# lijx10/DeepI2P

Measured on AMD Instinct MI355X. Metric: frames/sec (img+pc infer + 60-restart GN pose) KITTI 20k-pt, 1/2/4/8 GPU, higher is better.
Workload: dtype f32 network (fp32-input MFMA; 3x3 convolutions, GEMM-shaped point layers and the per-point head: bf16 MFMA on exact three-way fp32 splits, fp32 accumulation) + f64 solver; 1 GPU; BASELINE configs[1]: KITTI 20480-pt / 160x512, batch 32 per GPU, coarse classification + 60-restart 2D GN/LM solver, max_iter 500; mode=frames, points=20480, restarts=60, parallelism=dp1, streams=8, hw_queues=4, hip_graph=True, weights_broadcast_bytes=0

## Files before the change

deepi2p_amd/_lib.py:

```python
import ctypes
import os

import torch

_HERE = os.path.dirname(os.path.abspath(__file__))
LIB_PATH = os.environ.get("DI2P_LIB") or os.path.join(_HERE, "lib", "libdeepi2p_hip.so")
_lib = None

c_void_p, c_int, c_float, c_double, c_ll = ctypes.c_void_p, ctypes.c_int, ctypes.c_float, ctypes.c_double, ctypes.c_longlong


class DeepI2PHipError(RuntimeError):
    pass


class SrcT(ctypes.Structure):
    _fields_ = [("ptr", c_void_p), ("gidx", c_void_p), ("batch_stride", c_ll), ("row_stride", c_int),
                ("channels", c_int), ("mode", c_int), ("group", c_int), ("pad_", c_int)]


class EpilogueT(ctypes.Structure):
    _fields_ = [("scale", c_void_p), ("shift", c_void_p), ("batch_bias", c_void_p), ("relu", c_int),
                ("group_max", c_int), ("g_table", c_void_p * 2), ("g_idx", c_void_p * 2), ("g_w", c_void_p * 2),
                ("g_nodes", c_int * 2), ("g_k", c_int * 2), ("transpose_out", c_int), ("group_max_out", c_void_p),
                ("planes_out", c_void_p)]


class HeadX3T(ctypes.Structure):
    _fields_ = [("src", c_void_p * 2), ("batch_stride", c_ll * 2), ("row_stride", c_int * 2), ("channels", c_int * 2),
                ("W0p", c_void_p), ("W1p", c_void_p), ("scale_shift", c_void_p), ("relu0", c_int), ("relu1", c_int),
                ("tab", c_void_p * 2), ("idx", c_void_p * 2), ("w", c_void_p * 2), ("nodes", c_int * 2),
                ("W2t", c_void_p), ("scale2", c_void_p), ("shift2", c_void_p), ("relu2", c_int), ("P", c_int)]


class HeadLabelsX3T(ctypes.Structure):
    _fields_ = [("y0", c_void_p), ("batch_stride", c_ll), ("row_stride", c_int), ("K", c_int),
                ("W1p", c_void_p), ("scale1", c_void_p), ("shift1", c_void_p), ("relu1", c_int),
                ("W2p", c_void_p), ("scale2", c_void_p), ("shift2", c_void_p), ("P", c_int),
                ("scores", c_void_p), ("coarse", c_void_p), ("fine", c_void_p)]


class SampleOptT(ctypes.Structure):
    _fields_ = [("mode", c_int), ("crop_top", c_int), ("img_scale", c_double), ("img_H", c_int), ("img_W", c_int), ("Hs", c_int), ("Ws", c_int),
                ("amplitude", c_double * 6), ("color_range", c_double * 8)]
    dataset, crop_bottom, resize_k, max_range = 0, 0, 0, 0.0


SRC_DENSE, SRC_GATHER, SRC_GROUP = 0, 1, 2

_SIGS = {
    "di2p_index_max_forward": [c_void_p, c_void_p, c_void_p, c_int, c_int, c_int, c_int, c_void_p, c_void_p],
    "di2p_index_max_values": [c_void_p, c_void_p, c_void_p, c_void_p, c_void_p, c_int, c_int, c_int, c_int, c_void_p, c_void_p],
    "di2p_ball_query_forward": [c_void_p, c_void_p, c_float, c_int, c_int, c_int, c_int, c_void_p],
    "di2p_knn_nodes": [c_void_p, c_void_p, c_void_p, c_void_p, c_int, c_int, c_int, c_int, c_void_p],
    "di2p_cluster_stats": [c_void_p, c_void_p, c_int, c_void_p, c_void_p, c_void_p, c_int, c_int, c_int, c_void_p],
    "di2p_build_point_input": [c_void_p] * 7 + [c_int, c_int, c_int, c_void_p],
    "di2p_interpolate": [c_void_p] * 4 + [c_int] * 5 + [c_void_p],
    "di2p_gather_neighbors": [c_void_p] * 4 + [c_int] * 4 + [c_void_p],
    "di2p_argmax_channels": [c_void_p, c_void_p, c_int, c_int, c_int, c_ll, c_void_p],
    "di2p_pointwise_gemm": [ctypes.POINTER(SrcT), c_int, c_void_p, c_void_p, c_int, c_int, c_int, c_int,
                            ctypes.POINTER(EpilogueT), c_void_p],
    "di2p_pointwise_gemm_x3": [ctypes.POINTER(SrcT), c_int, c_void_p, c_void_p, c_int, c_int, c_int, c_int,
                               ctypes.POINTER(EpilogueT), c_void_p],
    "di2p_pointwise_gemm_x3p": [c_void_p, c_void_p, c_void_p, c_int, c_int, c_int, c_int, ctypes.POINTER(EpilogueT), c_void_p],
    "di2p_bf16x3_pack": [c_void_p, c_int, c_int, c_void_p, c_void_p],
    "di2p_bf16x3_pack_conv3x3": [c_void_p, c_int, c_int, c_int, c_void_p, c_void_p],
    "di2p_batch_gemv": [c_void_p, c_int, c_int, c_void_p, c_int, c_void_p, c_int, c_void_p],
    "di2p_batch_gemv2": [c_void_p, c_int, c_int, c_void_p, c_int, c_int, c_void_p, c_int, c_void_p, c_int, c_void_p],
    "di2p_attention_pool": [c_void_p, c_void_p, c_void_p, c_int, c_int, c_int, c_int, c_void_p],
    "di2p_point_head": [c_void_p, c_int, c_void_p, c_int, c_void_p, c_void_p, c_void_p, c_void_p, c_int, c_void_p, c_void_p,
                        c_void_p, c_int, c_void_p, c_int, c_int, c_int, c_int, c_void_p],
    "di2p_point_chain": [c_void_p, c_int, c_void_p, c_int, c_void_p, c_void_p, c_void_p, c_void_p, c_int, c_void_p, c_void_p,
                         c_void_p, c_int, c_void_p, c_int, c_int, c_int, c_void_p],
    "di2p_conv2d": [c_void_p] * 6 + [c_int] * 11 + [c_void_p],
    "di2p_conv2d_ws": [c_void_p] * 6 + [c_int] * 11 + [c_void_p, c_ll, c_void_p],
    "di2p_maxpool3x3s2": [c_void_p, c_void_p, c_int, c_int, c_int, c_int, c_void_p],
    "di2p_global_avgpool": [c_void_p, c_void_p, c_int, c_int, c_int, c_void_p],
    "di2p_channel_max": [c_void_p, c_void_p, c_int, c_int, c_int, c_void_p],
    "di2p_initial_guess": [c_void_p] * 5 + [c_int, c_int, c_void_p],
    "di2p_solve_batched": [c_void_p] * 6 + [c_double, c_double, ctypes.POINTER(c_double), ctypes.POINTER(c_double)]
                          + [c_int] * 5 + [c_void_p, c_void_p, c_void_p, c_void_p, c_void_p, c_void_p],
    "di2p_solve_batched_f32": [c_void_p] * 6 + [c_double, c_double, ctypes.POINTER(c_double), ctypes.POINTER(c_double)]
                              + [c_int] * 5 + [c_void_p, c_void_p, c_void_p, c_void_p, c_void_p, c_void_p],
    "di2p_select_best": [c_void_p, c_void_p, c_void_p, c_int, c_int, c_int, c_void_p, c_void_p, c_void_p, c_void_p],
    "di2p_solver_residuals": [c_void_p] * 4 + [c_double, c_double, c_int, c_int, c_int, c_void_p, c_void_p, c_void_p, c_void_p],
    "di2p_f32_to_f64": [c_void_p, c_void_p, c_ll, c_void_p],
    "di2p_farthest_point_sampling": [c_void_p, c_void_p, c_void_p, c_void_p, c_int, c_int, c_int, c_void_p],
    "di2p_gather_points": [c_void_p, c_void_p, c_void_p, c_int, c_int, c_int, c_int, c_void_p],
    "di2p_project_labels": [c_void_p, c_void_p, c_int, c_void_p, c_float, c_float, c_float, c_void_p, c_void_p, c_void_p, c_int, c_int, c_void_p],
    "di2p_label_accuracy": [c_void_p, c_void_p, c_void_p, c_void_p, c_void_p, c_int, c_int, c_void_p],
    "di2p_pnp_ransac": [c_void_p] * 5 + [c_int, c_void_p, c_int, c_double, c_int, c_int, c_int, c_int] + [c_void_p] * 7,
    "di2p_draw_restarts": [ctypes.c_ulonglong, c_int, c_int, c_double, c_double, c_void_p, c_void_p, c_void_p],
    "di2p_random_choice": [ctypes.c_ulonglong, c_int, c_int, c_int, c_int, c_void_p, c_void_p, c_void_p],
    "di2p_random_choice_ragged": [ctypes.c_ulonglong, c_int, c_int, c_void_p, c_int, c_int, c_void_p, c_void_p, c_void_p],
    "di2p_voxel_down_sample": [c_void_p, c_void_p, c_int, c_int, c_int, c_double, c_double, c_int] + [c_void_p] * 9,
    "di2p_estimate_normals": [c_void_p, c_int, c_int, c_double, c_int, c_double] + [c_void_p] * 5,
    "di2p_nearest_raw": [c_void_p, c_void_p, c_void_p, c_int, c_int, c_double] + [c_void_p] * 5,
    "di2p_gather_ragged": [c_void_p] * 6 + [c_int, c_int] + [c_void_p] * 4,
    "di2p_pnp_pack": [c_void_p] * 4 + [c_int, c_int, c_int] + [c_void_p] * 3,
    "di2p_pnp_ransac_epnp": [c_void_p] * 5 + [c_int, c_void_p, c_int, c_double, c_int, c_int] + [c_void_p] * 7,
    "di2p_classifier_loss": [c_void_p] * 4 + [c_int, c_int, c_int, c_float, c_float, c_float] + [c_void_p] * 5,
    "di2p_adam_step": [c_void_p] * 4 + [c_ll, c_int, c_float, c_float, c_float, c_float, c_void_p],
    "di2p_pack_pc_label": [c_void_p, c_void_p, c_void_p, c_void_p, c_void_p, c_void_p, c_int, c_int, c_void_p],
    "di2p_stem_pack": [c_void_p, c_void_p, c_void_p],
    "di2p_conv7x7s2_stem": [c_void_p] * 5 + [c_int] * 4 + [c_void_p],
    "di2p_winograd_weight_transform": [c_void_p, c_void_p, c_int, c_int, c_void_p],
    "di2p_winograd_weight_transform_dgrad": [c_void_p, c_void_p, c_int, c_int, c_void_p],
    "di2p_conv3x3_winograd": [c_void_p] * 6 + [c_int] * 6 + [c_void_p],
    "di2p_conv3x3_x3": [c_void_p] * 6 + [c_int] * 7 + [c_void_p] * 4 + [c_int, c_void_p],
    "di2p_conv3x3_x3_supported": [c_int] * 7,
    "di2p_conv3x3_x3_plan": [c_int] * 7 + [ctypes.POINTER(ctypes.c_int32)],
    "di2p_head_x3_pack": [c_void_p, c_int, c_void_p, c_void_p],
    "di2p_stem_x3_pack": [c_void_p, c_void_p, c_void_p],
    "di2p_stem_x3_supported": [c_int, c_int],
    "di2p_stem_x3": [c_void_p] * 5 + [c_int] * 3 + [c_void_p],
    "di2p_point_head_x3": [ctypes.POINTER(HeadX3T), c_void_p, c_int, c_int, c_void_p],
    "di2p_head_labels_x3_pack": [c_void_p, c_int, c_int, c_void_p, c_void_p],
    "di2p_point_head_labels_x3": [ctypes.POINTER(HeadLabelsX3T), c_int, c_int, c_void_p],
    "di2p_bn_train_forward": [c_void_p] * 9 + [c_float, c_float, c_int, c_int, c_int, c_int, c_void_p, c_void_p],
    "di2p_bn_train_backward": [c_void_p] * 6 + [c_int] + [c_void_p] * 4 + [c_int, c_int, c_int, c_void_p, c_void_p],
    "di2p_channel_sum": [c_void_p, c_void_p, c_int, c_int, c_int, c_void_p, c_void_p],
    "di2p_bmm_rc": [c_void_p, c_ll, c_ll, c_void_p, c_ll, c_ll, c_void_p, c_int, c_int, c_int, c_int, c_float, c_int, c_void_p, c_ll, c_void_p],
    "di2p_rc_vec_ok": [c_void_p, c_ll, c_ll, c_int],
    "di2p_rc_route": [c_int] * 7 + [ctypes.POINTER(ctypes.c_int32)],
    "di2p_pointwise_route": [c_int] * 6 + [ctypes.POINTER(ctypes.c_int32)],
    "di2p_conv2d_route": [c_int] * 12 + [c_ll, ctypes.POINTER(ctypes.c_int32)],
    "di2p_winograd_route": [c_int] * 5 + [ctypes.POINTER(ctypes.c_int32)],
    "di2p_point_chain_route": [c_int] * 6 + [ctypes.POINTER(ctypes.c_int32)],
    "di2p_point_head_route": [c_int] * 8 + [ctypes.POINTER(ctypes.c_int32)],
    "di2p_bmm_km": [c_void_p, c_int, c_ll, c_void_p, c_int, c_ll, c_void_p, c_int, c_int, c_int, c_int, c_float, c_void_p],
    "di2p_gather_backward": [c_void_p, c_void_p, c_void_p, c_int, c_void_p, c_int, c_int, c_int, c_int, c_void_p, c_ll, c_void_p],
    "di2p_conv2d_wgrad": [c_void_p] * 3 + [c_int] * 9 + [c_void_p, c_ll, c_void_p],
    "di2p_conv2d_dgrad": [c_void_p] * 3 + [c_int] * 9 + [c_void_p],
    "di2p_maxpool3x3s2_backward": [c_void_p] * 3 + [c_int] * 4 + [c_void_p],
    "di2p_segment_max_backward": [c_void_p] * 4 + [c_int] * 4 + [c_void_p],
    "di2p_group_max_forward": [c_void_p, c_void_p, c_void_p, c_ll, c_int, c_void_p],
    "di2p_group_max_backward": [c_void_p, c_void_p, c_void_p, c_ll, c_int, c_void_p],
    "di2p_dropout_mask": [ctypes.c_ulonglong, c_int, c_float, c_ll, c_void_p, c_void_p],
    "di2p_apply_mask": [c_void_p, c_void_p, c_float, c_void_p, c_ll, c_void_p],
    "di2p_sample_draws": [ctypes.c_ulonglong, c_void_p, c_int, c_int, ctypes.POINTER(SampleOptT)] + [c_void_p] * 10,
    "di2p_image_prepare": [c_void_p, c_int, c_int, c_int, ctypes.POINTER(SampleOptT), c_void_p, c_void_p, c_int, c_int, c_int, c_void_p, c_void_p,
                           c_void_p],
    "di2p_transform_segments": [c_void_p] * 4 + [c_int, c_int] + [c_void_p] * 3,
    "di2p_gather_ragged_aug": [c_void_p] * 6 + [c_int, c_int, ctypes.c_ulonglong, c_void_p, c_int, c_double, c_double] + [c_void_p] * 4,
    "di2p_random_choice_dseed": [c_void_p, c_int, c_int, c_int, c_int, c_void_p, c_void_p, c_void_p],
    "di2p_random_choice_ragged_dseed": [c_void_p, c_int, c_int, c_void_p, c_int, c_int, c_void_p, c_void_p, c_void_p],
    "di2p_range_shuffle": [c_void_p, c_void_p, c_int, c_int, c_int, c_double, ctypes.c_ulonglong] + [c_void_p] * 6,
    "di2p_gather_ragged_aug_intensity": [c_void_p] * 5 + [c_int, c_int, ctypes.c_ulonglong, c_void_p, c_int, c_double, c_double] + [c_void_p] * 3,
    "di2p_sample_draws_ds": [ctypes.c_ulonglong, c_void_p, c_int, c_int, ctypes.POINTER(SampleOptT), c_int] + [c_void_p] * 10,
    "di2p_image_prepare_ds": [c_void_p, c_int, c_int, c_int, ctypes.POINTER(SampleOptT), c_int, c_int, c_void_p, c_void_p, c_void_p, c_int, c_int,
                              c_void_p, c_void_p, c_void_p],
    "di2p_estimate_normals_cells": [c_void_p, c_int, c_int, c_double, c_int, c_double] + [c_void_p] * 5,
    "di2p_compose_poses": [c_void_p, c_void_p, c_int, c_void_p, c_void_p],
    "di2p_pose_errors": [c_void_p, c_void_p, c_int, c_void_p, c_int, c_int, c_double, c_double, c_void_p, c_void_p, c_void_p, c_void_p],
    "di2p_eval_accumulate": [c_void_p] * 5 + [c_int, c_void_p, c_void_p],
    "di2p_eval_acc_reset": [c_void_p, c_void_p],
    "di2p_enu2cam_points": [c_void_p, c_void_p, c_int, c_int, c_void_p],
    "di2p_vis_classification": [c_void_p] * 6 + [c_int] * 10 + [c_void_p] * 3,
    "di2p_vis_registration": [c_void_p] * 5 + [c_int] * 7 + [c_void_p] * 3,
    "di2p_submap_build": [c_void_p] * 6 + [c_int] * 5 + [c_double, c_double, c_int] + [c_void_p] * 7,
    "di2p_submap_to_camera": [c_void_p] * 4 + [c_int, c_int, c_void_p, c_void_p],
    "di2p_pose_matrices": [c_void_p, c_int, c_void_p, c_void_p],
    "di2p_sweep_transforms": [c_void_p] * 5 + [c_int, c_int] + [c_void_p] * 3,
    "di2p_sweep_accumulate": [c_void_p] * 4 + [c_int] * 6 + [c_float, c_float] + [c_void_p] * 6,
    "di2p_world_trace": [c_void_p, c_void_p, c_int, c_int, c_void_p, c_void_p, c_int, c_void_p, c_void_p, c_void_p],
    "di2p_world_render_camera": [c_void_p, c_void_p, c_int, c_int, c_void_p, c_void_p, c_int, c_int, c_double] + [c_void_p] * 4,
    "di2p_world_render_scan": [c_void_p, c_void_p, c_int, c_int, c_void_p, c_void_p, c_void_p, c_int, c_int] + [c_double] * 4
                              + [ctypes.c_ulonglong, c_void_p, c_int] + [c_void_p] * 5,
}
# ... 122 lines not shown
```

deepi2p_amd/csrc/common.h:

```cpp
#pragma once
#include <hip/hip_runtime.h>
#include <stdint.h>
#include <stdio.h>

#include "../../include/deepi2p_hip.h"

#define DI2P_WAVE 64

void di2p_set_error(const char* fmt, ...);

#define DI2P_CHECK_ARG(cond, msg)                                   \
    do {                                                            \
        if (!(cond)) {                                              \
            di2p_set_error("%s: %s", __func__, msg);                \
            return -1;                                              \
        }                                                           \
    } while (0)

#define DI2P_RETURN_LAUNCH()                                                        \
    do {                                                                            \
        hipError_t e_ = hipGetLastError();                                          \
        if (e_ != hipSuccess) {                                                     \
            di2p_set_error("%s: launch failed: %s", __func__, hipGetErrorString(e_)); \
            return (int)e_;                                                         \
        }                                                                           \
        return 0;                                                                   \
    } while (0)

static inline int di2p_cdiv(long long a, long long b) { return (int)((a + b - 1) / b); }

#define DI2P_OPTIONS(X) \
    X(CONV_NOSPLIT, "conv_nosplit", "DI2P_CONV_NOSPLIT", 0)                        \
    X(CONV_DEPTH1, "conv_depth1", "DI2P_CONV_DEPTH1", 0)                           \
    X(PW_NOVEC, "pw_novec", "DI2P_PW_NOVEC", 0)                                    \
    X(SOLVER_NOCULL, "solver_nocull", "DI2P_SOLVER_NOCULL", 0)                     \
    X(SOLVER_NOPREFILTER, "solver_noprefilter", "DI2P_SOLVER_NOPREFILTER", 0)      \
    X(SOLVER_TIER_SWEEPS, "solver_tier_sweeps", "DI2P_SOLVER_TIER_SWEEPS", 0)      \
    X(WINO_COB, "wino_cob", "DI2P_WINO_COB", 0)                                    \
    X(CONV_NOWINOGRAD, "conv_nowinograd", "DI2P_CONV_NOWINOGRAD", 0)               \
    X(WINO_KC, "wino_kc", "DI2P_WINO_KC", 0)                                       \
    X(CONV_NOSTEM, "conv_nostem", "DI2P_CONV_NOSTEM", 0)                           \
    X(WINO_REG, "wino_reg", "DI2P_WINO_REG", 0)                                    \
    X(SOLVER_NOCACHE, "solver_nocache", "DI2P_SOLVER_NOCACHE", 0)                  \
    X(SOLVER_PREP_SINGLE, "solver_prep_single", "DI2P_SOLVER_PREP_SINGLE", 0)      \
    X(SOLVER_PREP_BITONIC, "solver_prep_bitonic", "DI2P_SOLVER_PREP_BITONIC", 0)   \
    X(PW_X3, "pw_x3", "DI2P_PW_X3", 1)                                             \
    X(PW_NOCHAIN, "pw_nochain", "DI2P_PW_NOCHAIN", 0)                              \
    X(HEAD_REG, "head_reg", "DI2P_HEAD_REG", 0)                                    \
    X(CONV_S2SCALAR, "conv_s2scalar", "DI2P_CONV_S2SCALAR", 0)                     \
    X(CONV_X3, "conv_x3", "DI2P_CONV_X3", 31)                                      \
    X(CONV_X3_CFG, "conv_x3_cfg", "DI2P_CONV_X3_CFG", -1)                          \
    X(HEAD_X3, "head_x3", "DI2P_HEAD_X3", 1)                                       \
    X(HEAD_X3_TAB, "head_x3_tab", "DI2P_HEAD_X3_TAB", 1)                           \
    X(STEM_X3, "stem_x3", "DI2P_STEM_X3", 1)                                       \
    X(BN_UNFUSED, "bn_unfused", "DI2P_BN_UNFUSED", 0)                              \
    X(PW_X3_PLANES, "pw_x3_planes", "DI2P_PW_X3_PLANES", 1)                        \
    X(CONV_DGRAD_DENSE, "conv_dgrad_dense", "DI2P_CONV_DGRAD_DENSE", 0)            \
    X(RC_TILE64, "rc_tile64", "DI2P_RC_TILE64", 0)
enum Di2pOption {
#define DI2P_OPT_ENUM(ID, NAME, ENV, DEF) DI2P_OPT_##ID,
    DI2P_OPTIONS(DI2P_OPT_ENUM)
#undef DI2P_OPT_ENUM
    DI2P_OPT_COUNT
};
long long di2p_opt(int id);
int di2p_cu_count();
int di2p_allow_dynamic_lds(const void* kernel, size_t bytes, const char* who);
void di2p_pack_a32(const float* Wt, int K, int M, int tiles, int tile_stride, int step_stride, void* Wp, void* stream);
```

deepi2p_amd/csrc/gemm.hip:

```cpp
#include "bf16x3.h"
#include "mfma_tile.h"

#include <stdint.h>
#include <stdlib.h>

namespace {

struct LoaderWt {
    const float* Wt;
    int K, M;
    __device__ __forceinline__ float load(int k, int m) const { return (k < K && m < M) ? Wt[k * M + m] : 0.0f; }
};

struct SrcDev {
    const float* ptr[DI2P_MAX_SRC];
    const int* gidx[DI2P_MAX_SRC];
    long long batch_stride[DI2P_MAX_SRC];
    int row_stride[DI2P_MAX_SRC];
    int c_end[DI2P_MAX_SRC];
    int mode[DI2P_MAX_SRC];
    int group[DI2P_MAX_SRC];
    int n_src;
};

// ... 400 lines not shown
    __syncthreads();
    {
        LoaderWt4 la{tl.W1t, HEAD_M, HEAD_M};
        EpiDev e1{};
        e1.scale = tl.sc1; e1.shift = tl.sh1; e1.relu = tl.relu1; e1.group_max = 1;
        EpiPointwise ep{e1, nullptr, b, HEAD_M, N};
        ep.lds_tile = hbuf; ep.lds_n0 = j_blk; ep.lds_ld = HEAD_BN;
        mfma_gemm_block_blds<HeadCfg>(stage, la, hbuf, HEAD_BN, ep, HEAD_M, 0, j_blk);
    }
    __syncthreads();
    const int lane = threadIdx.x & 63, p = threadIdx.x >> 6;
    const int n = j_blk + lane;
    if (p < tl.P) {
        float a = 0.0f;
        for (int k0 = 0; k0 < HEAD_M; k0 += 16) {
            float w[16], h[16];
#pragma unroll
            for (int u = 0; u < 16; ++u) { w[u] = tl.W2t[(k0 + u) * tl.P + p]; h[u] = hbuf[(k0 + u) * HEAD_BN + lane]; }
#pragma unroll
            for (int u = 0; u < 16; ++u) a = fmaf(w[u], h[u], a);
        }
        if (tl.sc2) a *= tl.sc2[p];
        if (tl.sh2) a += tl.sh2[p];
        if (tl.relu2) a = fmaxf(a, 0.0f);
        if (n < N) out[((long long)b * tl.P + p) * N + n] = a;
    }
}

struct ChainTail {
    const float* W1t;
    const float* sc1;
    const float* sh1;
    const float* W2t;
    const float* sc2;
    const float* sh2;
    int relu1, relu2;
};

__device__ __forceinline__ void chain_rows_to_ksteps(const float (&v)[16], float* f) {
#pragma unroll
    for (int g = 0; g < 4; ++g) {
        auto p = __builtin_amdgcn_permlane32_swap(__float_as_uint(v[4 * g + 0]), __float_as_uint(v[4 * g + 1]), false, false);
        auto q = __builtin_amdgcn_permlane32_swap(__float_as_uint(v[4 * g + 2]), __float_as_uint(v[4 * g + 3]), false, false);
        f[4 * g + 0] = __uint_as_float(p[0]);
        f[4 * g + 1] = __uint_as_float(q[0]);
        f[4 * g + 2] = __uint_as_float(p[1]);
        f[4 * g + 3] = __uint_as_float(q[1]);
    }
}

#ifndef DI2P_CHAIN_WAVES
#define DI2P_CHAIN_WAVES 2
#endif
template <int M, int KS0, int NL, int TN>
__global__ __launch_bounds__(256) __attribute__((amdgpu_waves_per_eu(DI2P_CHAIN_WAVES, 8))) void point_chain_kernel(const float* __restrict__ X, long long x_bs, int x_rs, const float* __restrict__ W0t,
                                                           int K0, EpiDev e0, ChainTail tl, float* __restrict__ Y, int N, int nblk, int total) {
    constexpr int TM = M / 32, KS = M / 2, KSMAX = KS0 > KS ? KS0 : KS;
    extern __shared__ __attribute__((aligned(16))) float lds[];
    float* w0 = lds;
    float* w1 = w0 + 2 * KS0 * M;
    float* w2 = w1 + M * M;
    float* ss = w2 + (NL == 3 ? M * M : 0);
    for (int i = threadIdx.x; i < 2 * KS0 * M; i += 256) w0[i] = i < K0 * M ? W0t[i] : 0.0f;
    for (int i = threadIdx.x; i < M * M; i += 256) w1[i] = tl.W1t[i];
    if (NL == 3)
        for (int i = threadIdx.x; i < M * M; i += 256) w2[i] = tl.W2t[i];
    {
        const float* rows[6] = {e0.scale, e0.shift, tl.sc1, tl.sh1, NL == 3 ? tl.sc2 : nullptr, NL == 3 ? tl.sh2 : nullptr};
#pragma unroll
        for (int q = 0; q < 6; ++q)
            if (rows[q] && threadIdx.x < M) ss[q * M + threadIdx.x] = rows[q][threadIdx.x];
    }
    __syncthreads();
    if (e0.scale) e0.scale = ss;
    if (e0.shift) e0.shift = ss + M;
    const int lane = threadIdx.x & 63, wave = __builtin_amdgcn_readfirstlane(threadIdx.x >> 6);
    const int l31 = lane & 31, half = lane >> 5;
    EpiDev e1{}, e2{};
    e1.scale = tl.sc1 ? ss + 2 * M : nullptr; e1.shift = tl.sh1 ? ss + 3 * M : nullptr; e1.relu = tl.relu1; e1.group_max = 1;
    e2.scale = tl.sc2 ? ss + 4 * M : nullptr; e2.shift = tl.sh2 ? ss + 5 * M : nullptr; e2.relu = tl.relu2; e2.group_max = 1;

    float fn[TN][KS0];
    auto request = [&](int g) {
        const int fb = g / nblk, blk = g - fb * nblk;
        const float* Xb = X + (long long)fb * x_bs;
#pragma unroll
        for (int s = 0; s < KS0; ++s) {
            const int k = 2 * s + half;
#pragma unroll
            for (int j = 0; j < TN; ++j) {
                const float x = Xb[(long long)min(k, K0 - 1) * x_rs + min((blk * TN + j) * 32 + l31, N - 1)];
                fn[j][s] = k < K0 ? x : 0.0f;
            }
        }
    };
    const int g0 = blockIdx.x * 4 + wave, stride = gridDim.x * 4;
    if (g0 < total) request(g0);
    for (int g = g0; g < total; g += stride) {
        const int b = g / nblk, blk = g - b * nblk;
        EpiPointwise ep0{e0, nullptr, b, M, N}, ep1{e1, nullptr, b, M, N}, ep2{e2, nullptr, b, M, N};
        int n[TN], nc[TN];
#pragma unroll
        for (int j = 0; j < TN; ++j) { n[j] = (blk * TN + j) * 32 + l31; nc[j] = min(n[j], N - 1); }
        float f[TN][KSMAX];
#pragma unroll
        for (int j = 0; j < TN; ++j)
#pragma unroll
            for (int s = 0; s < KS0; ++s) f[j][s] = fn[j][s];
        request(min(g + stride, total - 1));
        f32x16 acc[TM][TN];
        auto zero = [&]() {
#pragma unroll
            for (int i = 0; i < TM; ++i)
#pragma unroll
                for (int j = 0; j < TN; ++j)
#pragma unroll
                    for (int r = 0; r < 16; ++r) acc[i][j][r] = 0.0f;
        };
        auto layer = [&](const float* w, auto ks_tag) {
            constexpr int STEPS = decltype(ks_tag)::value;
            const float* wl = w + half * M + l31;
#pragma unroll
            for (int s = 0; s < STEPS; ++s) {
                float a[TM];
#pragma unroll
                for (int i = 0; i < TM; ++i) a[i] = wl[2 * s * M + i * 32];
#pragma unroll
                for (int i = 0; i < TM; ++i)
#pragma unroll
                    for (int j = 0; j < TN; ++j) acc[i][j] = __builtin_amdgcn_mfma_f32_32x32x2f32(a[i], f[j][s], acc[i][j], 0, 0, 0);
            }
        };
        auto to_operands = [&](const EpiPointwise& ep) {
#pragma unroll
            for (int j = 0; j < TN; ++j)
#pragma unroll
                for (int i = 0; i < TM; ++i) {
                    float v[16];
                    ep.apply(i * 32 + 4 * half, nc[j], acc[i][j], v);
                    chain_rows_to_ksteps(v, &f[j][i * 16]);
                }
        };
        auto to_memory = [&](const EpiPointwise& ep) {
#pragma unroll
            for (int j = 0; j < TN; ++j)
#pragma unroll
                for (int i = 0; i < TM; ++i) {
                    float v[16];
                    ep.apply(i * 32 + 4 * half, nc[j], acc[i][j], v);
                    if (n[j] < N) {
#pragma unroll
                        for (int r = 0; r < 16; ++r)
                            Y[((long long)b * M + i * 32 + 4 * half + (r & 3) + 8 * (r >> 2)) * N + n[j]] = v[r];
                    }
                }
        };
        zero();
        layer(w0, std::integral_constant<int, KS0>{});
        to_operands(ep0);
        zero();
        layer(w1, std::integral_constant<int, KS>{});
        if (NL == 3) {
            to_operands(ep1);
            zero();
            layer(w2, std::integral_constant<int, KS>{});
            to_memory(ep2);
        } else {
            to_memory(ep1);
        }
    }
}

template <bool G33, int KS0>
__global__ __launch_bounds__(512) void point_head_reg_kernel(SrcDev srcs, const float* __restrict__ W0t, int K0, EpiDev e0, HeadTail tl,
                                                              float* __restrict__ out, int N, int nblk, int total) {
    constexpr int M = HEAD_M, TM = M / 32, KS = M / 2;
    extern __shared__ __attribute__((aligned(16))) float lds[];
    float* w0 = lds;
    float* w1 = w0 + 2 * KS0 * M;
    float* w2 = w1 + M * M;
    float* ss = w2 + M * 4;
    for (int i = threadIdx.x; i < 2 * KS0 * M; i += 512) w0[i] = i < K0 * M ? W0t[i] : 0.0f;
    for (int i = threadIdx.x; i < M * M; i += 512) w1[i] = tl.W1t[i];
    for (int i = threadIdx.x; i < M * 4; i += 512) w2[i] = (i & 3) < tl.P ? tl.W2t[(i >> 2) * tl.P + (i & 3)] : 0.0f;
    {
        const float* rows[4] = {e0.scale, e0.shift, tl.sc1, tl.sh1};
#pragma unroll
        for (int q = 0; q < 4; ++q)
            if (rows[q] && threadIdx.x < M) ss[q * M + threadIdx.x] = rows[q][threadIdx.x];
    }
    __syncthreads();
    if (e0.scale) e0.scale = ss;
    if (e0.shift) e0.shift = ss + M;
    EpiDev e1{};
    e1.scale = tl.sc1 ? ss + 2 * M : nullptr; e1.shift = tl.sh1 ? ss + 3 * M : nullptr; e1.relu = tl.relu1; e1.group_max = 1;
    const int lane = threadIdx.x & 63, wave = __builtin_amdgcn_readfirstlane(threadIdx.x >> 6);
    const int l31 = lane & 31, half = lane >> 5;
    const int c0 = srcs.c_end[0];

    constexpr int CH = 8;
    static_assert(KS0 % CH == 0, "layer 0 = whole chunks");
    float f0[KS0];
    auto request = [&](int g) {
        const int fb = __builtin_amdgcn_readfirstlane(g / nblk);
        const int col = min((g - fb * nblk) * 32 + l31, N - 1);
        const int rs0 = srcs.row_stride[0], rs1 = srcs.row_stride[1];
// ... 699 lines not shown
    else hipLaunchKernelGGL(pointwise_gemm_x3p_kernel<false>, grid, dim3(256), 0, st, (const u32x4_t*)planes, (const u32x4_t*)Wp, Y, M, K, N, Mp, e);
    DI2P_RETURN_LAUNCH();
}

extern "C" int di2p_point_head(const di2p_src_t* srcs, int n_src, const float* W0t, int K0, const di2p_epilogue_t* epi0,
                               const float* W1t, const float* scale1, const float* shift1, int relu1, const float* W2t,
                               const float* scale2, const float* shift2, int relu2, float* out, int B, int M, int P, int N,
                               void* stream) {
    DI2P_CHECK_ARG(srcs && n_src >= 1 && n_src <= DI2P_MAX_SRC && W0t && W1t && W2t && out && epi0, "null pointer");
    DI2P_CHECK_ARG(M == HEAD_M && P >= 1 && P <= 4, "fused head: hidden width 128, at most 4 outputs (use the separate layers otherwise)");
    DI2P_CHECK_ARG(B >= 0 && N >= 4 && N % 4 == 0 && K0 >= 1, "bad size");
    DI2P_CHECK_ARG(epi0->group_max <= 1 && !epi0->transpose_out && !epi0->planes_out, "fused head: layer 0 takes scale/shift/relu/bias/gathered only");
    if (B == 0) return 0;
    for (int i = 0; i < n_src; ++i) DI2P_CHECK_ARG(srcs[i].ptr && srcs[i].channels > 0 && srcs[i].mode == DI2P_SRC_DENSE, "fused head: dense sources only");
    SrcDev s;
    bool dense;
    if (pw_sources(__func__, srcs, n_src, K0, "K0", s, dense)) return -1;
    DI2P_CHECK_ARG(dense, "sources must be 16-byte addressable");
    DI2P_CHECK_ARG(aligned16(W0t) && aligned16(W1t), "weights must be 16-byte aligned");
    EpiDev e;
    if (pw_epilogue(__func__, epi0, nullptr, M, N, false, e)) return -1;
    HeadTail tl{W1t, scale1, shift1, W2t, scale2, shift2, relu1, relu2, P};
    bool reg_range = true;
    for (int i = 0; i < n_src; ++i) reg_range = reg_range && (long long)srcs[i].channels * srcs[i].row_stride * 4 < (1ll << 31);
    const HeadRoute rt = head_route(K0, n_src, srcs[0].channels, reg_range, e.g_table[0] && e.g_table[1] && e.g_k[0] == 3 && e.g_k[1] == 3, B, N,
                                    di2p_cu_count());
    if (rt.reg) {
        constexpr int KS0 = 48;
        const int nblk = rt.nblk;
        const long long total = rt.total;
        DI2P_CHECK_ARG(total < (1ll << 30), "too many column blocks");
        const int wgs = rt.wgs;
        const size_t lds_reg = (size_t)(2 * KS0 * HEAD_M + HEAD_M * HEAD_M + HEAD_M * 4 + 4 * HEAD_M) * sizeof(float);
        if (rt.g33) {
            if (di2p_allow_dynamic_lds((const void*)point_head_reg_kernel<true, KS0>, lds_reg, __func__)) return -1;
            hipLaunchKernelGGL((point_head_reg_kernel<true, KS0>), dim3(wgs), dim3(512), lds_reg, (hipStream_t)stream, s, W0t, K0, e, tl, out, N, nblk, (int)total);
        } else {
            if (di2p_allow_dynamic_lds((const void*)point_head_reg_kernel<false, KS0>, lds_reg, __func__)) return -1;
            hipLaunchKernelGGL((point_head_reg_kernel<false, KS0>), dim3(wgs), dim3(512), lds_reg, (hipStream_t)stream, s, W0t, K0, e, tl, out, N, nblk, (int)total);
        }
        DI2P_RETURN_LAUNCH();
    }
    const size_t lds = (HeadCfg::LDS_FLOATS + HEAD_M * HEAD_BN) * sizeof(float);
    if (rt.g33) {
        if (di2p_allow_dynamic_lds((const void*)point_head_kernel<true>, lds, __func__)) return -1;
        hipLaunchKernelGGL(point_head_kernel<true>, dim3(di2p_cdiv(N, HEAD_BN), B), dim3(HeadCfg::THREADS), lds, (hipStream_t)stream, s, W0t, K0, e, tl, out, N);
    } else {
        if (di2p_allow_dynamic_lds((const void*)point_head_kernel<false>, lds, __func__)) return -1;
        hipLaunchKernelGGL(point_head_kernel<false>, dim3(di2p_cdiv(N, HEAD_BN), B), dim3(HeadCfg::THREADS), lds, (hipStream_t)stream, s, W0t, K0, e, tl, out, N);
    }
    DI2P_RETURN_LAUNCH();
}

extern "C" int di2p_point_chain(const di2p_src_t* srcs, int n_src, const float* W0t, int K0, const di2p_epilogue_t* epi0,
                                const float* W1t, const float* scale1, const float* shift1, int relu1, const float* W2t,
                                const float* scale2, const float* shift2, int relu2, float* Y, int B, int M, int N, void* stream) {
    DI2P_CHECK_ARG(srcs && n_src == 1 && W0t && W1t && epi0, "fused chain: one dense source");
    DI2P_CHECK_ARG(M == 32 || M == 64, "fused chain: width 32 or 64 (use the separate layers otherwise)");
    DI2P_CHECK_ARG(K0 <= M, "fused chain: at most M input channels");
    DI2P_CHECK_ARG(B >= 0 && N >= 1 && K0 >= 1, "bad size");
    DI2P_CHECK_ARG(epi0->group_max <= 1 && !epi0->transpose_out && !epi0->planes_out, "fused chain: layer 0 takes scale/shift/relu/bias/gathered only");
    if (B == 0) return 0;
    DI2P_CHECK_ARG(Y && srcs[0].ptr && srcs[0].channels == K0 && srcs[0].mode == DI2P_SRC_DENSE, "fused chain: one dense source of K0 channels");
    DI2P_CHECK_ARG((long long)srcs[0].channels * srcs[0].row_stride < (1ll << 31), "per-frame source extent must fit 31 bits");
    EpiDev e;
    if (pw_epilogue(__func__, epi0, nullptr, M, N, false, e)) return -1;
    ChainTail tl{W1t, scale1, shift1, W2t, scale2, shift2, relu1, relu2};
    const float* X = srcs[0].ptr;
    const long long x_bs = srcs[0].batch_stride;
    const int x_rs = (int)srcs[0].row_stride;
    hipStream_t st = (hipStream_t)stream;
    const ChainRoute rt = chain_route(M, K0, W2t != nullptr, B, N, di2p_cu_count());
    DI2P_CHECK_ARG(rt.total < (1ll << 30), "too many column blocks");
#define DI2P_CHAIN_LAUNCH(MM, KS0, NL, TN)                                                                                          \
    do {                                                                                                                            \
        const size_t lds = (size_t)(2 * (KS0) * (MM) + ((NL) - 1) * (MM) * (MM) + 6 * (MM)) * sizeof(float);                        \
        hipLaunchKernelGGL((point_chain_kernel<MM, KS0, NL, TN>), dim3(rt.wgs), dim3(256), lds, st, X, x_bs, x_rs, W0t, K0, e, tl, Y, N, \
                           rt.nblk, (int)rt.total);                                                                                 \
    } while (0)
    const bool three = rt.layers == 3;
    if (M == 32) {
        if (rt.ks0 == 4) { if (three) DI2P_CHAIN_LAUNCH(32, 4, 3, DI2P_CHAIN_TN32); else DI2P_CHAIN_LAUNCH(32, 4, 2, DI2P_CHAIN_TN32); }
        else             { if (three) DI2P_CHAIN_LAUNCH(32, 16, 3, DI2P_CHAIN_TN32); else DI2P_CHAIN_LAUNCH(32, 16, 2, DI2P_CHAIN_TN32); }
    } else {
        if (rt.ks0 == 16) { if (three) DI2P_CHAIN_LAUNCH(64, 16, 3, DI2P_CHAIN_TN64); else DI2P_CHAIN_LAUNCH(64, 16, 2, DI2P_CHAIN_TN64); }
        else              { if (three) DI2P_CHAIN_LAUNCH(64, 32, 3, DI2P_CHAIN_TN64); else DI2P_CHAIN_LAUNCH(64, 32, 2, DI2P_CHAIN_TN64); }
    }
#undef DI2P_CHAIN_LAUNCH
    DI2P_RETURN_LAUNCH();
}

extern "C" int di2p_point_chain_route(int M, int K0, int layers, int B, int N, int cus, int32_t* out) {
    DI2P_CHECK_ARG(out && (M == 32 || M == 64) && K0 >= 1 && K0 <= M && (layers == 2 || layers == 3) && B >= 1 && N >= 1 && cus >= 1, "bad args");
    const ChainRoute rt = chain_route(M, K0, layers == 3, B, N, cus);
    DI2P_CHECK_ARG(rt.total < (1ll << 30), "too many column blocks");
    out[0] = M; out[1] = rt.ks0; out[2] = rt.layers; out[3] = rt.tn; out[4] = rt.nblk; out[5] = (int)rt.total; out[6] = rt.wgs; out[7] = rt.w;
    return 0;
}

extern "C" int di2p_point_head_route(int K0, int n_src, int c0, int reg_range, int g33, int B, int N, int cus, int32_t* out) {
    DI2P_CHECK_ARG(out && K0 >= 1 && n_src >= 1 && n_src <= DI2P_MAX_SRC && c0 >= 1 && c0 <= K0 && B >= 1 && N >= 4 && N % 4 == 0 && cus >= 1, "bad args");
    const HeadRoute rt = head_route(K0, n_src, c0, reg_range != 0, g33 != 0, B, N, cus);
    DI2P_CHECK_ARG(!rt.reg || rt.total < (1ll << 30), "too many column blocks");
    out[0] = rt.reg; out[1] = rt.g33; out[2] = rt.bn; out[3] = rt.nblk; out[4] = (int)rt.total; out[5] = rt.wgs;
    return 0;
}

extern "C" int di2p_batch_gemv(const float* Wt, int M, int k0, const float* v, int Kv, float* out, int B, void* stream) {
    DI2P_CHECK_ARG(Wt && v && out && M >= 1 && Kv >= 1 && k0 >= 0 && B >= 0, "bad args");
    if (B == 0) return 0;
    hipLaunchKernelGGL(batch_gemv_kernel, dim3(di2p_cdiv(M, 64), B), dim3(256), 0, (hipStream_t)stream, Wt, M, k0, v, Kv, 0,
                       (const float*)nullptr, 0, out);
    DI2P_RETURN_LAUNCH();
}

extern "C" int di2p_batch_gemv2(const float* Wt, int M, int k0, const float* v0, int Kv0, int k1, const float* v1, int Kv1,
                                float* out, int B, void* stream) {
    DI2P_CHECK_ARG(Wt && v0 && v1 && out && M >= 1 && Kv0 >= 1 && Kv1 >= 1 && k0 >= 0 && k1 >= 0 && B >= 0, "bad args");
    if (B == 0) return 0;
    hipLaunchKernelGGL(batch_gemv_kernel, dim3(di2p_cdiv(M, 64), B), dim3(256), 0, (hipStream_t)stream, Wt, M, k0, v0, Kv0, k1, v1, Kv1, out);
    DI2P_RETURN_LAUNCH();
}

extern "C" int di2p_attention_pool(const float* feat, const float* score, float* out, int B, int C, int HW, int Mn, void* stream) {
    DI2P_CHECK_ARG(feat && score && out && B >= 0 && C >= 1 && HW >= 1 && Mn >= 1, "bad args");
    if (B == 0) return 0;
    using Cfg = Cfg64x64;
    hipLaunchKernelGGL(attention_pool_kernel<Cfg>, dim3(di2p_cdiv(Mn, Cfg::BN), di2p_cdiv(C, Cfg::BM), B), dim3(Cfg::THREADS),
                       Cfg::LDS_FLOATS * sizeof(float), (hipStream_t)stream, feat, score, out, C, HW, Mn);
    DI2P_RETURN_LAUNCH();
}
```

deepi2p_amd/csrc/head_x3.hip:

```cpp
#include <stdint.h>

#include <type_traits>

#include "bf16x3.h"
#include "common.h"

namespace {

using bf16x3::u32x4_t;
using bf16x3::f32x16;

constexpr int HX_M = 128, HX_TM = 4, HX_TROW = HX_M + 4;

struct HxArgs {
    const float* src[2]; long long src_bs[2]; int src_rs[2]; int c0, K0;
    const u32x4_t* W0p; const u32x4_t* W1p;
    const float* ss;
    const float* tab[2]; const int* idx[2]; const float* gw[2]; int nodes[2];
    const float* W2t; const float* sc2; const float* sh2;
    float* out;
    int relu0, relu1, relu2, P, N, nblk, total, parts;
};

template <bool TAB_LDS, int KS0, int NW, int MINW, bool SYNC, bool DEEP, bool LEAN = false>
__global__ __launch_bounds__(NW * 64, MINW) void point_head_x3_kernel(const HxArgs a) {
    extern __shared__ __attribute__((aligned(16))) float lds[];
    float* ssl = lds;
    float* w2l = ssl + 4 * HX_M;
    float* tabl = w2l + 4 * HX_M;
    const int tid = threadIdx.x, lane = tid & 63, wave = __builtin_amdgcn_readfirstlane(tid >> 6);
    const int nl = lane & 31, h = lane >> 5;
    for (int i = tid; i < 4 * HX_M; i += NW * 64) {
        ssl[i] = a.ss[i];
        w2l[i] = (i & 3) < a.P ? a.W2t[(i >> 2) * a.P + (i & 3)] : 0.0f;
    }
    int g_first, g_stride, g_end, fb_fixed = 0;
    if (TAB_LDS) {
        const int fb = blockIdx.x / a.parts, part = blockIdx.x - fb * a.parts;
        fb_fixed = fb;
#pragma unroll
        for (int t = 0; t < 2; ++t) {
            const float* T = a.tab[t] + (long long)fb * a.nodes[t] * HX_M;
            float* L = tabl + (t == 0 ? 0 : a.nodes[0] * HX_TROW);
            for (int i = tid; i < a.nodes[t] * (HX_M / 4); i += NW * 64) {
                const int node = i / (HX_M / 4), c4 = i - node * (HX_M / 4);
                *reinterpret_cast<float4*>(L + node * HX_TROW + 4 * c4) = *reinterpret_cast<const float4*>(T + node * HX_M + 4 * c4);
            }
        }
        g_first = fb * a.nblk + part * NW + wave; g_stride = a.parts * NW; g_end = (fb + 1) * a.nblk;
    } else {
        g_first = blockIdx.x * NW + wave; g_stride = gridDim.x * NW; g_end = a.total;
    }
    __syncthreads();
    const __amdgpu_buffer_rsrc_t w0r = __builtin_amdgcn_make_buffer_rsrc((void*)a.W0p, 0, (a.K0 / 16) * HX_TM * 3 * 1024, 0x00020000);
    const __amdgpu_buffer_rsrc_t w1r = __builtin_amdgcn_make_buffer_rsrc((void*)a.W1p, 0, (HX_M / 16) * HX_TM * 3 * 1024, 0x00020000);

    int gi_n[6];
    float gw_n[6], x_n[KS0][8];
    const int trips = SYNC ? (g_end - (g_first - wave) + g_stride - 1) / g_stride : 0;
    for (int it = 0, g0 = g_first; SYNC ? it < trips : g0 < g_end; ++it, g0 += g_stride) {
        const bool live = g0 < g_end;
        const int g = SYNC ? min(g0, g_end - 1) : g0;
        asm volatile("" ::: "memory");
        int hq = 4 * h;
        asm volatile("" : "+v"(hq));
        const int fb = TAB_LDS ? fb_fixed : __builtin_amdgcn_readfirstlane(g / a.nblk);
        const int n = (g - fb * a.nblk) * 32 + nl, nc = min(n, a.N - 1);
        auto request_nb = [&](int gg, int (&gi_)[6], float (&gw_)[6]) __attribute__((always_inline)) {
            const int fq = TAB_LDS ? fb_fixed : __builtin_amdgcn_readfirstlane(gg / a.nblk);
            const int nq = min((gg - fq * a.nblk) * 32 + nl, a.N - 1);
#pragma unroll
            for (int t = 0; t < 2; ++t)
#pragma unroll
                for (int j = 0; j < 3; ++j) {
                    const long long o = ((long long)fq * a.N + nq) * 3 + j;
                    gi_[3 * t + j] = a.idx[t][o];
                    gw_[3 * t + j] = a.gw[t] ? a.gw[t][o] : 1.0f;
                }
        };
        auto x_load = [&](int gg, int s, float (&f)[8]) __attribute__((always_inline)) {
            const int fq = TAB_LDS ? fb_fixed : __builtin_amdgcn_readfirstlane(gg / a.nblk);
            const int nq = min((gg - fq * a.nblk) * 32 + nl, a.N - 1);
            const __amdgpu_buffer_rsrc_t r0 = __builtin_amdgcn_make_buffer_rsrc((void*)(a.src[0] + (long long)fq * a.src_bs[0]), 0, a.c0 * a.src_rs[0] * 4, 0x00020000);
            const __amdgpu_buffer_rsrc_t r1 = __builtin_amdgcn_make_buffer_rsrc((void*)(a.src[1] + (long long)fq * a.src_bs[1]), 0, (a.K0 - a.c0) * a.src_rs[1] * 4, 0x00020000);
            const int v0 = (8 * h * a.src_rs[0] + nq) * 4, v1 = (8 * h * a.src_rs[1] + nq) * 4;
            const int c = 16 * s;
            if (c < a.c0) {
#pragma unroll
                for (int e = 0; e < 8; ++e) f[e] = __builtin_bit_cast(float, __builtin_amdgcn_raw_buffer_load_b32(r0, v0, (c + e) * a.src_rs[0] * 4, 0));
            } else {
#pragma unroll
                for (int e = 0; e < 8; ++e) f[e] = __builtin_bit_cast(float, __builtin_amdgcn_raw_buffer_load_b32(r1, v1, (c - a.c0 + e) * a.src_rs[1] * 4, 0));
            }
        };
        int gi[6];
        float gwt[6];
        float xall[KS0][8];
        if (it == 0) {
            request_nb(g, gi_n, gw_n);
#pragma unroll
            for (int s = 0; s < KS0; ++s) x_load(g, s, x_n[s]);
        }
#pragma unroll
        for (int s = 0; s < 6; ++s) { gi[s] = gi_n[s]; gwt[s] = gw_n[s]; }
#pragma unroll
        for (int s = 0; s < KS0; ++s)
#pragma unroll
            for (int e = 0; e < 8; ++e) xall[s][e] = x_n[s][e];
        f32x16 acc[HX_TM];
#pragma unroll
        for (int i = 0; i < HX_TM; ++i)
#pragma unroll
            for (int r = 0; r < 16; ++r) acc[i][r] = 0.0f;
        u32x4_t af[2][HX_TM][3];
        auto a_load = [&](int slot, const __amdgpu_buffer_rsrc_t& wr, int ks, int p) __attribute__((always_inline)) {
#pragma unroll
            for (int i = 0; i < HX_TM; ++i) af[slot][i][p] = __builtin_amdgcn_raw_buffer_load_b128(wr, lane * 16, ((ks * HX_TM + i) * 3 + p) * 1024, 0);
        };
        auto kstep = [&](int slot, const u32x4_t (&bf)[3], const __amdgpu_buffer_rsrc_t& wr, int ks_next) __attribute__((always_inline)) {
#define DI2P_HX_PROD(QA, QB) _Pragma("unroll") for (int i = 0; i < HX_TM; ++i) acc[i] = bf16x3::mma(af[slot][i][QA], bf[QB], acc[i]);
            if constexpr (SYNC) __builtin_amdgcn_s_barrier();
            if constexpr (DEEP) {
                if (ks_next >= 0) { a_load(slot ^ 1, wr, ks_next, 2); a_load(slot ^ 1, wr, ks_next, 1); a_load(slot ^ 1, wr, ks_next, 0); }
            }
            DI2P_HX_PROD(2, 0)
            if (!DEEP && ks_next >= 0) a_load(slot ^ 1, wr, ks_next, 2);
            DI2P_HX_PROD(1, 1) DI2P_HX_PROD(1, 0)
            if (!DEEP && ks_next >= 0) a_load(slot ^ 1, wr, ks_next, 1);
// ... 43 lines not shown
                if (LEAN) {
                    if (k + 1 < 4 * HX_TM) g_issue(k + 1, q[(k + 1) & 1]);
                    __builtin_amdgcn_sched_barrier(0);
                } else if ((k & 1) == 0) {
                    if (k + 2 < 4 * HX_TM) g_issue(k + 2, q[(k + 2) & 3]);
                    if (k + 3 < 4 * HX_TM) g_issue(k + 3, q[(k + 3) & 3]);
                    __builtin_amdgcn_sched_barrier(0);
                }
                const float4 (&qq)[6] = q[LEAN ? (k & 1) : (k & 3)];
                float4 t4 = make_float4(0.0f, 0.0f, 0.0f, 0.0f);
#pragma unroll
                for (int s = 0; s < 6; ++s) {
                    t4.x = fmaf(gwt[s], qq[s].x, t4.x); t4.y = fmaf(gwt[s], qq[s].y, t4.y);
                    t4.z = fmaf(gwt[s], qq[s].z, t4.z); t4.w = fmaf(gwt[s], qq[s].w, t4.w);
                }
                const float4 sc = *reinterpret_cast<const float4*>(ssl + 32 * i + 8 * gq + hq);
                const float4 sh = *reinterpret_cast<const float4*>(ssl + HX_M + 32 * i + 8 * gq + hq);
                v[4 * gq + 0] = (acc[i][4 * gq + 0] + t4.x) * sc.x + sh.x; v[4 * gq + 1] = (acc[i][4 * gq + 1] + t4.y) * sc.y + sh.y;
                v[4 * gq + 2] = (acc[i][4 * gq + 2] + t4.z) * sc.z + sh.z; v[4 * gq + 3] = (acc[i][4 * gq + 3] + t4.w) * sc.w + sh.w;
                if (LEAN || (k & 1)) __builtin_amdgcn_sched_barrier(0);
            }
            if (a.relu0) {
#pragma unroll
                for (int r = 0; r < 16; ++r) v[r] = fmaxf(v[r], 0.0f);
            }
#pragma unroll
            for (int q2 = 0; q2 < 2; ++q2)
#pragma unroll
                for (int j = 0; j < 4; ++j) {
                    float X = v[8 * q2 + j], Y = v[8 * q2 + 4 + j];
                    asm volatile("s_nop 1\n\tv_permlane32_swap_b32 %0, %1" : "+v"(X), "+v"(Y));
                    f1[2 * i + q2][j] = X;
                    f1[2 * i + q2][4 + j] = Y;
                }
        }
#pragma unroll
        for (int i = 0; i < HX_TM; ++i)
#pragma unroll
            for (int r = 0; r < 16; ++r) acc[i][r] = 0.0f;
        {
            u32x4_t bfr[2][3];
            bf16x3::split8(f1[0], bfr[0][0], bfr[0][1], bfr[0][2]);
#pragma unroll
            for (int s = 0; s < 2 * HX_TM; ++s) {
                __builtin_amdgcn_sched_barrier(0);
                if (s + 1 < 2 * HX_TM) bf16x3::split8(f1[s + 1], bfr[(s + 1) & 1][0], bfr[(s + 1) & 1][1], bfr[(s + 1) & 1][2]);
                kstep(s & 1, bfr[s & 1], w1r, s + 1 < 2 * HX_TM ? s + 1 : -1);
#pragma unroll
                for (int u = 0; u < 6 * HX_TM; ++u) { __builtin_amdgcn_sched_group_barrier(0x008, 1, 0); __builtin_amdgcn_sched_group_barrier(0x002, 3, 0); }
            }
            __builtin_amdgcn_sched_barrier(0);
        }
        __builtin_amdgcn_sched_barrier(0);
        {
            const int gn = min(g + g_stride, g_end - 1);
            request_nb(gn, gi_n, gw_n);
#pragma unroll
            for (int s = 0; s < KS0; ++s) x_load(gn, s, x_n[s]);
        }
        __builtin_amdgcn_sched_barrier(0);
        float part[4] = {0.0f, 0.0f, 0.0f, 0.0f};
#pragma unroll
        for (int i = 0; i < HX_TM; ++i)
#pragma unroll
            for (int gq = 0; gq < 4; ++gq) {
                if (gq & 1) __builtin_amdgcn_sched_barrier(0);
                const int row = 32 * i + 8 * gq + hq;
                const float4 sc = *reinterpret_cast<const float4*>(ssl + 2 * HX_M + row);
                const float4 sh = *reinterpret_cast<const float4*>(ssl + 3 * HX_M + row);
                float y[4] = {acc[i][4 * gq + 0] * sc.x + sh.x, acc[i][4 * gq + 1] * sc.y + sh.y, acc[i][4 * gq + 2] * sc.z + sh.z, acc[i][4 * gq + 3] * sc.w + sh.w};
#pragma unroll
                for (int j = 0; j < 4; ++j) {
                    if (a.relu1) y[j] = fmaxf(y[j], 0.0f);
                    const float4 w = *reinterpret_cast<const float4*>(w2l + 4 * (row + j));
                    part[0] = fmaf(w.x, y[j], part[0]); part[1] = fmaf(w.y, y[j], part[1]);
                    part[2] = fmaf(w.z, y[j], part[2]); part[3] = fmaf(w.w, y[j], part[3]);
                }
                if (LEAN) asm volatile("" : "+v"(part[0]), "+v"(part[1]), "+v"(part[2]), "+v"(part[3]));
            }
#pragma unroll
        for (int p = 0; p < 4; ++p) {
            const float other = __builtin_bit_cast(float, __builtin_amdgcn_ds_bpermute((lane ^ 32) * 4, __builtin_bit_cast(int, part[p])));
            float o = (hq ? other : part[p]) + (hq ? part[p] : other);
            if (p < a.P) {
                if (a.sc2) o *= a.sc2[p];
                if (a.sh2) o += a.sh2[p];
                if (a.relu2) o = fmaxf(o, 0.0f);
                if (n < a.N && hq == 0 && live) a.out[((long long)fb * a.P + p) * a.N + n] = o;
            }
        }
    }
}

__global__ __launch_bounds__(256) void pack_a32_kernel(const float* __restrict__ Wt, unsigned short* __restrict__ Wp, int K, int M, int tiles,
                                                       int tile_stride, int step_stride) {
    const long long t = (long long)blockIdx.x * 256 + threadIdx.x;
    const int ks = K / 16;
    if (t >= (long long)tiles * ks * 64) return;
    const int lane = (int)(t & 63), s = (int)((t >> 6) % ks), tile = (int)((t >> 6) / ks);
    const int row = 32 * tile + (lane & 31), k0 = 16 * s + 8 * (lane >> 5);
    unsigned short* d = Wp + (((long long)tile * tile_stride + (long long)s * step_stride) * 3 * 64 + lane) * 8;
#pragma unroll
    for (int e = 0; e < 8; ++e) {
        const float v = row < M ? Wt[(long long)(k0 + e) * M + row] : 0.0f;
        float pl[3];
        bf16x3::split(v, pl[0], pl[1], pl[2]);
#pragma unroll
        for (int p = 0; p < 3; ++p) d[p * 64 * 8 + e] = bf16x3::bits(pl[p]);
    }
}

}

void di2p_pack_a32(const float* Wt, int K, int M, int tiles, int tile_stride, int step_stride, void* Wp, void* stream) {
    hipLaunchKernelGGL(pack_a32_kernel, dim3(di2p_cdiv((long long)tiles * (K / 16) * 64, 256)), dim3(256), 0, (hipStream_t)stream, Wt,
                       (unsigned short*)Wp, K, M, tiles, tile_stride, step_stride);
}

extern "C" long long di2p_head_x3_packed_bytes(int K) { return K >= 16 && K % 16 == 0 ? (long long)(K / 16) * HX_TM * 3 * 1024 : 0; }

extern "C" int di2p_head_x3_pack(const float* Wt, int K, void* Wp, void* stream) {
    DI2P_CHECK_ARG(Wt && Wp && K >= 16 && K % 16 == 0, "needs K % 16 == 0 (and 128 output channels)");
    DI2P_CHECK_ARG(((uintptr_t)Wp & 15) == 0, "packed weights must be 16-byte aligned");
    di2p_pack_a32(Wt, K, HX_M, HX_TM, 1, HX_TM, Wp, stream);
    DI2P_RETURN_LAUNCH();
}

extern "C" int di2p_point_head_x3(const di2p_head_x3_t* hd, float* out, int B, int N, void* stream) {
    DI2P_CHECK_ARG(hd && out, "null pointer");
    DI2P_CHECK_ARG(B >= 0 && N >= 1, "bad size");
    DI2P_CHECK_ARG(hd->src[0] && hd->src[1] && hd->W0p && hd->W1p && hd->scale_shift && hd->W2t, "null operand");
    DI2P_CHECK_ARG(hd->channels[0] >= 16 && hd->channels[0] % 16 == 0 && hd->channels[1] >= 16 && hd->channels[1] % 16 == 0, "source channels must be multiples of 16");
    DI2P_CHECK_ARG(hd->P >= 1 && hd->P <= 4, "1..4 outputs");
    for (int t = 0; t < 2; ++t) DI2P_CHECK_ARG(hd->tab[t] && hd->idx[t] && hd->nodes[t] >= 1, "both gathered tables (3 neighbours each) are required");
    DI2P_CHECK_ARG(((uintptr_t)hd->W0p & 15) == 0 && ((uintptr_t)hd->W1p & 15) == 0 && ((uintptr_t)hd->tab[0] & 15) == 0 && ((uintptr_t)hd->tab[1] & 15) == 0 &&
                   ((uintptr_t)hd->scale_shift & 15) == 0, "16-byte alignment of the packed weights, the tables and the scale / shift rows");
    for (int t = 0; t < 2; ++t)
        DI2P_CHECK_ARG((long long)hd->channels[t] * hd->row_stride[t] * 4 < (1ll << 31), "per-frame source extent must fit 31 bits");
    if (B == 0) return 0;
    HxArgs a{};
    for (int t = 0; t < 2; ++t) {
        a.src[t] = hd->src[t]; a.src_bs[t] = hd->batch_stride[t]; a.src_rs[t] = hd->row_stride[t];
        a.tab[t] = hd->tab[t]; a.idx[t] = hd->idx[t]; a.gw[t] = hd->w[t]; a.nodes[t] = hd->nodes[t];
    }
    a.c0 = hd->channels[0]; a.K0 = hd->channels[0] + hd->channels[1];
    a.W0p = (const u32x4_t*)hd->W0p; a.W1p = (const u32x4_t*)hd->W1p; a.ss = hd->scale_shift;
    a.W2t = hd->W2t; a.sc2 = hd->scale2; a.sh2 = hd->shift2; a.out = out;
    a.relu0 = hd->relu0; a.relu1 = hd->relu1; a.relu2 = hd->relu2; a.P = hd->P; a.N = N;
    a.nblk = di2p_cdiv(N, 32); a.total = B * a.nblk;
    hipStream_t st = (hipStream_t)stream;
    const size_t lds_small = (size_t)8 * HX_M * sizeof(float);
    const size_t lds_tab = lds_small + (size_t)(hd->nodes[0] + hd->nodes[1]) * HX_TROW * sizeof(float);
    const long long opt = di2p_opt(DI2P_OPT_HEAD_X3_TAB);
    DI2P_CHECK_ARG(a.K0 == 96, "this build instantiates the head for 96 dense channels (32 + 64: first_pointnet + second_pointnet)");
    if (opt != 0 && lds_tab <= 160 * 1024) {
        const int cus = di2p_cu_count();
        int parts = di2p_cdiv(cus, B);
        while (parts > 1 && a.nblk < parts * 16) --parts;
        a.parts = parts;
        if (opt == 2) {
            if (di2p_allow_dynamic_lds((const void*)point_head_x3_kernel<true, 6, 4, 1, false, true>, lds_tab, __func__)) return -1;
            hipLaunchKernelGGL((point_head_x3_kernel<true, 6, 4, 1, false, true>), dim3(B * parts), dim3(256), lds_tab, st, a);
        } else {
            if (di2p_allow_dynamic_lds((const void*)point_head_x3_kernel<true, 6, 8, 2, false, false, true>, lds_tab, __func__)) return -1;
            hipLaunchKernelGGL((point_head_x3_kernel<true, 6, 8, 2, false, false, true>), dim3(B * parts), dim3(512), lds_tab, st, a);
        }
    } else {
        const int grid = (int)(a.total / 4 < 1ll * di2p_cu_count() ? di2p_cdiv(a.total, 4) : di2p_cu_count());
        hipLaunchKernelGGL((point_head_x3_kernel<false, 6, 4, 1, false, true>), dim3(grid), dim3(256), lds_small, st, a);
    }
    DI2P_RETURN_LAUNCH();
}
```

deepi2p_amd/csrc/point_ops.hip:

```cpp
#include "common.h"

namespace {

template <int KN>
__global__ __launch_bounds__(256) void knn_nodes_kernel(const float* __restrict__ query, const float* __restrict__ nodes,
                                                        int* __restrict__ idx, float* __restrict__ weights, int Nq,
                                                        int M) {
    const int b = blockIdx.y;
    const float* __restrict__ nb = nodes + (long long)b * 3 * M;
    const int n = blockIdx.x * blockDim.x + threadIdx.x;
    const int nc = min(n, Nq - 1);
    const float* q = query + (long long)b * 3 * Nq;
    const float qx = q[nc], qy = q[Nq + nc], qz = q[2 * Nq + nc];
    unsigned kd[KN];
    int ki[KN];
#pragma unroll
    for (int j = 0; j < KN; ++j) { kd[j] = 0x7f800001u; ki[j] = 0x7fffffff; }
    auto consider = [&](float nx, float ny, float nz, int m) __attribute__((always_inline)) {
        const float dx = __fsub_rn(qx, nx), dy = __fsub_rn(qy, ny), dz = __fsub_rn(qz, nz);
        const unsigned d = __float_as_uint(__fadd_rn(__fadd_rn(__fmul_rn(dx, dx), __fmul_rn(dy, dy)), __fmul_rn(dz, dz)));
        bool lt[KN];
#pragma unroll
        for (int j = 0; j < KN; ++j) lt[j] = d < kd[j];
#pragma unroll
// ... 87 lines not shown
            bi[j] = sw ? bi[j - 1] : t;
            bi[j - 1] = sw ? t : bi[j - 1];
        }
    int mine_i = 0;
    float mine_d = 0.0f;
#pragma unroll
    for (int j = 0; j < KN; ++j)
        if (lane == j) { mine_i = bi[j]; mine_d = bd[j]; }
    if (lane < KN) idx[((long long)b * Nq + n) * KN + lane] = mine_i;
    if (weights) {
        float sum = bd[0];
#pragma unroll
        for (int j = 1; j < KN; ++j) sum = __fadd_rn(sum, bd[j]);
        if (lane < KN) weights[((long long)b * Nq + n) * KN + lane] = __fsub_rn(1.0f, __fdiv_rn(mine_d, sum));
    }
}

constexpr double kFix = 16777216.0;

__global__ __launch_bounds__(1024) void cluster_stats_kernel(const float* __restrict__ pc, const int* __restrict__ knn_idx,
                                                             int idx_stride, float* __restrict__ cluster_mean,
                                                             float* __restrict__ mask, int* __restrict__ min_idx, int N,
                                                             int M) {
    extern __shared__ unsigned long long s_acc[];
    const int b = blockIdx.x;
    for (int i = threadIdx.x; i < 4 * M; i += blockDim.x) s_acc[i] = 0ull;
    __syncthreads();
    const float* p = pc + (long long)b * 3 * N;
    const int* ki = knn_idx + (long long)b * N * idx_stride;
    for (int n = threadIdx.x; n < N; n += blockDim.x) {
        const int k = ki[(long long)n * idx_stride];
        if (min_idx) min_idx[(long long)b * N + n] = k;
        const long long fx = __double2ll_rn((double)p[n] * kFix);
        const long long fy = __double2ll_rn((double)p[N + n] * kFix);
        const long long fz = __double2ll_rn((double)p[2 * N + n] * kFix);
        atomicAdd(&s_acc[4 * k + 0], (unsigned long long)fx);
        atomicAdd(&s_acc[4 * k + 1], (unsigned long long)fy);
        atomicAdd(&s_acc[4 * k + 2], (unsigned long long)fz);
        atomicAdd(&s_acc[4 * k + 3], 1ull);
    }
    __syncthreads();
    for (int k = threadIdx.x; k < M; k += blockDim.x) {
        const float cnt = (float)s_acc[4 * k + 3];
        const float den = __fadd_rn(cnt, 1e-5f);
#pragma unroll
        for (int c = 0; c < 3; ++c) {
            const float s = (float)((double)(long long)s_acc[4 * k + c] / kFix);
            cluster_mean[((long long)b * 3 + c) * M + k] = __fdiv_rn(s, den);
        }
        if (mask) mask[(long long)b * M + k] = cnt > 0.0f ? 1.0f : 0.0f;
    }
}

__global__ __launch_bounds__(256) void build_point_input_kernel(const float* __restrict__ pc, const float* __restrict__ intensity,
                                                                const float* __restrict__ sn, const float* __restrict__ cluster_mean,
                                                                const int* __restrict__ min_idx, float* __restrict__ centers,
                                                                float* __restrict__ aug, int N, int M) {
    const int b = blockIdx.y;
    const int n = blockIdx.x * blockDim.x + threadIdx.x;
    if (n >= N) return;
    const int k = min_idx[(long long)b * N + n];
    const float* cm = cluster_mean + (long long)b * 3 * M;
    const float* p = pc + (long long)b * 3 * N;
    float* a = aug + (long long)b * 7 * N;
#pragma unroll
    for (int c = 0; c < 3; ++c) {
        const float ctr = cm[c * M + k];
        if (centers) centers[((long long)b * 3 + c) * N + n] = ctr;
        a[c * N + n] = __fsub_rn(p[c * N + n], ctr);
    }
    a[3 * N + n] = intensity[(long long)b * N + n];
    const float* s = sn + (long long)b * 3 * N;
#pragma unroll
    for (int c = 0; c < 3; ++c) a[(4 + c) * N + n] = s[c * N + n];
}

__global__ __launch_bounds__(256) void interpolate_kernel(const float* __restrict__ feats, const int* __restrict__ idx,
                                                          const float* __restrict__ weights, float* __restrict__ out, int C,
                                                          int M, int Nq, int k) {
    const int b = blockIdx.z;
    const int n = blockIdx.x * blockDim.x + threadIdx.x;
    if (n >= Nq) return;
    const int c0 = blockIdx.y * 32;
    const int* ii = idx + ((long long)b * Nq + n) * k;
    const float* ww = weights + ((long long)b * Nq + n) * k;
    for (int c = c0; c < min(C, c0 + 32); ++c) {
        const float* f = feats + ((long long)b * C + c) * M;
        float acc = 0.0f;
        for (int j = 0; j < k; ++j) acc = __fadd_rn(acc, __fmul_rn(ww[j], f[ii[j]]));
        out[((long long)b * C + c) * Nq + n] = acc;
    }
}

template <int KN>
__global__ __launch_bounds__(256) void interpolate_lds_kernel(const float* __restrict__ feats, const int* __restrict__ idx,
                                                              const float* __restrict__ weights, float* __restrict__ out, int C, int M, int Nq) {
    extern __shared__ float tab[];
    const int b = blockIdx.z, c0 = blockIdx.y * 32, cn = min(32, C - c0);
    const float* f = feats + ((long long)b * C + c0) * M;
    for (int i = threadIdx.x; i < cn * M; i += 256) tab[i] = f[i];
    __syncthreads();
    const int n = blockIdx.x * 256 + threadIdx.x;
    if (n >= Nq) return;
    int ii[KN];
    float ww[KN];
#pragma unroll
    for (int j = 0; j < KN; ++j) { ii[j] = idx[((long long)b * Nq + n) * KN + j]; ww[j] = weights[((long long)b * Nq + n) * KN + j]; }
    for (int c = 0; c < cn; ++c) {
        float acc = 0.0f;
#pragma unroll
        for (int j = 0; j < KN; ++j) acc = __fadd_rn(acc, __fmul_rn(ww[j], tab[c * M + ii[j]]));
        out[((long long)b * C + c0 + c) * Nq + n] = acc;
    }
}

__global__ void gather_neighbors_kernel(const float* __restrict__ database, const float* __restrict__ query,
                                        const int* __restrict__ idx, float* __restrict__ out, int Md, int Mq, int K) {
    const int b = blockIdx.y;
    const int t = blockIdx.x * blockDim.x + threadIdx.x;
    if (t >= Mq * K) return;
    const int m = t / K;
    const int src = idx[(long long)b * Mq * K + t];
#pragma unroll
    for (int c = 0; c < 3; ++c)
        out[((long long)b * 3 + c) * Mq * K + t] =
            __fsub_rn(database[((long long)b * 3 + c) * Md + src], query[((long long)b * 3 + c) * Mq + m]);
}
// ... 23 lines not shown
    float m = -__builtin_inff();
    if (row < rows) {
        const float* r = x + row * N;
        for (int n = n0; n < N; n += G) m = nanmax(m, r[n]);
    }
    for (int o = G >> 1; o > 0; o >>= 1) m = nanmax(m, __shfl_xor(m, o));
    if (row < rows && n0 == 0) y[row] = m;
}

__global__ void f32_to_f64_kernel(const float* __restrict__ in, double* __restrict__ out, long long n) {
    long long i = (long long)blockIdx.x * blockDim.x + threadIdx.x;
    const long long stride = (long long)gridDim.x * blockDim.x;
    for (; i < n; i += stride) out[i] = (double)in[i];
}

}

extern "C" int di2p_knn_nodes(const float* query, const float* nodes, int32_t* idx, float* weights, int B, int Nq, int M,
                              int k, void* stream) {
    DI2P_CHECK_ARG(B >= 0 && Nq >= 0 && M > 0, "bad size");
    DI2P_CHECK_ARG(k >= 1 && k <= 16 && k <= M, "k must be in [1,16] and <= M");
    DI2P_CHECK_ARG(M <= 4096, "M must be <= 4096");
    if (B == 0 || Nq == 0) return 0;
    const dim3 grid(di2p_cdiv(Nq, 256), B), block(256);
    hipStream_t st = (hipStream_t)stream;
    const bool per_wave = M <= 256 && Nq <= 1024;
    const dim3 wgrid(di2p_cdiv(Nq, 4), B);
#define DI2P_KNN_CASE(KK) \
    case KK: if (per_wave) hipLaunchKernelGGL(knn_nodes_wave_kernel<KK>, wgrid, block, 0, st, query, nodes, idx, weights, Nq, M); \
             else hipLaunchKernelGGL(knn_nodes_kernel<KK>, grid, block, 0, st, query, nodes, idx, weights, Nq, M); \
             break;
    switch (k) {
        DI2P_KNN_CASE(1) DI2P_KNN_CASE(2) DI2P_KNN_CASE(3) DI2P_KNN_CASE(4) DI2P_KNN_CASE(5) DI2P_KNN_CASE(6)
        DI2P_KNN_CASE(7) DI2P_KNN_CASE(8) DI2P_KNN_CASE(9) DI2P_KNN_CASE(10) DI2P_KNN_CASE(11) DI2P_KNN_CASE(12)
        DI2P_KNN_CASE(13) DI2P_KNN_CASE(14) DI2P_KNN_CASE(15) DI2P_KNN_CASE(16)
    }
#undef DI2P_KNN_CASE
    DI2P_RETURN_LAUNCH();
}

extern "C" int di2p_cluster_stats(const float* pc, const int32_t* knn_idx, int idx_stride, float* cluster_mean, float* mask,
                                  int32_t* min_idx, int B, int N, int M, void* stream) {
    DI2P_CHECK_ARG(B >= 0 && N >= 0 && M > 0 && idx_stride >= 1, "bad size");
    DI2P_CHECK_ARG(M <= 2048, "M too large");
    if (B == 0) return 0;
    hipLaunchKernelGGL(cluster_stats_kernel, dim3(B), dim3(1024), (size_t)4 * M * sizeof(unsigned long long),
                       (hipStream_t)stream, pc, knn_idx, idx_stride, cluster_mean, mask, min_idx, N, M);
    DI2P_RETURN_LAUNCH();
}

extern "C" int di2p_build_point_input(const float* pc, const float* intensity, const float* sn, const float* cluster_mean,
                                      const int32_t* min_idx, float* pc_centers, float* augmented, int B, int N, int M,
                                      void* stream) {
    DI2P_CHECK_ARG(B >= 0 && N >= 0 && M > 0, "bad size");
    if (B == 0 || N == 0) return 0;
    hipLaunchKernelGGL(build_point_input_kernel, dim3(di2p_cdiv(N, 256), B), dim3(256), 0, (hipStream_t)stream, pc,
                       intensity, sn, cluster_mean, min_idx, pc_centers, augmented, N, M);
    DI2P_RETURN_LAUNCH();
}

extern "C" int di2p_interpolate(const float* feats, const int32_t* idx, const float* weights, float* out, int B, int C, int M,
                                int Nq, int k, void* stream) {
    DI2P_CHECK_ARG(B >= 0 && C >= 0 && M > 0 && Nq >= 0 && k >= 1, "bad size");
    if (B == 0 || C == 0 || Nq == 0) return 0;
    const dim3 grid(di2p_cdiv(Nq, 256), di2p_cdiv(C, 32), B);
    const size_t lds = (size_t)32 * M * sizeof(float);
    if (k <= 4 && lds <= 64 * 1024 && Nq >= 1024) {
        hipStream_t st = (hipStream_t)stream;
        switch (k) {
            case 1: hipLaunchKernelGGL(interpolate_lds_kernel<1>, grid, dim3(256), lds, st, feats, idx, weights, out, C, M, Nq); break;
            case 2: hipLaunchKernelGGL(interpolate_lds_kernel<2>, grid, dim3(256), lds, st, feats, idx, weights, out, C, M, Nq); break;
            case 3: hipLaunchKernelGGL(interpolate_lds_kernel<3>, grid, dim3(256), lds, st, feats, idx, weights, out, C, M, Nq); break;
            default: hipLaunchKernelGGL(interpolate_lds_kernel<4>, grid, dim3(256), lds, st, feats, idx, weights, out, C, M, Nq); break;
        }
        DI2P_RETURN_LAUNCH();
    }
    hipLaunchKernelGGL(interpolate_kernel, grid, dim3(256), 0, (hipStream_t)stream, feats, idx, weights, out, C, M, Nq, k);
    DI2P_RETURN_LAUNCH();
}

extern "C" int di2p_gather_neighbors(const float* database, const float* query, const int32_t* idx, float* out, int B, int Md,
                                     int Mq, int K, void* stream) {
    DI2P_CHECK_ARG(B >= 0 && Md > 0 && Mq >= 0 && K >= 1, "bad size");
    if (B == 0 || Mq == 0) return 0;
    hipLaunchKernelGGL(gather_neighbors_kernel, dim3(di2p_cdiv((long long)Mq * K, 256), B), dim3(256), 0,
                       (hipStream_t)stream, database, query, idx, out, Md, Mq, K);
    DI2P_RETURN_LAUNCH();
}

extern "C" int di2p_argmax_channels(const float* scores, int32_t* out, int B, int C, int N, long long batch_stride, void* stream) {
    DI2P_CHECK_ARG(B >= 0 && C >= 1 && N >= 0, "bad size");
    if (B == 0 || N == 0) return 0;
    if (batch_stride <= 0) batch_stride = (long long)C * N;
    hipLaunchKernelGGL(argmax_channels_kernel, dim3(di2p_cdiv(N, 256), B), dim3(256), 0, (hipStream_t)stream, scores, out, C, N, batch_stride);
    DI2P_RETURN_LAUNCH();
}

extern "C" int di2p_channel_max(const float* x, float* y, int B, int C, int N, void* stream) {
    DI2P_CHECK_ARG(B >= 0 && C >= 0 && N >= 1, "bad size");
    const long long rows = (long long)B * C;
    if (rows == 0) return 0;
    int G = 1;
    while (G < N && G < 64) G <<= 1;
    hipLaunchKernelGGL(channel_max_kernel, dim3(di2p_cdiv(rows, 4 * (64 / G))), dim3(256), 0, (hipStream_t)stream, x, y, rows, N, G);
    DI2P_RETURN_LAUNCH();
}

extern "C" int di2p_f32_to_f64(const float* in, double* out, long long n, void* stream) {
    if (n <= 0) return 0;
    const int blocks = (int)((n + 255) / 256 < 4096 ? (n + 255) / 256 : 4096);
// ... 4 lines not shown
```

deepi2p_amd/csrc/solver.hip:

```cpp
#include "common.h"
#include "solver_prep.h"

#include <float.h>
#include <math.h>
#include <stdlib.h>
#include <type_traits>

#ifndef DI2P_SOLVER_DEFAULT_MINW
#define DI2P_SOLVER_DEFAULT_MINW 4
#endif
#ifndef DI2P_SOLVER_DEFAULT_WPH
#define DI2P_SOLVER_DEFAULT_WPH 4
#endif
#ifndef DI2P_SOLVER_PF
#define DI2P_SOLVER_PF 4
#endif
#ifndef DI2P_SOLVER_PFC
#define DI2P_SOLVER_PFC 2
#endif

namespace {

enum { T_MAX_ITER = 0, T_GRADIENT = 1, T_PARAMETER = 2, T_FUNCTION = 3, T_RADIUS = 4, T_INVALID = 5, T_EVAL_FAIL = 6 };

// ... 1391 lines not shown
        int* sweeps_out = a->sweeps_out;
        if (sweeps_out) sweeps_out[hr] = st.nsweep;
    }
}

__device__ __forceinline__ void angle_axis_to_R(const double* w, double* R) {
    const double t2 = w[0] * w[0] + w[1] * w[1] + w[2] * w[2];
    if (t2 > DBL_EPSILON) {
        const double t = sqrt(t2), wx = w[0] / t, wy = w[1] / t, wz = w[2] / t, c = cos(t), s = sin(t);
        R[0] = c + wx * wx * (1 - c);       R[1] = wx * wy * (1 - c) - wz * s;  R[2] = wy * s + wx * wz * (1 - c);
        R[3] = wz * s + wx * wy * (1 - c);  R[4] = c + wy * wy * (1 - c);       R[5] = -wx * s + wy * wz * (1 - c);
        R[6] = -wy * s + wx * wz * (1 - c); R[7] = wx * s + wy * wz * (1 - c);  R[8] = c + wz * wz * (1 - c);
    } else {
        R[0] = 1; R[1] = -w[2]; R[2] = w[1]; R[3] = w[2]; R[4] = 1; R[5] = -w[0]; R[6] = -w[1]; R[7] = w[0]; R[8] = 1;
    }
}

__global__ __launch_bounds__(64) void select_best_kernel(const double* __restrict__ params, const double* __restrict__ cost,
                                                         const int* __restrict__ has_inside, int np, int R, int* __restrict__ best,
                                                         double* __restrict__ P, double* __restrict__ best_cost) {
    const int f = blockIdx.x, lane = threadIdx.x;
    double bc = __builtin_inf();
    int bi = 0x7fffffff;
    for (int r = lane; r < R; r += 64) {
        const double c = cost[(long long)f * R + r];
        if (c < bc || (c == bc && r < bi)) { bc = c; bi = r; }
    }
#pragma unroll
    for (int o = 32; o > 0; o >>= 1) {
        const double oc = __shfl_xor(bc, o);
        const int oi = __shfl_xor(bi, o);
        if (oc < bc || (oc == bc && oi < bi)) { bc = oc; bi = oi; }
    }
    if (lane != 0) return;
    double* Pf = P + (long long)f * 16;
    for (int i = 0; i < 16; ++i) Pf[i] = (i % 5 == 0) ? 1.0 : 0.0;
    if (has_inside && has_inside[f] == 0) {
        best[f] = -1;
        best_cost[f] = 1e4;
        return;
    }
    if (bi == 0x7fffffff) bi = 0;
    const double* x = params + ((long long)f * R + bi) * np;
    double w[3] = {0, 0, 0};
    int toff;
    if (np == 4) { w[1] = x[0]; toff = 1; } else { w[0] = x[0]; w[1] = x[1]; w[2] = x[2]; toff = 3; }
    double Rm[9];
    angle_axis_to_R(w, Rm);
    for (int r = 0; r < 3; ++r) { for (int c = 0; c < 3; ++c) Pf[r * 4 + c] = Rm[r * 3 + c]; Pf[r * 4 + 3] = x[toff + r]; }
    best[f] = bi;
    best_cost[f] = cost[(long long)f * R + bi];
}

__global__ __launch_bounds__(1024) void initial_guess_kernel(const double* __restrict__ points, const int* __restrict__ labels,
                                                             double* __restrict__ yaw0, int* __restrict__ labels_out,
                                                             int* __restrict__ has_inside, int N) {
    __shared__ double s_a[1024], s_b[1024], s_c[1024];
    const int f = blockIdx.x, tid = threadIdx.x;
    const double* px = points + (long long)f * 3 * N;
    const double* pz = px + 2 * (long long)N;
    const int* lab = labels + (long long)f * N;
    double sx = 0, sz = 0, cnt = 0;
    for (int n = tid; n < N; n += 1024)
        if (lab[n] == 1) { sx += px[n]; sz += pz[n]; cnt += 1.0; }
    s_a[tid] = sx; s_b[tid] = sz; s_c[tid] = cnt;
    __syncthreads();
    for (int o = 512; o > 0; o >>= 1) {
        if (tid < o) { s_a[tid] += s_a[tid + o]; s_b[tid] += s_b[tid + o]; s_c[tid] += s_c[tid + o]; }
        __syncthreads();
    }
    const double count = s_c[0];
    const double mx = s_a[0] / count, mz = s_b[0] / count;
    __syncthreads();
    if (!(count > 0.0)) {
        if (tid == 0) { yaw0[f] = 0.0; has_inside[f] = 0; }
        for (int n = tid; n < N; n += 1024) labels_out[(long long)f * N + n] = lab[n];
        return;
    }
    const double kPi = 3.14159265358979323846;
    double a = fmod(atan2(mz, mx) - kPi / 2 + kPi, 2 * kPi);
    if (a < 0) a += 2 * kPi;
    a -= kPi;
    const double c = cos(a), s = sin(a);
    double zmin = __builtin_inf();
    for (int n = tid; n < N; n += 1024)
        if (lab[n] == 1) zmin = fmin(zmin, -s * px[n] + c * pz[n]);
    s_a[tid] = zmin;
    __syncthreads();
    for (int o = 512; o > 0; o >>= 1) {
        if (tid < o) s_a[tid] = fmin(s_a[tid], s_a[tid + o]);
        __syncthreads();
    }
    const double thr = s_a[0] - 10.0;
    for (int n = tid; n < N; n += 1024) {
        const double zr = -s * px[n] + c * pz[n];
        labels_out[(long long)f * N + n] = zr > thr ? lab[n] : -1;
    }
    if (tid == 0) { yaw0[f] = a; has_inside[f] = 1; }
}

template <int NP>
__global__ __launch_bounds__(256) void residuals_kernel(const double* __restrict__ points, const int* __restrict__ labels,
                                                        const double* __restrict__ Kmat, const double* __restrict__ params, double H,
                                                        double W, int N, double* __restrict__ residuals, int* __restrict__ counts,
                                                        double* __restrict__ cost_out) {
    __shared__ int s_scan[256];
    __shared__ double s_cost[256];
    __shared__ int s_base;
    constexpr int TOFF = NP == 4 ? 1 : 3;
    const int f = blockIdx.x, tid = threadIdx.x;
    const double* px = points + (long long)f * 3 * N;
    const int* lab = labels + (long long)f * N;
    const double* Kf = Kmat + (long long)f * 9;
    const Cam k{Kf[0], Kf[4], Kf[2], Kf[5], H - 1.0, W - 1.0};
    const double* x = params + (long long)f * NP;
    double xr[NP];
    for (int i = 0; i < NP; ++i) xr[i] = x[i];
    Rot<NP> rot;
    make_rot<NP>(xr, rot);
    double* out = residuals + (long long)f * 3 * N;
    if (tid == 0) s_base = 0;
    double cost = 0.0;
    __syncthreads();
    for (int n0 = 0; n0 < N; n0 += 256) {
        const int n = n0 + tid;
        int nr = 0;
        double rv[3] = {0, 0, 0};
        if (n < N && (lab[n] == 0 || lab[n] == 1)) {
            const double X = px[n], Y = px[N + n], Z = px[2 * (long long)N + n];
            const double qx = rot.R[0] * X + rot.R[1] * Y + rot.R[2] * Z, qy = rot.R[3] * X + rot.R[4] * Y + rot.R[5] * Z,
                         qz = rot.R[6] * X + rot.R[7] * Y + rot.R[8] * Z;
            const double p0 = qx + xr[TOFF], p1 = qy + xr[TOFF + 1], p2 = qz + xr[TOFF + 2];
            const double pix_x = p0 * k.fx / p2 + k.cx, pix_y = p1 * k.fy / p2 + k.cy;
            if (lab[n] == 1) {
                nr = 3;
                rv[0] = fmax(-pix_x, 0.0) + fmax(pix_x - k.W1, 0.0);
                rv[1] = fmax(-pix_y, 0.0) + fmax(pix_y - k.H1, 0.0);
                rv[2] = fmax(-p2, 0.0) * 100.0;
            } else {
                nr = 1;
                const double dx = k.W1 * 0.5 - fabs(pix_x - k.W1 * 0.5), dy = k.H1 * 0.5 - fabs(pix_y - k.H1 * 0.5);
                rv[0] = (dx + dy) * (fmax(p2, 0.0) / p2) * (fmax(dx, 0.0) / dx) * (fmax(dy, 0.0) / dy);
            }
            const double s = rv[0] * rv[0] + rv[1] * rv[1] + rv[2] * rv[2];
            cost += 0.5 * log1p(s);
            const double sq = sqrt(1.0 / (1.0 + s));
            for (int i = 0; i < 3; ++i) rv[i] *= sq;
        }
// ... 99 lines not shown
        if (g_prof) DI2P_LAUNCH_SOLVE(4, (MINW > 3 ? 3 : MINW), WPH, true, pend1, tier, 0);
        else DI2P_LAUNCH_SOLVE(4, MINW, WPH, false, pend1, tier, 0);
        if (tier > 0) DI2P_LAUNCH_SOLVE(4, 3, 12, false, pending, 0, 1);
    } else {
        if (g_prof) DI2P_LAUNCH_SOLVE(6, 2, 4, true, pend1, tier, 0);
        else DI2P_LAUNCH_SOLVE(6, 2, 4, false, pend1, tier, 0);
        if (tier > 0) DI2P_LAUNCH_SOLVE(6, 2, 8, false, pending, 0, 1);
    }
#undef DI2P_LAUNCH_SOLVE
    return 0;
}

}

template <typename PT>
static int solve_batched_entry(const char* who, const PT* points, const int32_t* labels, const double* K, const double* init_y, const double* init_T,
                               const double* yaw0, double H, double W, const double* lb_host, const double* ub_host, int max_iter, int is_2d,
                               int F, int R, int N, double* params, double* cost, int32_t* iters, int32_t* sweeps, void* workspace, void* stream) {
    const bool ptrs = points && labels && K && init_y && init_T && lb_host && ub_host && params && cost && iters && workspace;
    if (!ptrs || !(F >= 0 && R >= 0 && N >= 0 && max_iter >= 0)) { di2p_set_error("%s: %s", who, ptrs ? "bad size" : "null pointer"); return -1; }
    if (F == 0 || R == 0) return 0;
    launch_solve<PT>(points, labels, K, init_y, init_T, yaw0, H, W, lb_host, ub_host, max_iter, is_2d, F, R, N, params, cost, iters, sweeps, workspace, (hipStream_t)stream);
    const hipError_t e = hipGetLastError();
    if (e != hipSuccess) { di2p_set_error("%s: launch failed: %s", who, hipGetErrorString(e)); return (int)e; }
    return 0;
}

extern "C" int di2p_solve_batched(const double* points, const int32_t* labels, const double* K, const double* init_y,
                                  const double* init_T, const double* yaw0, double H, double W, const double* lb_host,
                                  const double* ub_host, int max_iter, int is_2d, int F, int R, int N, double* params,
                                  double* cost, int32_t* iters, int32_t* sweeps, void* workspace, void* stream) {
    return solve_batched_entry(__func__, points, labels, K, init_y, init_T, yaw0, H, W, lb_host, ub_host, max_iter, is_2d, F, R, N, params, cost, iters, sweeps, workspace, stream);
}

extern "C" int di2p_solve_batched_f32(const float* points, const int32_t* labels, const double* K, const double* init_y,
                                      const double* init_T, const double* yaw0, double H, double W, const double* lb_host,
                                      const double* ub_host, int max_iter, int is_2d, int F, int R, int N, double* params,
                                      double* cost, int32_t* iters, int32_t* sweeps, void* workspace, void* stream) {
    return solve_batched_entry(__func__, points, labels, K, init_y, init_T, yaw0, H, W, lb_host, ub_host, max_iter, is_2d, F, R, N, params, cost, iters, sweeps, workspace, stream);
}

extern "C" int di2p_select_best(const double* params, const double* cost, const int32_t* has_inside, int is_2d, int F, int R,
                                int32_t* best, double* P, double* best_cost, void* stream) {
    DI2P_CHECK_ARG(params && cost && best && P && best_cost && F >= 0 && R >= 1, "bad args");
    if (F == 0) return 0;
    hipLaunchKernelGGL(select_best_kernel, dim3(F), dim3(64), 0, (hipStream_t)stream, params, cost, has_inside, is_2d ? 4 : 6, R, best, P, best_cost);
    DI2P_RETURN_LAUNCH();
}

extern "C" int di2p_initial_guess(const double* points, const int32_t* labels, double* yaw0, int32_t* labels_out,
                                  int32_t* has_inside, int F, int N, void* stream) {
    DI2P_CHECK_ARG(points && labels && yaw0 && labels_out && has_inside && F >= 0 && N >= 0, "bad args");
    if (F == 0) return 0;
    hipLaunchKernelGGL(initial_guess_kernel, dim3(F), dim3(1024), 0, (hipStream_t)stream, points, labels, yaw0, labels_out, has_inside, N);
    DI2P_RETURN_LAUNCH();
}

extern "C" int di2p_solver_residuals(const double* points, const int32_t* labels, const double* K, const double* params, double H,
                                     double W, int is_2d, int F, int N, double* residuals, int32_t* counts, double* cost,
                                     void* stream) {
    DI2P_CHECK_ARG(points && labels && K && params && residuals && counts && cost && F >= 0 && N >= 0, "bad args");
    if (F == 0) return 0;
    if (is_2d)
        hipLaunchKernelGGL(residuals_kernel<4>, dim3(F), dim3(256), 0, (hipStream_t)stream, points, labels, K, params, H, W, N, residuals, counts, cost);
    else
        hipLaunchKernelGGL(residuals_kernel<6>, dim3(F), dim3(256), 0, (hipStream_t)stream, points, labels, K, params, H, W, N, residuals, counts, cost);
    DI2P_RETURN_LAUNCH();
}

extern "C" long long di2p_solve_workspace_bytes(int F, int R, int N) {
    if (F < 0 || N < 0 || R < 0) return 0;
    return (long long)solve_ws_layout(F, R, N).bytes;
}

extern "C" void di2p_solver_set_profile_buffer(void* buf) { g_prof = (long long*)buf; }
```

deepi2p_amd/networks.py:

```python
import torch
import torch.nn as nn

from . import _lib, ops
from .ops import Src

BN_EPS = 1e-5


class _Holder(nn.Module):
    pass


def _register(root, key, tensor, is_buffer):
    parts = key.split(".")
    mod = root
    for p in parts[:-1]:
        if p not in mod._modules:
            mod.add_module(p, _Holder())
        mod = mod._modules[p]
    if is_buffer:
        mod.register_buffer(parts[-1], tensor)
    else:
        mod.register_parameter(parts[-1], nn.Parameter(tensor, requires_grad=False))

# ... 122 lines not shown

def _run_pn(x, layers, **kw):
    N = x.shape[2]
    if not kw and ops.point_chain_ok([Src(x)], layers, N):
        return ops.point_chain([Src(x)], layers, N)
    for layer in layers:
        x = _run_layer([Src(x)], layer, N, **kw)
    return x


def _run_split_pn(dense_srcs, dense_rows, node_feats, node_rows, idx, layers, N):
    Wt, scale, shift, act = layers[0]
    M = Wt.shape[1]
    B = node_feats.shape[0]
    head = (Wt[dense_rows[0]:dense_rows[1]], scale, shift, act)
    chain = [head] + list(layers[1:])
    if ops.point_chain_ok(dense_srcs, chain, N):
        G = ops.pointwise_gemm([Src(node_feats)], Wt[node_rows[0]:node_rows[1]], M, node_feats.shape[2], transpose_out=True)
        return ops.point_chain(dense_srcs, chain, N, gathered=[(G, idx.reshape(B, N, 1), None)])
    x = _run_split_layer(dense_srcs, dense_rows, node_feats, node_rows, idx, layers[0], N)
    return _run_pn(x, layers[1:])


class PCEncoder(_PackedModule):
    def __init__(self, opt, Ca: int, Cb: int, Cg: int, prefix=""):
        super().__init__()
        self.opt, self.Ca, self.Cb, self.Cg = opt, Ca, Cb, Cg
        spec = (_pn_spec("first_pointnet", 7, [Ca // 2] * 3, True)
                + _pn_spec("second_pointnet", Ca, [Ca, Ca], True)
                + _c2d_spec("knnlayer.layers_before.0", 3 + Ca, Cb) + _c2d_spec("knnlayer.layers_before.1", Cb, Cb)
                + _c2d_spec("knnlayer.layers_after.0", 2 * Cb, 2 * Cb) + _c2d_spec("knnlayer.layers_after.1", 2 * Cb, Cb)
                + _pn_spec("final_pointnet", 3 + Cb, [Cg // 2, Cg], True))
        _materialise(self, spec)

    def _pack(self):
        if self._packed is None:
            sd = self._sd()
            p = {"first": _pn_pack(sd, "first_pointnet"), "second": _pn_pack(sd, "second_pointnet"),
                 "final": _pn_pack(sd, "final_pointnet")}
            for name in ("layers_before.0", "layers_before.1", "layers_after.0", "layers_after.1"):
                q = "knnlayer." + name
                p[name] = _fold(sd, q + ".conv", q + ".norm")
            self._packed = p
        return self._packed

    def _group_index(self, B, Mb, K, device):
        key = (B, Mb, K, str(device))
        cache = self.__dict__.setdefault("_gidx_cache", {})
        if key not in cache:
            cache[key] = (torch.arange(Mb * K, dtype=torch.int32, device=device) // K).unsqueeze(0).expand(B, -1).contiguous()
            torch.cuda.current_stream().synchronize()
        return cache[key]

    def forward_device(self, pc, intensity, sn, node_a, node_b):
        if pc.size(2) != self.opt.input_pt_num:
            raise RuntimeError("N must equal opt.input_pt_num (the reference bakes it in, networks_pc.py:44-45)")
        p = self._pack()
        B, N, Ma, Mb = pc.size(0), pc.size(2), node_a.size(2), node_b.size(2)
        idx_a, w_a = ops.knn_nodes(pc, node_a, self.opt.k_interp_point_a, want_weights=True)
        cluster_mean, mask, min_idx = ops.cluster_stats(pc, idx_a, Ma)
        pc_centers, aug = ops.build_point_input(pc, intensity, sn, cluster_mean, min_idx)
        first = _run_pn(aug, p["first"])
        _, first_max = ops.index_max(first, min_idx, Ma, return_values=True, mask=mask)
        Ch = first.shape[1]
        second = _run_split_pn([Src(first)], (0, Ch), first_max, (Ch, 2 * Ch), min_idx, p["second"], N)
        _, node_a_features = ops.index_max(second, min_idx, Ma, return_values=True, mask=mask)
        K = self.opt.k_ab
        knn_I = ops.knn_nodes(node_b, cluster_mean, K)
        coord = ops.gather_neighbors(cluster_mean, node_b, knn_I)
        y = _run_split_layer([Src(coord)], (0, 3), node_a_features, (3, 3 + node_a_features.shape[1]), knn_I.view(B, Mb * K),
                             p["layers_before.0"], Mb * K)
        pow2 = K & (K - 1) == 0 and K <= 32
        Cb1 = p["layers_before.1"][0].shape[1]
        pl = [pow2 and ops.x3_planes_link(p["layers_before.1"], p["layers_after.0"][0][Cb1:2 * Cb1], B, Mb * K),
              pow2 and ops.x3_planes_link(p["layers_after.0"], p["layers_after.1"][0], B, Mb * K)]
        if pow2:
            y, fmax = _run_layer([Src(y)], p["layers_before.1"], Mb * K, group_max=K, also_full=True, planes_out=pl[0])
            Cb = y.shape[1]
        else:
            y = _run_layer([Src(y)], p["layers_before.1"], Mb * K)
            Cb = y.shape[1]
            fmax = ops.channel_max(y.view(B, Cb * Mb, K)).view(B, Cb, Mb)
        y = _run_split_layer([y if pl[0] else Src(y)], (Cb, 2 * Cb), fmax, (0, Cb), self._group_index(B, Mb, K, pc.device), p["layers_after.0"], Mb * K,
                             planes_out=pl[1])
        if pow2:
            node_b_features = _run_layer([y if pl[1] else Src(y)], p["layers_after.1"], Mb * K, group_max=K)
        else:
            y = _run_layer([Src(y)], p["layers_after.1"], Mb * K)
            node_b_features = ops.channel_max(y.view(B, y.shape[1] * Mb, K)).view(B, y.shape[1], Mb)
        final = _run_layer([Src(node_b), Src(node_b_features)], p["final"][0], Mb)
        final = _run_pn(final, p["final"][1:])
        global_feature = ops.channel_max(final).unsqueeze(2)
        ref_tuple = (pc_centers, cluster_mean, idx_a, first, second, node_a_features, node_b_features, global_feature)
        return ref_tuple, dict(w_a=w_a, min_idx=min_idx, mask=mask, knn_I=knn_I)

    def forward(self, pc, intensity, sn, node_a, node_b):
        t, _ = self.forward_device(pc, intensity, sn, node_a, node_b)
        return t[0], t[1], t[2].long(), t[3], t[4], t[5], t[6], t[7]


def _block_conv3x3(blk, n, x, stride, residual=None):
    Wt, sc, sh, _ = blk["c" + n]
    Cout = Wt.shape[1]
    kernel, cfg = ops.conv_route(x.shape, (Cout, x.shape[1], 3, 3), stride, 1)
    if kernel == "x3" and stride == 2:
        _, sd_, shd, _ = blk["ds"]
        return ops.conv3x3_x3(x, blk["X" + n], Cout, sc, sh, 2, True, downsample=(blk["Xd"], sd_, shd), cfg=cfg)
    if kernel == "x3":
        return ops.conv3x3_x3(x, blk["X" + n], Cout, sc, sh, 1, True, residual=residual, cfg=cfg), None
    if kernel == "winograd":
        return ops.conv3x3_winograd(x, blk["U" + n], sc, sh, True, residual=residual), None
    return ops.conv2d(x, Wt, sc, sh, 3, 3, stride, 1, True, residual=residual, tap_major=True), None


class ImageEncoder(_PackedModule):
    LAYERS = (3, 4, 6, 3)

    def __init__(self, opt):
        super().__init__()
        self.opt = opt
        r = "backbone"
        spec = [(r + ".conv1.weight", (64, 3, 7, 7))] + _bn_spec(r + ".bn1", 64)
        inpl = 64
        for li, (planes, nb) in enumerate(zip((64, 128, 256, 512), self.LAYERS), start=1):
            for bi in range(nb):
                q = "%s.layer%d.%d" % (r, li, bi)
                spec += [(q + ".conv1.weight", (planes, inpl, 3, 3))] + _bn_spec(q + ".bn1", planes)
                spec += [(q + ".conv2.weight", (planes, planes, 3, 3))] + _bn_spec(q + ".bn2", planes)
                if bi == 0 and li > 1:
                    spec += [(q + ".downsample.0.weight", (planes, inpl, 1, 1))] + _bn_spec(q + ".downsample.1", planes)
                inpl = planes
        spec += [(r + ".fc.weight", (1000, 512)), (r + ".fc.bias", (1000,))]
        _materialise(self, spec)

    def _pack(self):
        if self._packed is None:
            sd = self._sd()
            r = "backbone"
            p = {"stem": _fold(sd, r + ".conv1", r + ".bn1"), "blocks": []}
            w_stem = sd[r + ".conv1.weight"]
            if w_stem.is_cuda and tuple(w_stem.shape) == (64, 3, 7, 7):
                p["stem_p"] = ops.stem_weights(w_stem)
                p["stem_x3"] = ops.stem_x3_weights(w_stem)
            for li, nb in enumerate(self.LAYERS, start=1):
                for bi in range(nb):
                    q = "%s.layer%d.%d" % (r, li, bi)
                    blk = {"c1": _fold(sd, q + ".conv1", q + ".bn1", True), "c2": _fold(sd, q + ".conv2", q + ".bn2", True),
# ... 30 lines not shown
            if identity is None:
                identity = x
                if "ds" in blk:
                    Wd, sd_, shd, _ = blk["ds"]
                    identity = ops.conv2d(x, Wd, sd_, shd, 1, 1, blk["stride"], 0, False, tap_major=True)
            x, _ = _block_conv3x3(blk, "2", y, 1, identity)
            if blk["last_of_stage"]:
                stage_out[blk["stage"]] = x
        return stage_out[3], stage_out[4], ops.global_avgpool(stage_out[4])


class KeypointDetector(_PackedModule):
    fuse_head = True

    def __init__(self, opt):
        super().__init__()
        self.opt = opt
        self.pc_encoder = PCEncoder(opt, Ca=64, Cb=256, Cg=512)
        self.img_encoder = ImageEncoder(opt)
        self.H_fine_res = int(round(opt.img_H / opt.img_fine_resolution_scale))
        self.W_fine_res = int(round(opt.img_W / opt.img_fine_resolution_scale))
        L = self.H_fine_res * self.W_fine_res
        spec = (_pn_spec("node_b_attention_pn", 256 + 512, [256, L], False)
                + _pn_spec("node_b_pn", 256 + 512 + 512 + 512, [1024, 512, 512], False)
                + _pn_spec("node_a_attention_pn", 64 + 512, [256, L * 4], False)
                + _pn_spec("node_a_pn", 64 + 256 + 512, [512, 128, 128], False))
        if opt.is_fine_resolution:
            spec += _pn_spec("per_point_pn", 736, [256, 256, 2 + L], False)
        else:
            spec += _pn_spec("per_point_pn", 736, [128, 128, 2], False)
        _materialise(self, spec)

    def _pack(self):
        if self._packed is None:
            sd = {k: v for k, v in self.state_dict().items() if not k.startswith(("pc_encoder.", "img_encoder."))}
            p = {n: _pn_pack(sd, n) for n in ("node_b_attention_pn", "node_b_pn", "node_a_attention_pn", "node_a_pn", "per_point_pn")}
            Wt = p["node_b_pn"][0][0]
            p["node_b_pn_dense_Wt"] = torch.cat((Wt[0:256], Wt[768:1280]), dim=0).contiguous()
            l0, l1, l2 = p["per_point_pn"]
            if (l0[0].is_cuda and tuple(l0[0].shape) == (736, 128) and tuple(l1[0].shape) == (128, 128) and l2[0].shape[0] == 128
                    and l2[0].shape[1] <= 4 and not l0[0].requires_grad):
                ones = torch.ones(128, device=l0[0].device)
                p["head_x3"] = {"W0p": ops.head_x3_pack(l0[0][640:736].contiguous()), "W1p": ops.head_x3_pack(l1[0]),
                                "ss": torch.stack((l0[1] if l0[1] is not None else ones, l0[2], l1[1] if l1[1] is not None else ones, l1[2])).contiguous(),
                                "relu0": l0[3], "relu1": l1[3], "W2t": l2[0], "sc2": l2[1], "sh2": l2[2], "relu2": l2[3]}
            if (l0[0].is_cuda and l0[0].shape[1] == 256 and tuple(l1[0].shape) == (256, 256) and l2[0].shape[0] == 256 and l2[0].shape[1] >= 3
                    and not l2[3] and not l0[0].requires_grad):
                p["head_labels_x3"] = {"W1p": ops.head_labels_pack(l1[0]), "W2p": ops.head_labels_pack(l2[0]), "P": int(l2[0].shape[1]),
                                       "sc1": l1[1] if l1[1] is not None else torch.ones(256, device=l1[0].device), "sh1": l1[2],
                                       "relu1": l1[3], "sc2": l2[1], "sh2": l2[2]}
            self._packed = p
        return self._packed

    def forward(self, pc, intensity, sn, node_a, node_b, img):
        p, B, N, first, second, idx_a, idx_pb, gathered = self._trunk(pc, intensity, sn, node_a, node_b, img)
        Wt, sc, sh, act = p["per_point_pn"][0]
        M0 = Wt.shape[1]
        G_a, ex_w_a = gathered[0][0], gathered[0][2]
        G_b, w_pb = gathered[1][0], gathered[1][2]
        l1, l2 = p["per_point_pn"][1], p["per_point_pn"][2]
        if ("head_x3" in p and self.fuse_head and _lib.get_option("head_x3") and first.shape[1] == 32 and second.shape[1] == 64
                and idx_a.shape[-1] == 3 and idx_pb.shape[-1] == 3):
            scores = ops.point_head_x3(first, second, p["head_x3"],
                                       [(G_a, idx_a.reshape(B, N, 3), ex_w_a), (G_b, idx_pb.reshape(B, N, 3), w_pb)], N)
        elif M0 == 128 and l1[0].shape[1] == 128 and l2[0].shape[1] <= 4 and N % 4 == 0 and self.fuse_head:
            scores = ops.point_head([Src(first), Src(second)], (Wt[640:736], sc, sh, act), l1, l2, N, gathered=gathered)
        else:
            h = ops.pointwise_gemm([Src(first), Src(second)], Wt[640:736], M0, N, scale=sc, shift=sh, relu=act, gathered=gathered)
            scores = _run_pn(h, p["per_point_pn"][1:], x3=False if M0 == 128 else None)
        coarse = scores[:, 0:2, :]
        if self.opt.is_fine_resolution:
            return coarse, scores[:, 2:, :]
        return coarse

    def predict_labels(self, pc, intensity, sn, node_a, node_b, img, scores_out=None):
        if not self.opt.is_fine_resolution:
            return ops.argmax_channels(self.forward(pc, intensity, sn, node_a, node_b, img)), None
        p, B, N, first, second, idx_a, idx_pb, gathered = self._trunk(pc, intensity, sn, node_a, node_b, img)
        Wt, sc, sh, act = p["per_point_pn"][0]
        M0 = Wt.shape[1]
        h = ops.pointwise_gemm([Src(first), Src(second)], Wt[640:736], M0, N, scale=sc, shift=sh, relu=act, gathered=gathered)
        if "head_labels_x3" not in p:
            raise RuntimeError("predict_labels: the fine head has no labels-only kernel for per_point_pn %s"
                               % [tuple(l[0].shape) for l in p["per_point_pn"]])
        return ops.point_head_labels(h, p["head_labels_x3"], N, scores_out=scores_out)

    def _trunk(self, pc, intensity, sn, node_a, node_b, img):
        ops.require_cuda(pc, intensity, sn, node_a, node_b, img)
        p = self._pack()
        B, N, Ma, Mb = pc.size(0), pc.size(2), node_a.size(2), node_b.size(2)
        (pc_center, cluster_mean, idx_a, first, second, node_a_features, node_b_features, global_feature), ex = \
            self.pc_encoder.forward_device(pc, intensity, sn, node_a, node_b)
        s16, s32, iglob = self.img_encoder(img)
        s16f = s16.view(B, s16.size(1), -1)
        s32f = s32.view(B, s32.size(1), -1)
        ig = iglob.view(B, -1)
        gf = global_feature.view(B, -1)

        Wt, sc, sh, act = p["node_b_attention_pn"][0]
        h = ops.pointwise_gemm([Src(node_b_features)], Wt[0:256], Wt.shape[1], Mb, scale=sc, shift=sh, relu=act,
                               batch_bias=ops.batch_gemv(Wt, 256, ig))
        score_b = _run_pn(h, p["node_b_attention_pn"][1:])
        w_s32 = ops.attention_pool(s32f, score_b)
        Wt, sc, sh, act = p["node_b_pn"][0]
        bias = ops.batch_gemv2(Wt, 256, gf, 1280, ig)
        h = ops.pointwise_gemm([Src(node_b_features), Src(w_s32)], p["node_b_pn_dense_Wt"], Wt.shape[1], Mb,
                               scale=sc, shift=sh, relu=act, batch_bias=bias)
        up_b = _run_pn(h, p["node_b_pn"][1:])
        idx_pb, w_pb = ops.knn_nodes(pc, node_b, self.opt.k_interp_point_b, want_weights=True)
        Wt, sc, sh, act = p["node_a_attention_pn"][0]
        h = ops.pointwise_gemm([Src(node_a_features)], Wt[0:64], Wt.shape[1], Ma, scale=sc, shift=sh, relu=act,
                               batch_bias=ops.batch_gemv(Wt, 64, ig))
        score_a = _run_pn(h, p["node_a_attention_pn"][1:])
        w_s16 = ops.attention_pool(s16f, score_a)
        idx_ab, w_ab = ops.knn_nodes(node_a, node_b, self.opt.k_interp_ab, want_weights=True)
        interp_ab = ops.interpolate(up_b, idx_ab, w_ab)
        h = _run_layer([Src(node_a_features), Src(interp_ab), Src(w_s16)], p["node_a_pn"][0], Ma)
        up_a = _run_pn(h, p["node_a_pn"][1:])
        Wt, sc, sh, act = p["per_point_pn"][0]
        M0 = Wt.shape[1]
        G_a = ops.pointwise_gemm([Src(up_a)], Wt[0:128], M0, Ma, transpose_out=True)
        G_b = ops.pointwise_gemm([Src(up_b)], Wt[128:640], M0, Mb, transpose_out=True)
        gathered = [(G_a, idx_a, ex["w_a"]), (G_b, idx_pb, w_pb)]
        return p, B, N, first, second, idx_a, idx_pb, gathered

    def intermediates(self, pc, intensity, sn, node_a, node_b, img):
        p = self._pack()
        B, N, Ma, Mb = pc.size(0), pc.size(2), node_a.size(2), node_b.size(2)
        t, ex = self.pc_encoder.forward_device(pc, intensity, sn, node_a, node_b)
        s16, s32, iglob = self.img_encoder(img)
        return dict(pc_center=t[0], cluster_mean=t[1], a_min_k_idx=t[2], first_pn_out=t[3], second_pn_out=t[4],
                    node_a_features=t[5], node_b_features=t[6], global_feature=t[7], s16=s16, s32=s32, img_global=iglob,
                    w_a=ex["w_a"], knn_I=ex["knn_I"])


def model_state_dict_convert_auto(sd):
    if len(sd) and all(k.startswith("module.") for k in sd):
        return {k[len("module."):]: v for k, v in sd.items()}
    return sd


class MMClassifer:

    fine = True

    def __init__(self, opt, writer=None):
        self.opt = opt
        self.writer = writer
        opt.is_fine_resolution = self.fine if not hasattr(opt, "is_fine_resolution") else opt.is_fine_resolution
        self.device = getattr(opt, "device", torch.device("cuda", 0))
        self.detector = KeypointDetector(opt).to(self.device).eval()
        self.pc = self.intensity = self.sn = self.node_a = self.node_b = self.P = self.img = self.K = None

    def load_model(self, model_path):
        self.detector.load_state_dict(model_state_dict_convert_auto(torch.load(model_path, map_location="cpu")))

    def set_input(self, pc, intensity, sn, node_a, node_b, P, img, K):
        def put(name, t):
            cur = getattr(self, name)
            if cur is None or cur.shape != t.shape or cur.dtype != t.dtype:
                cur = torch.empty(t.shape, dtype=t.dtype, device=self.device)
                setattr(self, name, cur)
            cur.copy_(t, non_blocking=True)
        for n, t in (("pc", pc), ("intensity", intensity), ("sn", sn), ("node_a", node_a), ("node_b", node_b),
                     ("P", P), ("img", img), ("K", K)):
            put(n, t)

    def forward(self, pc, intensity, sn, node_a, node_b, img):
        return self.detector(pc, intensity, sn, node_a, node_b, img)

    def _trainer(self):
        if getattr(self, "_trainer_obj", None) is None:
            from .training import ClassifierTrainer
            self._trainer_obj = ClassifierTrainer(self.detector, self.opt, lr=self._lr())
        return self._trainer_obj

    def _lr(self):
# ... 51 lines not shown
```

deepi2p_amd/ops.py:

```python
import ctypes
import weakref

import torch

from . import _lib
from ._lib import EpilogueT, SrcT, call, ptr, require_cuda, stream

_f32, _i32, _f64 = torch.float32, torch.int32, torch.float64
MAX_GK = 16


def _chk(t, dtype, name):
    if t.dtype != dtype:
        raise RuntimeError("%s must be %s, got %s" % (name, dtype, t.dtype))


def _work(name, macs):
    if _lib.WORK is not None:
        _lib.WORK[name] = _lib.WORK.get(name, 0) + macs


def index_max(data, index, K, return_values=False, mask=None):
    require_cuda(data, index, mask)
    _chk(data, _f32, "data")
# ... 7 lines not shown
    idx = torch.empty((B, C, K), dtype=_i32, device=data.device)
    ws = torch.empty((B * C * K,), dtype=torch.int64, device=data.device)
    if return_values:
        val = torch.empty((B, C, K), dtype=_f32, device=data.device)
        call("di2p_index_max_values", ptr(data), ptr(index), ptr(mask), ptr(val), ptr(idx), B, C, N, K, ptr(ws), stream())
        return idx, val
    call("di2p_index_max_forward", ptr(data), ptr(index), ptr(idx), B, C, N, K, ptr(ws), stream())
    return idx


def ball_query(node_to_point_dist, radius, K):
    require_cuda(node_to_point_dist)
    _chk(node_to_point_dist, _f32, "node_to_point_dist")
    B, M, N = node_to_point_dist.shape
    out = torch.empty((B, M, int(K)), dtype=_i32, device=node_to_point_dist.device)
    call("di2p_ball_query_forward", ptr(node_to_point_dist), ptr(out), float(radius), int(K), B, M, N, stream())
    return out


def _shape(t, shape, name, what):
    if t.dim() != len(shape) or any(e is not None and int(s) != int(e) for s, e in zip(t.shape, shape)):
        raise RuntimeError("%s must be %s, got %s" % (name, what, list(t.shape)))


def knn_nodes(query, nodes, k, want_weights=False):
    require_cuda(query, nodes)
    _chk(query, _f32, "query")
    _chk(nodes, _f32, "nodes")
    _shape(query, (None, 3, None), "query", "f32[B, 3, Nq]")
    B, _, Nq = query.shape
    _shape(nodes, (B, 3, None), "nodes", "f32[B, 3, M] for query f32[B, 3, Nq]")
    M, k = nodes.shape[2], int(k)
    idx = torch.empty((B, Nq, k), dtype=_i32, device=query.device)
    w = torch.empty((B, Nq, k), dtype=_f32, device=query.device) if want_weights else None
    call("di2p_knn_nodes", ptr(query), ptr(nodes), ptr(idx), ptr(w), B, Nq, M, k, stream())
    return (idx, w) if want_weights else idx


def cluster_stats(pc, knn_idx, M):
    require_cuda(pc, knn_idx)
    _chk(pc, _f32, "pc")
    _chk(knn_idx, _i32, "knn_idx")
    _shape(pc, (None, 3, None), "pc", "f32[B, 3, N]")
    B, _, N = pc.shape
    _shape(knn_idx, (B, N, None), "knn_idx", "i32[B, N, k] for pc f32[B, 3, N]")
    M = int(M)
    mean = torch.empty((B, 3, M), dtype=_f32, device=pc.device)
    mask = torch.empty((B, M), dtype=_f32, device=pc.device)
    min_idx = torch.empty((B, N), dtype=_i32, device=pc.device)
    call("di2p_cluster_stats", ptr(pc), ptr(knn_idx), knn_idx.shape[2], ptr(mean), ptr(mask), ptr(min_idx), B, N, M, stream())
    return mean, mask, min_idx


def build_point_input(pc, intensity, sn, cluster_mean, min_idx):
    require_cuda(pc, intensity, sn, cluster_mean, min_idx)
    for t, name in ((pc, "pc"), (intensity, "intensity"), (sn, "sn"), (cluster_mean, "cluster_mean")):
        _chk(t, _f32, name)
    _chk(min_idx, _i32, "min_idx")
    _shape(pc, (None, 3, None), "pc", "f32[B, 3, N]")
    B, _, N = pc.shape
    _shape(intensity, (B, 1, N), "intensity", "f32[B, 1, N] for pc f32[B, 3, N]")
    _shape(sn, (B, 3, N), "sn", "f32[B, 3, N] for pc f32[B, 3, N]")
    _shape(cluster_mean, (B, 3, None), "cluster_mean", "f32[B, 3, M] for pc f32[B, 3, N]")
    _shape(min_idx, (B, N), "min_idx", "i32[B, N] for pc f32[B, 3, N]")
    centers = torch.empty_like(pc)
    aug = torch.empty((B, 7, N), dtype=_f32, device=pc.device)
    call("di2p_build_point_input", ptr(pc), ptr(intensity), ptr(sn), ptr(cluster_mean), ptr(min_idx), ptr(centers),
         ptr(aug), B, N, cluster_mean.shape[2], stream())
    return centers, aug


def interpolate(feats, idx, weights):
    require_cuda(feats, idx, weights)
    _chk(feats, _f32, "feats")
    _chk(idx, _i32, "idx")
    _chk(weights, _f32, "weights")
    _shape(feats, (None, None, None), "feats", "f32[B, C, M]")
    B, C, M = feats.shape
    _shape(idx, (B, None, None), "idx", "i32[B, Nq, k] for feats f32[B, C, M]")
    Nq, k = idx.shape[1], idx.shape[2]
    _shape(weights, (B, Nq, k), "weights", "f32[B, Nq, k] for idx i32[B, Nq, k]")
    out = torch.empty((B, C, Nq), dtype=_f32, device=feats.device)
    call("di2p_interpolate", ptr(feats), ptr(idx), ptr(weights), ptr(out), B, C, M, Nq, k, stream())
    return out


def gather_neighbors(database, query, idx):
    require_cuda(database, query, idx)
    _chk(database, _f32, "database")
    _chk(query, _f32, "query")
    _chk(idx, _i32, "idx")
    _shape(database, (None, 3, None), "database", "f32[B, 3, Md]")
    B, _, Md = database.shape
    _shape(query, (B, 3, None), "query", "f32[B, 3, Mq] for database f32[B, 3, Md]")
    _shape(idx, (B, query.shape[2], None), "idx", "i32[B, Mq, K] for query f32[B, 3, Mq]")
    Mq, K = idx.shape[1], idx.shape[2]
    out = torch.empty((B, 3, Mq * K), dtype=_f32, device=database.device)
    call("di2p_gather_neighbors", ptr(database), ptr(query), ptr(idx), ptr(out), B, Md, Mq, K, stream())
    return out


def argmax_channels(scores):
    if not scores.is_cuda:
        raise RuntimeError("tensor must be a CUDA tensor/variable")
    B, C, N = scores.shape
    if scores.stride(2) != 1 or scores.stride(1) != N:
        raise RuntimeError("scores rows must be contiguous")
    out = torch.empty((B, N), dtype=_i32, device=scores.device)
    call("di2p_argmax_channels", ptr(scores), ptr(out), B, C, N, scores.stride(0), stream())
    return out


def channel_max(x):
    require_cuda(x)
    _chk(x, _f32, "x")
    _shape(x, (None, None, None), "x", "f32[B, C, N]")
    B, C, N = x.shape
    out = torch.empty((B, C), dtype=_f32, device=x.device)
    call("di2p_channel_max", ptr(x), ptr(out), B, C, N, stream())
# ... 196 lines not shown
        e.planes_out = ptr(Y.t)
        if group_max > 1:
            Ymax = torch.empty((B, M, Nout), dtype=_f32, device=Wt.device)
            e.group_max_out = ptr(Ymax)
        y_ptr = None
    elif also_full and group_max > 1:
        Y = torch.empty((B, M, N), dtype=_f32, device=Wt.device)
        Ymax = torch.empty((B, M, Nout), dtype=_f32, device=Wt.device)
        e.group_max_out = ptr(Ymax)
        y_ptr = ptr(Y)
    else:
        Y = torch.empty((B, Nout, M) if transpose_out else (B, M, Nout), dtype=_f32, device=Wt.device)
        y_ptr = ptr(Y)
    if Wp is not None:
        _work("di2p_pointwise_gemm_x3", B * M * K * N)
        if from_planes:
            call("di2p_pointwise_gemm_x3p", ptr(srcs[0].t), ptr(Wp), y_ptr, B, M, K, N, ctypes.byref(e), stream())
        else:
            call("di2p_pointwise_gemm_x3", arr, len(srcs), ptr(Wp), y_ptr, B, M, K, N, ctypes.byref(e), stream())
        return (Y, Ymax) if Ymax is not None else Y
    _work("di2p_pointwise_gemm", B * M * K * N)
    call("di2p_pointwise_gemm", arr, len(srcs), ptr(Wt), ptr(Y), B, M, K, N, ctypes.byref(e), stream())
    return (Y, Ymax) if Ymax is not None else Y


def point_head(srcs, layer0, layer1, layer2, N, batch_bias=None, gathered=None):
    Wt0, sc0, sh0, act0 = layer0
    Wt1, sc1, sh1, act1 = layer1
    Wt2, sc2, sh2, act2 = layer2
    B = srcs[0].t.shape[0]
    M, P = Wt0.shape[1], Wt2.shape[1]
    require_cuda(Wt0, Wt1, Wt2, sc0, sh0, sc1, sh1, sc2, sh2, batch_bias)
    e = EpilogueT()
    e.scale, e.shift, e.batch_bias = ptr(sc0), ptr(sh0), ptr(batch_bias)
    e.relu, e.group_max, e.transpose_out = int(bool(act0)), 1, 0
    _fill_gathered(e, gathered, B, M, N)
    out = torch.empty((B, P, N), dtype=_f32, device=Wt0.device)
    _work("di2p_point_head", B * N * (Wt0.shape[0] * M + M * M + M * P))
    call("di2p_point_head", _fill_srcs(srcs), len(srcs), ptr(Wt0), Wt0.shape[0], ctypes.byref(e), ptr(Wt1), ptr(sc1), ptr(sh1),
         int(bool(act1)), ptr(Wt2), ptr(sc2), ptr(sh2), int(bool(act2)), ptr(out), B, M, P, N, stream())
    return out


def head_x3_pack(Wt):
    require_cuda(Wt)
    K, M = Wt.shape
    if M != 128 or K % 16 or not Wt.is_contiguous():
        raise RuntimeError("head_x3_pack needs a contiguous f32[K,128] with K % 16 == 0")
    Wp = torch.empty((_lib.load().di2p_head_x3_packed_bytes(K),), dtype=torch.uint8, device=Wt.device)
    call("di2p_head_x3_pack", ptr(Wt), K, ptr(Wp), stream())
    return Wp


def point_head_x3(src0, src1, packed, gathered, N):
    require_cuda(src0, src1, packed["W0p"], packed["W1p"], packed["ss"], packed["W2t"], packed["sc2"], packed["sh2"])
    B = src0.shape[0]
    P = packed["W2t"].shape[1]
    k0 = int(src0.shape[1]) + int(src1.shape[1])
    hb = _lib.load().di2p_head_x3_packed_bytes
    if k0 % 16 or packed["W0p"].numel() * packed["W0p"].element_size() != hb(k0) or packed["W1p"].numel() * packed["W1p"].element_size() != hb(128):
        raise RuntimeError("point_head_x3: W0p / W1p must be head_x3_pack of the [%d,128] dense rows and of the [128,128] second layer" % k0)
    for name, n in (("ss", 4 * 128), ("W2t", 128 * P), ("sc2", P), ("sh2", P)):
        if packed[name] is None and name in ("sc2", "sh2"):
            continue
        _chk(packed[name], _f32, "point_head_x3 " + name)
        if packed[name].numel() < n:
            raise RuntimeError("point_head_x3: %s holds %d values, needs %d" % (name, packed[name].numel(), n))
    if tuple(packed["W2t"].shape) != (128, P) or not 1 <= P <= 4:
        raise RuntimeError("point_head_x3: W2t must be f32[128,P] with P <= 4")
    h = _lib.HeadX3T()
    for t, x in enumerate((src0, src1)):
        _chk(x, _f32, "head source")
        if x.dim() != 3 or x.shape[2] != N or x.stride(2) != 1:
            raise RuntimeError("head sources must be [B, ch, N] with unit column stride")
        h.src[t], h.batch_stride[t], h.row_stride[t], h.channels[t] = ptr(x), x.stride(0), x.stride(1), x.shape[1]
    for t, (tab, gi, gw) in enumerate(gathered):
        require_cuda(tab, gi, gw)
        _chk(tab, _f32, "gathered table")
        _chk(gi, _i32, "gathered index")
        if tuple(tab.shape[0::2]) != (B, 128) or tuple(gi.shape) != (B, N, 3) or (gw is not None and tuple(gw.shape) != (B, N, 3)):
            raise RuntimeError("the head takes node tables [B,nodes,128] with three neighbours per point")
        h.tab[t], h.idx[t], h.w[t], h.nodes[t] = ptr(tab), ptr(gi), ptr(gw), tab.shape[1]
    h.W0p, h.W1p, h.scale_shift = ptr(packed["W0p"]), ptr(packed["W1p"]), ptr(packed["ss"])
    h.relu0, h.relu1, h.relu2, h.P = int(bool(packed["relu0"])), int(bool(packed["relu1"])), int(bool(packed["relu2"])), P
    h.W2t, h.scale2, h.shift2 = ptr(packed["W2t"]), ptr(packed["sc2"]), ptr(packed["sh2"])
    out = torch.empty((B, P, N), dtype=_f32, device=src0.device)
    _work("di2p_point_head_x3", B * N * ((src0.shape[1] + src1.shape[1]) * 128 + 128 * 128 + 128 * P))
    call("di2p_point_head_x3", ctypes.byref(h), ptr(out), B, N, stream())
    return out


def head_labels_pack(Wt):
    require_cuda(Wt)
    _chk(Wt, _f32, "head_labels_pack weights")
    if Wt.dim() != 2 or Wt.shape[0] % 16 or Wt.shape[0] < 16:
        raise RuntimeError("head_labels_pack needs a contiguous f32[K,M] with K % 16 == 0")
    K, M = int(Wt.shape[0]), int(Wt.shape[1])
    Wp = torch.empty((_lib.load().di2p_head_labels_x3_packed_bytes(K, M),), dtype=torch.uint8, device=Wt.device)
    call("di2p_head_labels_x3_pack", ptr(Wt), K, M, ptr(Wp), stream())
    return Wp


def point_head_labels(y0, packed, N, scores_out=None):
    require_cuda(y0, packed["W1p"], packed["W2p"], packed["sc1"], packed["sh1"], packed["sc2"], packed["sh2"], scores_out)
    _chk(y0, _f32, "point_head_labels y0")
    P = int(packed["P"])
    if y0.dim() != 3 or y0.shape[1] != 256 or y0.shape[2] != N or y0.stride(2) != 1:
        raise RuntimeError("point_head_labels: y0 must be f32[B,256,N] with unit column stride")
    B = int(y0.shape[0])
    hb = _lib.load().di2p_head_labels_x3_packed_bytes
    if P < 3 or packed["W1p"].numel() * packed["W1p"].element_size() != hb(256, 256) or packed["W2p"].numel() * packed["W2p"].element_size() != hb(256, P):
        raise RuntimeError("point_head_labels: W1p / W2p must be head_labels_pack of the [256,256] layer 1 and of the [256,%d] layer 2 (P >= 3)" % P)
    for name, n in (("sc1", 256), ("sh1", 256), ("sc2", P), ("sh2", P)):
        if packed[name] is None:
            if name in ("sc2", "sh2"):
                continue
            raise RuntimeError("point_head_labels: %s is required" % name)
        _chk(packed[name], _f32, "point_head_labels " + name)
        if packed[name].numel() != n:
            raise RuntimeError("point_head_labels: %s holds %d values, needs %d" % (name, packed[name].numel(), n))
    if scores_out is not None:
        _chk(scores_out, _f32, "point_head_labels scores_out")
        if tuple(scores_out.shape) != (B, P, N) or scores_out.device != y0.device:
            raise RuntimeError("point_head_labels: scores_out must be f32[%d,%d,%d] on the device of y0" % (B, P, N))
    h = _lib.HeadLabelsX3T()
    h.y0, h.batch_stride, h.row_stride, h.K = ptr(y0), y0.stride(0), y0.stride(1), 256
    h.W1p, h.scale1, h.shift1, h.relu1 = ptr(packed["W1p"]), ptr(packed["sc1"]), ptr(packed["sh1"]), int(bool(packed["relu1"]))
    h.W2p, h.scale2, h.shift2, h.P = ptr(packed["W2p"]), ptr(packed["sc2"]), ptr(packed["sh2"]), P
    coarse = torch.empty((B, N), dtype=_i32, device=y0.device)
    fine = torch.empty((B, N), dtype=_i32, device=y0.device)
    h.scores, h.coarse, h.fine = ptr(scores_out), ptr(coarse), ptr(fine)
    _work("di2p_point_head_labels_x3", B * N * 256 * (256 + P))
    call("di2p_point_head_labels_x3", ctypes.byref(h), B, N, stream())
    return coarse, fine


def point_chain_ok(srcs, layers, N):
    if len(layers) not in (2, 3) or len(srcs) != 1 or _lib.get_option("pw_nochain"):
        return False
    M = layers[0][0].shape[1]
    if M not in (32, 64) or layers[0][0].shape[0] > M or any(tuple(l[0].shape) != (M, M) for l in layers[1:]):
        return False
    if any(l[0].requires_grad or not l[0].is_contiguous() for l in layers):
        return False
    return srcs[0].mode == _lib.SRC_DENSE and srcs[0].t.stride(2) == 1


def point_chain(srcs, layers, N, batch_bias=None, gathered=None):
    Wt0, sc0, sh0, act0 = layers[0]
    Wt1, sc1, sh1, act1 = layers[1]
    Wt2, sc2, sh2, act2 = layers[2] if len(layers) == 3 else (None, None, None, False)
    B = srcs[0].t.shape[0]
    M = Wt0.shape[1]
    require_cuda(Wt0, Wt1, Wt2, sc0, sh0, sc1, sh1, sc2, sh2, batch_bias)
    e = EpilogueT()
    e.scale, e.shift, e.batch_bias = ptr(sc0), ptr(sh0), ptr(batch_bias)
    e.relu, e.group_max, e.transpose_out = int(bool(act0)), 1, 0
    _fill_gathered(e, gathered, B, M, N)
    out = torch.empty((B, M, N), dtype=_f32, device=Wt0.device)
    _work("di2p_point_chain", B * N * (Wt0.shape[0] * M + (len(layers) - 1) * M * M))
    call("di2p_point_chain", _fill_srcs(srcs), len(srcs), ptr(Wt0), Wt0.shape[0], ctypes.byref(e), ptr(Wt1), ptr(sc1), ptr(sh1),
         int(bool(act1)), ptr(Wt2), ptr(sc2), ptr(sh2), int(bool(act2)), ptr(out), B, M, N, stream())
    return out


def batch_gemv(Wt, k0, v):
    require_cuda(Wt, v)
    B, Kv = v.shape
    M = Wt.shape[1]
    out = torch.empty((B, M), dtype=_f32, device=Wt.device)
    call("di2p_batch_gemv", ptr(Wt), M, int(k0), ptr(v), Kv, ptr(out), B, stream())
    return out


def batch_gemv2(Wt, k0, v0, k1, v1):
    require_cuda(Wt, v0, v1)
    B = v0.shape[0]
    M = Wt.shape[1]
    out = torch.empty((B, M), dtype=_f32, device=Wt.device)
    call("di2p_batch_gemv2", ptr(Wt), M, int(k0), ptr(v0), v0.shape[1], int(k1), ptr(v1), v1.shape[1], ptr(out), B, stream())
    return out


def attention_pool(feat, score):
    require_cuda(feat, score)
    B, C, HW = feat.shape
    Mn = score.shape[2]
    out = torch.empty((B, C, Mn), dtype=_f32, device=feat.device)
    call("di2p_attention_pool", ptr(feat), ptr(score), ptr(out), B, C, HW, Mn, stream())
    return out


def _conv_operands(who, x, Cout, KH, KW, stride, pad, scale, shift, residual):
    _chk(x, _f32, who + " input")
    if x.dim() != 4:
        raise RuntimeError("%s takes x f32[B,Cin,H,W]" % who)
    B, Cin, H, W = x.shape
    OH, OW = (H + 2 * pad - KH) // stride + 1, (W + 2 * pad - KW) // stride + 1
    for name, v in (("scale", scale), ("shift", shift)):
        if v is None or v.dtype != _f32:
            raise RuntimeError("%s %s must be %s, got %s" % (who, name, _f32, None if v is None else v.dtype))
        if v.numel() < Cout:
            raise RuntimeError("%s: %s holds %d values, needs %d" % (who, name, v.numel(), Cout))
    if residual is not None:
        _chk(residual, _f32, who + " residual")
        if residual.shape != (B, Cout, OH, OW):
            raise RuntimeError("%s: residual must be f32%s, got %s" % (who, (B, Cout, OH, OW), tuple(residual.shape)))
    return B, Cin, H, W, OH, OW


def conv_route(x_shape, w_shape, stride, pad, training=False):
    B, Cin, H, W = x_shape
    Cout, _, KH, KW = w_shape
# ... 182 lines not shown
    require_cuda(w)
    U = torch.empty((16, Cin, Cout), dtype=_f32, device=w.device)
    call("di2p_winograd_weight_transform", ptr(w), ptr(U), Cin, Cout, stream())
    return U


def winograd_weights_dgrad(weight):
    Cout, Cin, KH, KW = weight.shape
    if (KH, KW) != (3, 3) or weight.dtype != _f32:
        raise RuntimeError("winograd_weights_dgrad needs an f32 3x3 filter bank")
    w = weight.detach().contiguous()
    require_cuda(w)
    U = torch.empty((16, Cout, Cin), dtype=_f32, device=w.device)
    call("di2p_winograd_weight_transform_dgrad", ptr(w), ptr(U), Cout, Cin, stream())
    return U


def conv3x3_winograd(x, U, scale, shift, relu, residual=None):
    require_cuda(x, U, scale, shift, residual)
    _chk(U, _f32, "conv3x3_winograd U")
    Cout = U.shape[-1]
    B, Cin, H, W, _, _ = _conv_operands("conv3x3_winograd", x, Cout, 3, 3, 1, 1, scale, shift, residual)
    if tuple(U.shape) != (16, Cin, Cout):
        raise RuntimeError("U must be f32[16, Cin, Cout] = [16, %d, %d], got %s" % (Cin, Cout, tuple(U.shape)))
    y = torch.empty((B, Cout, H, W), dtype=_f32, device=x.device)
    _work("di2p_conv3x3_winograd", B * Cout * Cin * 16 * ((H + 1) // 2) * ((W + 1) // 2))
    call("di2p_conv3x3_winograd", ptr(x), ptr(U), ptr(scale), ptr(shift), ptr(residual), ptr(y), B, Cin, H, W, Cout, int(bool(relu)), stream())
    return y


def maxpool3x3s2(x):
    require_cuda(x)
    B, C, H, W = x.shape
    y = torch.empty((B, C, (H - 1) // 2 + 1, (W - 1) // 2 + 1), dtype=_f32, device=x.device)
    call("di2p_maxpool3x3s2", ptr(x), ptr(y), B, C, H, W, stream())
    return y


def global_avgpool(x):
    require_cuda(x)
    B, C, H, W = x.shape
    y = torch.empty((B, C, 1, 1), dtype=_f32, device=x.device)
    call("di2p_global_avgpool", ptr(x), ptr(y), B, C, H * W, stream())
    return y


def _dbl3(v):
    a = (ctypes.c_double * 3)()
    for i in range(3):
        a[i] = float(v[i])
    return a


def initial_guess(points64, labels):
    require_cuda(points64, labels)
    F, _, N = points64.shape
    yaw0 = torch.empty((F,), dtype=_f64, device=points64.device)
    labels_out = torch.empty_like(labels)
    has_inside = torch.empty((F,), dtype=_i32, device=points64.device)
    call("di2p_initial_guess", ptr(points64), ptr(labels), ptr(yaw0), ptr(labels_out), ptr(has_inside), F, N, stream())
    return yaw0, labels_out, has_inside


def solve_batched(points, labels, K, init_y, init_T, H, W, lb, ub, max_iter, is_2d, yaw0=None, sweeps=None, workspace=None):
    require_cuda(points, labels, K, init_y, init_T, yaw0, workspace)
    _chk(labels, _i32, "labels")
    _chk(K, _f64, "K")
    _chk(init_y, _f64, "init_y")
    _chk(init_T, _f64, "init_T")
    F, _, N = points.shape
    R = init_y.shape[1]
    npar = 4 if is_2d else 6
    params = torch.empty((F, R, npar), dtype=_f64, device=points.device)
    cost = torch.empty((F, R), dtype=_f64, device=points.device)
    iters = torch.empty((F, R), dtype=_i32, device=points.device)
    name = "di2p_solve_batched" if points.dtype == _f64 else "di2p_solve_batched_f32"
    if points.dtype not in (_f64, _f32):
        raise RuntimeError("points must be float64 or float32")
    need = _lib.load().di2p_solve_workspace_bytes(F, R, N)
    if workspace is None:
        ws = torch.empty((need,), dtype=torch.uint8, device=points.device)
    else:
        ws = workspace
        _chk(ws, torch.uint8, "workspace")
        if ws.device != points.device:
            raise RuntimeError("workspace must be on the points' device")
        if ws.numel() < need:
            raise RuntimeError("workspace has %d bytes, di2p_solve_workspace_bytes(%d, %d, %d) = %d" % (ws.numel(), F, R, N, need))
    call(name, ptr(points), ptr(labels), ptr(K), ptr(init_y), ptr(init_T), ptr(yaw0), float(H), float(W), _dbl3(lb),
         _dbl3(ub), int(max_iter), int(bool(is_2d)), F, R, N, ptr(params), ptr(cost), ptr(iters), ptr(sweeps), ptr(ws), stream())
    return params, cost, iters


def select_best(params, cost, is_2d, has_inside=None):
    require_cuda(params, cost, has_inside)
    F, R = cost.shape
    best = torch.empty((F,), dtype=_i32, device=cost.device)
    P = torch.empty((F, 4, 4), dtype=_f64, device=cost.device)
    bc = torch.empty((F,), dtype=_f64, device=cost.device)
    call("di2p_select_best", ptr(params), ptr(cost), ptr(has_inside), int(bool(is_2d)), F, R, ptr(best), ptr(P), ptr(bc), stream())
    return best, P, bc


def solver_residuals(points64, labels, K, params, H, W, is_2d):
    require_cuda(points64, labels, K, params)
    F, _, N = points64.shape
    res = torch.empty((F, 3 * N), dtype=_f64, device=points64.device)
    counts = torch.empty((F,), dtype=_i32, device=points64.device)
    cost = torch.empty((F,), dtype=_f64, device=points64.device)
    call("di2p_solver_residuals", ptr(points64), ptr(labels), ptr(K), ptr(params), float(H), float(W), int(bool(is_2d)),
         F, N, ptr(res), ptr(counts), ptr(cost), stream())
    return res, counts, cost
```

deepi2p_amd/registration.py:

```python
import math

import numpy as np
import torch

from . import ops

__version__ = "deepi2p_amd-1"


def _hip_dev():
    if not torch.cuda.is_available():
        raise RuntimeError("deepi2p_amd.registration needs a HIP device (there is no CPU fallback)")
    return torch.device("cuda", torch.cuda.current_device())


def solvePGivenK_batched(points, labels, K, init_y_angles, init_Ts, H, W, t_xyz_lower_bound, t_xyz_upper_bound,
                         max_iter, is_2d, return_all=False):
    dev = _hip_dev()
    pts = torch.as_tensor(np.ascontiguousarray(points, dtype=np.float64), device=dev).unsqueeze(0)
    lab = torch.as_tensor(np.ascontiguousarray(labels).astype(np.int32), device=dev).unsqueeze(0)
    Kt = torch.as_tensor(np.ascontiguousarray(K, dtype=np.float64), device=dev).reshape(1, 3, 3)
    ys = torch.as_tensor(np.ascontiguousarray(init_y_angles, dtype=np.float64), device=dev).reshape(1, -1)
    R = ys.shape[1]
    Ts = torch.as_tensor(np.ascontiguousarray(init_Ts, dtype=np.float64), device=dev).reshape(1, R, 3)
# ... 78 lines not shown
    noise, Ts = draw_restarts(rng, n, ry_sigma, init_t_amplitude)
    return init_y_angle + noise, Ts


def solve_P_random_perturb(pc_np, coarse_predictions_np, K_np, H, W, init_t_amplitude, init_y_angle, ry_sigma,
                           t_lowerbound, t_upperbound, iteration_num, is_2d, thread_num=None, rng=None,
                           restarts=None, max_iter=500):
    if restarts is None:
        ys, Ts = restart_list(init_y_angle, ry_sigma, init_t_amplitude, iteration_num, thread_num, rng)
    else:
        ys, Ts = restarts
    if len(ys) == 0:
        return None, 1e20, None
    P, cost, best, params, _ = solvePGivenK_batched(pc_np, coarse_predictions_np, K_np, ys, Ts, H, W, t_lowerbound,
                                                    t_upperbound, max_iter, is_2d, return_all=True)
    dev = _hip_dev()
    pts = torch.as_tensor(np.ascontiguousarray(pc_np, dtype=np.float64), device=dev).unsqueeze(0)
    lab = torch.as_tensor(np.ascontiguousarray(coarse_predictions_np).astype(np.int32), device=dev).unsqueeze(0)
    Kt = torch.as_tensor(np.ascontiguousarray(K_np, dtype=np.float64), device=dev).reshape(1, 3, 3)
    res, counts, _ = ops.solver_residuals(pts, lab, Kt, torch.as_tensor(params[best:best + 1], device=dev), H, W, is_2d)
    return P[best], float(cost[best]), res[0, :int(counts.item())].cpu().numpy()


class RegistrationPipeline:

    def __init__(self, H, W, R=60, ry_sigma=10 * math.pi / 180, init_t_amplitude=10.0,
                 t_lowerbound=(-5, -0.1, -10), t_upperbound=(5, 0.1, 10), max_iter=500, is_2d=True, seed=0, frame="cam"):
        from . import evaluation
        self.enu, self.frame = bool(evaluation.check_frame(frame)), frame
        self._convert = {}
        self.H, self.W, self.R = H, W, R
        self.ry_sigma, self.amp = ry_sigma, init_t_amplitude
        self.lb, self.ub = list(t_lowerbound), list(t_upperbound)
        self.max_iter, self.is_2d = max_iter, is_2d
        self.rng = np.random.default_rng(seed)

    def draw(self, F, device):
        noise, Ts = draw_restarts(self.rng, self.R, self.ry_sigma, self.amp, F=F)
        return (torch.as_tensor(noise, dtype=torch.float64, device=device),
                torch.as_tensor(Ts, dtype=torch.float64, device=device))

    def draw_on_device(self, F, device, seed):
        noise = torch.empty((F, self.R), dtype=torch.float64, device=device)
        Ts = torch.empty((F, self.R, 3), dtype=torch.float64, device=device)
        ops.call("di2p_draw_restarts", int(seed), F, self.R, float(self.ry_sigma), float(self.amp), ops.ptr(noise), ops.ptr(Ts),
                 ops.stream())
        return noise, Ts

    def __call__(self, pc_f32, labels_i32, K_f64, restarts):
        F, _, N = pc_f32.shape
        if self.enu:
            from . import evaluation
            pc_f32 = evaluation.enu2cam_points(pc_f32)
        pts64 = torch.empty((F, 3, N), dtype=torch.float64, device=pc_f32.device)
        ops.call("di2p_f32_to_f64", ops.ptr(pc_f32), ops.ptr(pts64), F * 3 * N, ops.stream())
        yaw0, lab_front, has_inside = ops.initial_guess(pts64, labels_i32)
        noise, Ts = restarts
        sweeps = torch.empty(noise.shape, dtype=torch.int32, device=pc_f32.device)
        params, cost, iters = ops.solve_batched(pc_f32, lab_front, K_f64, noise, Ts, self.H, self.W, self.lb, self.ub,
                                                self.max_iter, self.is_2d, yaw0=yaw0, sweeps=sweeps)
        best, P, bc = ops.select_best(params, cost, self.is_2d, has_inside=has_inside)
        out = dict(P=P, cost=bc, best=best, yaw0=yaw0, costs=cost, iters=iters, sweeps=sweeps, params=params, labels_front=lab_front)
        if self.enu:
            out["P_cam"], out["P"] = P, compose_convert(self._convert, P)
        return out


def compose_convert(cache, P_cam):
    key = (P_cam.device, P_cam.shape[0])
    if key not in cache:
        from . import evaluation
        cache[key] = evaluation.convert_matrices(P_cam.shape[0], P_cam.device)
    P = torch.empty_like(P_cam)
    ops.call("di2p_compose_poses", ops.ptr(P_cam), ops.ptr(cache[key]), P_cam.shape[0], ops.ptr(P), ops.stream())
    return P
```

include/deepi2p_hip.h:

```cpp
#ifndef DEEPI2P_HIP_H
#define DEEPI2P_HIP_H

#include <stdint.h>

#ifdef __cplusplus
extern "C" {
#endif

const char* di2p_last_error(void);
int di2p_version(void);
int di2p_set_option(const char* name, long long value);
long long di2p_get_option(const char* name);

int di2p_index_max_forward(const float* data, const int32_t* index, int32_t* max_idx,
                           int B, int C, int N, int K, void* workspace, void* stream);
int di2p_index_max_values(const float* data, const int32_t* index, const float* mask, float* max_val,
                          int32_t* max_idx, int B, int C, int N, int K, void* workspace, void* stream);

int di2p_ball_query_forward(const float* node_to_point_dist, int32_t* out_idx, float radius, int K,
                            int B, int M, int N, void* stream);

int di2p_knn_nodes(const float* query, const float* nodes, int32_t* idx, float* weights,
                   int B, int Nq, int M, int k, void* stream);
int di2p_cluster_stats(const float* pc, const int32_t* knn_idx, int idx_stride, float* cluster_mean,
                       float* mask, int32_t* min_idx, int B, int N, int M, void* stream);
int di2p_build_point_input(const float* pc, const float* intensity, const float* sn,
                           const float* cluster_mean, const int32_t* min_idx, float* pc_centers,
                           float* augmented, int B, int N, int M, void* stream);
int di2p_interpolate(const float* feats, const int32_t* idx, const float* weights, float* out,
                     int B, int C, int M, int Nq, int k, void* stream);
int di2p_gather_neighbors(const float* database, const float* query, const int32_t* idx, float* out,
                          int B, int Md, int Mq, int K, void* stream);
int di2p_argmax_channels(const float* scores, int32_t* out, int B, int C, int N, long long batch_stride , void* stream);

#define DI2P_MAX_SRC 3
#define DI2P_MAX_GK 16
enum { DI2P_SRC_DENSE = 0,
       DI2P_SRC_GATHER = 1,
       DI2P_SRC_GROUP = 2     };
typedef struct {
    const float* ptr;
    const int32_t* gidx;
    long long batch_stride;
    int row_stride;
    int channels;
    int mode;
    int group;
    int pad_;
} di2p_src_t;

typedef struct {
    const float* scale;
    const float* shift;
    const float* batch_bias;
    int relu;
    int group_max;
    const float* g_table[2];
    const int32_t* g_idx[2];
    const float* g_w[2];
    int g_nodes[2];
    int g_k[2];
    int transpose_out;
    float* group_max_out;
    void* planes_out;
} di2p_epilogue_t;

int di2p_pointwise_gemm(const di2p_src_t* srcs_host, int n_src, const float* Wt, float* Y,
                        int B, int M, int K, int N, const di2p_epilogue_t* epi_host, void* stream);
long long di2p_bf16x3_packed_bytes(int K, int M);
int di2p_bf16x3_pack(const float* Wt, int K, int M, void* Wp, void* stream);
int di2p_bf16x3_pack_conv3x3(const float* W, int Cout, int Cin, int dgrad, void* Wp, void* stream);
int di2p_pointwise_gemm_x3(const di2p_src_t* srcs_host, int n_src, const void* Wp, float* Y,
                           int B, int M, int K, int N, const di2p_epilogue_t* epi_host, void* stream);
long long di2p_bf16x3_planes_bytes(int B, int C, int N);
int di2p_pointwise_gemm_x3p(const void* planes, const void* Wp, float* Y,
                            int B, int M, int K, int N, const di2p_epilogue_t* epi_host, void* stream);

int di2p_point_head(const di2p_src_t* srcs_host, int n_src, const float* W0t, int K0, const di2p_epilogue_t* epi0_host,
                    const float* W1t, const float* scale1, const float* shift1, int relu1,
                    const float* W2t, const float* scale2, const float* shift2, int relu2,
                    float* out, int B, int M, int P, int N, void* stream);

int di2p_point_chain(const di2p_src_t* srcs_host, int n_src, const float* W0t, int K0, const di2p_epilogue_t* epi0_host,
                     const float* W1t, const float* scale1, const float* shift1, int relu1, const float* W2t,
                     const float* scale2, const float* shift2, int relu2, float* Y, int B, int M, int N, void* stream);

int di2p_batch_gemv(const float* Wt, int M, int k0, const float* v, int Kv, float* out, int B, void* stream);
int di2p_batch_gemv2(const float* Wt, int M, int k0, const float* v0, int Kv0, int k1, const float* v1, int Kv1,
                     float* out, int B, void* stream);

int di2p_attention_pool(const float* feat, const float* score, float* out, int B, int C, int HW, int Mn, void* stream);

int di2p_conv2d(const float* x, const float* Wt, const float* scale, const float* shift,
                const float* residual, float* y, int B, int Cin, int H, int W, int Cout,
                int KH, int KW, int stride, int pad, int relu, int tap_major, void* stream);
int di2p_conv2d_ws(const float* x, const float* Wt, const float* scale, const float* shift,
                   const float* residual, float* y, int B, int Cin, int H, int W, int Cout,
                   int KH, int KW, int stride, int pad, int relu, int tap_major,
                   void* workspace, long long workspace_bytes, void* stream);
long long di2p_conv2d_workspace_bytes(int B, int Cin, int H, int W, int Cout, int KH, int KW, int stride, int pad,
                                      int tap_major);
int di2p_winograd_weight_transform(const float* weight, float* U, int Cin, int Cout, void* stream);
int di2p_winograd_weight_transform_dgrad(const float* weight, float* U, int Cin_g, int Cout_g, void* stream);
int di2p_conv3x3_winograd(const float* x, const float* U, const float* scale, const float* shift, const float* residual, float* y, int B,
                          int Cin, int H, int W, int Cout, int relu, void* stream);
int di2p_pointwise_route(int M, int K, int N, int B, int dense, int wt_aligned, int32_t* out);
int di2p_conv2d_route(int B, int Cin, int H, int W, int Cout, int KH, int KW, int stride, int pad, int tap_major, int x_aligned,
                      int wt_aligned, long long workspace_bytes, int32_t* out);
int di2p_winograd_route(int B, int Cin, int H, int W, int Cout, int32_t* out);
int di2p_point_chain_route(int M, int K0, int layers, int B, int N, int cus, int32_t* out);
int di2p_point_head_route(int K0, int n_src, int c0, int reg_range, int g33, int B, int N, int cus, int32_t* out);
typedef struct {
    const float* src[2]; long long batch_stride[2]; int row_stride[2]; int channels[2];
    const void* W0p; const void* W1p; const float* scale_shift; int relu0, relu1;
    const float* tab[2]; const int32_t* idx[2]; const float* w[2]; int nodes[2];
    const float* W2t; const float* scale2; const float* shift2; int relu2, P;
} di2p_head_x3_t;
long long di2p_head_x3_packed_bytes(int K);
int di2p_head_x3_pack(const float* Wt, int K, void* Wp, void* stream);
int di2p_point_head_x3(const di2p_head_x3_t* h, float* out, int B, int N, void* stream);
typedef struct {
    const float* y0; long long batch_stride; int row_stride; int K;
    const void* W1p; const float* scale1; const float* shift1; int relu1;
    const void* W2p; const float* scale2; const float* shift2; int P;
    float* scores; int32_t* coarse; int32_t* fine;
} di2p_head_labels_x3_t;
long long di2p_head_labels_x3_packed_bytes(int K, int P);
int di2p_head_labels_x3_pack(const float* Wt, int K, int P, void* Wp, void* stream);
int di2p_point_head_labels_x3(const di2p_head_labels_x3_t* h, int B, int N, void* stream);
int di2p_conv3x3_x3_supported(int B, int Cin, int H, int W, int Cout, int stride, int cfg);
int di2p_conv3x3_x3_plan(int B, int Cin, int H, int W, int Cout, int stride, int cfg, int32_t* out);
int di2p_conv3x3_x3(const float* x, const void* Wp, const float* scale, const float* shift, const float* residual, float* y, int B,
                    int Cin, int H, int W, int Cout, int stride, int relu, const void* Wp_ds, const float* scale_ds,
                    const float* shift_ds, float* y_ds, int cfg, void* stream);
int di2p_stem_pack(const float* weight, float* Wp, void* stream);
int di2p_conv7x7s2_stem(const float* x, const float* Wp, const float* scale, const float* shift, float* y, int B, int H, int W, int relu,
                        void* stream);
int di2p_maxpool3x3s2(const float* x, float* y, int B, int C, int H, int W, void* stream);
long long di2p_stem_x3_packed_bytes(void);
int di2p_stem_x3_pack(const float* weight, void* Wp, void* stream);
int di2p_stem_x3_supported(int H, int W);
int di2p_stem_x3(const float* x, const void* Wp, const float* scale, const float* shift, float* y, int B, int H, int W, void* stream);
int di2p_global_avgpool(const float* x, float* y, int B, int C, int HW, void* stream);
int di2p_channel_max(const float* x, float* y, int B, int C, int N, void* stream);

int di2p_initial_guess(const double* points, const int32_t* labels, double* yaw0, int32_t* labels_out,
                       int32_t* has_inside, int F, int N, void* stream);
int di2p_solve_batched(const double* points, const int32_t* labels, const double* K,
                       const double* init_y, const double* init_T, const double* yaw0,
                       double H, double W, const double* lb_host, const double* ub_host,
                       int max_iter, int is_2d, int F, int R, int N,
                       double* params, double* cost, int32_t* iters, int32_t* sweeps , void* workspace, void* stream);
int di2p_solve_batched_f32(const float* points, const int32_t* labels, const double* K,
                           const double* init_y, const double* init_T, const double* yaw0,
                           double H, double W, const double* lb_host, const double* ub_host,
                           int max_iter, int is_2d, int F, int R, int N,
                           double* params, double* cost, int32_t* iters, int32_t* sweeps , void* workspace, void* stream);
long long di2p_solve_workspace_bytes(int F, int R, int N);
void di2p_solver_set_profile_buffer(void* buf);
int di2p_select_best(const double* params, const double* cost, const int32_t* has_inside, int is_2d,
                     int F, int R, int32_t* best, double* P, double* best_cost, void* stream);
int di2p_solver_residuals(const double* points, const int32_t* labels, const double* K,
                          const double* params, double H, double W, int is_2d, int F, int N,
                          double* residuals, int32_t* counts, double* cost, void* stream);

int di2p_farthest_point_sampling(const float* pts, const int32_t* init_idx, int32_t* idx_out, float* nodes_out,
                                 int B, int M, int k, void* stream);
int di2p_gather_points(const float* src, const int32_t* idx, float* out, int B, int C, int Nsrc, int Nout, void* stream);
int di2p_project_labels(const float* pc, const float* P, int p_rows, const float* K, float H, float W, float fine_scale,
                        int32_t* coarse, int32_t* fine, float* pxpy, int B, int N, void* stream);
int di2p_label_accuracy(const int32_t* coarse_pred, const int32_t* coarse_gt, const int32_t* fine_pred,
                        const int32_t* fine_gt, float* out, int B, int N, void* stream);
int di2p_pack_pc_label(const float* pc, const int32_t* coarse_pred, const int32_t* coarse_gt, const int32_t* fine_pred,
                       const int32_t* fine_gt, double* out, int B, int N, void* stream);

long long di2p_pnp_workspace_bytes(int F, int N, int iters);
int di2p_pnp_pack(const float* pc, const int32_t* coarse, const int32_t* fine, const float* pixels, int W_fine, int F, int N,
                  float* corr, int32_t* n_corr, void* stream);
int di2p_pnp_ransac(const float* pc, const int32_t* coarse, const int32_t* fine, const float* pixels,
                    const double* K_scaled, int W_fine, const int32_t* samples, int iters, double reproj_err,
                    int refine_rounds, int refine_iters, int F, int N, double* P_out, double* outlier_ratio, int32_t* n_inliers,
                    int32_t* n_corr, int32_t* best, void* workspace, void* stream);
int di2p_pnp_ransac_epnp(const float* pc, const int32_t* coarse, const int32_t* fine, const float* pixels,
                         const double* K_scaled, int W_fine, const int32_t* samples, int iters, double reproj_err, int F, int N,
                         double* P_out, double* outlier_ratio, int32_t* n_inliers, int32_t* n_corr, int32_t* best,
                         void* workspace, void* stream);

int di2p_f32_to_f64(const float* in, double* out, long long n, void* stream);

int di2p_draw_restarts(unsigned long long seed, int F, int R, double ry_sigma, double t_amplitude, double* ry_noise,
                       double* init_T, void* stream);
long long di2p_random_choice_workspace_bytes(int B, int n_src);
int di2p_random_choice(unsigned long long seed, int stream_id, int B, int n_src, int n_out, int32_t* idx_out, void* workspace,
                       void* stream);

long long di2p_random_choice_ragged_workspace_bytes(int B, int max_src);
int di2p_random_choice_ragged(unsigned long long seed, int stream_id, int B, const int32_t* offsets, int max_src, int n_out, int32_t* idx_out,
                              void* workspace, void* stream);

long long di2p_scan_prep_workspace_bytes(int B, int cap);
// ... 139 lines not shown
```

Measured before the change: 5106 frames/s.

## Add node-sorted point order with fused segmented max; read f32 points in initial guess

Adds an optional point permutation that sorts points by their assigned cluster node. The first point chain can then fuse the per-node max-pool through wave-level segmented shuffles and atomicMax on bit patterns, and the head kernel writes results back in the original order through the permutation. The node-order path is gated by a new option that defaults to off. Separately, the registration path now calls an f32 variant of the initial guess directly, which drops the f32-to-f64 conversion kernel and its buffer. The atomic max relies on non-negative post-ReLU values.

```diff
diff --git a/deepi2p_amd/_lib.py b/deepi2p_amd/_lib.py
--- a/deepi2p_amd/_lib.py
+++ b/deepi2p_amd/_lib.py
@@ -55,6 +55,8 @@
     "di2p_knn_nodes": [c_void_p, c_void_p, c_void_p, c_void_p, c_int, c_int, c_int, c_int, c_void_p],
     "di2p_cluster_stats": [c_void_p, c_void_p, c_int, c_void_p, c_void_p, c_void_p, c_int, c_int, c_int, c_void_p],
     "di2p_build_point_input": [c_void_p] * 7 + [c_int, c_int, c_int, c_void_p],
+    "di2p_build_point_input_perm": [c_void_p] * 8 + [c_int, c_int, c_int, c_void_p],
+    "di2p_point_perm": [c_void_p] * 5 + [c_int, c_void_p, c_int, c_int, c_int, c_int, c_void_p],
     "di2p_interpolate": [c_void_p] * 4 + [c_int] * 5 + [c_void_p],
     "di2p_gather_neighbors": [c_void_p] * 4 + [c_int] * 4 + [c_void_p],
     "di2p_argmax_channels": [c_void_p, c_void_p, c_int, c_int, c_int, c_ll, c_void_p],
@@ -72,12 +74,15 @@
                         c_void_p, c_int, c_void_p, c_int, c_int, c_int, c_int, c_void_p],
     "di2p_point_chain": [c_void_p, c_int, c_void_p, c_int, c_void_p, c_void_p, c_void_p, c_void_p, c_int, c_void_p, c_void_p,
                          c_void_p, c_int, c_void_p, c_int, c_int, c_int, c_void_p],
+    "di2p_point_chain_segmax": [c_void_p, c_int, c_void_p, c_int, c_void_p, c_void_p, c_void_p, c_void_p, c_int, c_void_p, c_void_p,
+                                c_void_p, c_int, c_void_p, c_void_p, c_void_p, c_int, c_int, c_int, c_int, c_void_p],
     "di2p_conv2d": [c_void_p] * 6 + [c_int] * 11 + [c_void_p],
     "di2p_conv2d_ws": [c_void_p] * 6 + [c_int] * 11 + [c_void_p, c_ll, c_void_p],
     "di2p_maxpool3x3s2": [c_void_p, c_void_p, c_int, c_int, c_int, c_int, c_void_p],
     "di2p_global_avgpool": [c_void_p, c_void_p, c_int, c_int, c_int, c_void_p],
     "di2p_channel_max": [c_void_p, c_void_p, c_int, c_int, c_int, c_void_p],
     "di2p_initial_guess": [c_void_p] * 5 + [c_int, c_int, c_void_p],
+    "di2p_initial_guess_f32": [c_void_p] * 5 + [c_int, c_int, c_void_p],
     "di2p_solve_batched": [c_void_p] * 6 + [c_double, c_double, ctypes.POINTER(c_double), ctypes.POINTER(c_double)]
                           + [c_int] * 5 + [c_void_p, c_void_p, c_void_p, c_void_p, c_void_p, c_void_p],
     "di2p_solve_batched_f32": [c_void_p] * 6 + [c_double, c_double, ctypes.POINTER(c_double), ctypes.POINTER(c_double)]
@@ -115,6 +120,7 @@
     "di2p_stem_x3_supported": [c_int, c_int],
     "di2p_stem_x3": [c_void_p] * 5 + [c_int] * 3 + [c_void_p],
     "di2p_point_head_x3": [ctypes.POINTER(HeadX3T), c_void_p, c_int, c_int, c_void_p],
+    "di2p_point_head_x3_perm": [ctypes.POINTER(HeadX3T), c_void_p, c_void_p, c_int, c_int, c_void_p],
     "di2p_head_labels_x3_pack": [c_void_p, c_int, c_int, c_void_p, c_void_p],
     "di2p_point_head_labels_x3": [ctypes.POINTER(HeadLabelsX3T), c_int, c_int, c_void_p],
     "di2p_bn_train_forward": [c_void_p] * 9 + [c_float, c_float, c_int, c_int, c_int, c_int, c_void_p, c_void_p],
diff --git a/deepi2p_amd/csrc/common.h b/deepi2p_amd/csrc/common.h
--- a/deepi2p_amd/csrc/common.h
+++ b/deepi2p_amd/csrc/common.h
@@ -56,7 +56,8 @@
     X(BN_UNFUSED, "bn_unfused", "DI2P_BN_UNFUSED", 0)                              \
     X(PW_X3_PLANES, "pw_x3_planes", "DI2P_PW_X3_PLANES", 1)                        \
     X(CONV_DGRAD_DENSE, "conv_dgrad_dense", "DI2P_CONV_DGRAD_DENSE", 0)            \
-    X(RC_TILE64, "rc_tile64", "DI2P_RC_TILE64", 0)
+    X(RC_TILE64, "rc_tile64", "DI2P_RC_TILE64", 0)                                 \
+    X(PT_NODE_ORDER, "pt_node_order", "DI2P_PT_NODE_ORDER", 0)
 enum Di2pOption {
 #define DI2P_OPT_ENUM(ID, NAME, ENV, DEF) DI2P_OPT_##ID,
     DI2P_OPTIONS(DI2P_OPT_ENUM)
diff --git a/deepi2p_amd/csrc/gemm.hip b/deepi2p_amd/csrc/gemm.hip
--- a/deepi2p_amd/csrc/gemm.hip
+++ b/deepi2p_amd/csrc/gemm.hip
@@ -476,9 +476,10 @@
 #ifndef DI2P_CHAIN_WAVES
 #define DI2P_CHAIN_WAVES 2
 #endif
-template <int M, int KS0, int NL, int TN>
+template <int M, int KS0, int NL, int TN, bool SEGMAX = false>
 __global__ __launch_bounds__(256) __attribute__((amdgpu_waves_per_eu(DI2P_CHAIN_WAVES, 8))) void point_chain_kernel(const float* __restrict__ X, long long x_bs, int x_rs, const float* __restrict__ W0t,
-                                                           int K0, EpiDev e0, ChainTail tl, float* __restrict__ Y, int N, int nblk, int total) {
+                                                           int K0, EpiDev e0, ChainTail tl, float* __restrict__ Y, int N, int nblk, int total,
+                                                           const int* __restrict__ seg_key, unsigned* __restrict__ seg_max, int seg_nodes) {
     constexpr int TM = M / 32, KS = M / 2, KSMAX = KS0 > KS ? KS0 : KS;
     extern __shared__ __attribute__((aligned(16))) float lds[];
     float* w0 = lds;
@@ -576,6 +577,27 @@
 #pragma unroll
                         for (int r = 0; r < 16; ++r)
                             Y[((long long)b * M + i * 32 + 4 * half + (r & 3) + 8 * (r >> 2)) * N + n[j]] = v[r];
+                    }
+                    if constexpr (SEGMAX) {
+                        const int key = n[j] < N ? seg_key[(long long)b * N + n[j]] : -1;
+#pragma unroll
+                        for (int o = 1; o < 32; o <<= 1) {
+                            const int left = __shfl_up(key, o, 32);
+                            const bool take = l31 >= o && left == key;
+#pragma unroll
+                            for (int r = 0; r < 16; ++r) {
+                                const float u = __shfl_up(v[r], o, 32);
+                                v[r] = take ? fmaxf(v[r], u) : v[r];
+                            }
+                        }
+                        const int right = __shfl_down(key, 1, 32);
+                        const bool last = l31 == 31 || right != key;
+                        if (last && (unsigned)key < (unsigned)seg_nodes) {
+#pragma unroll
+                            for (int r = 0; r < 16; ++r)
+                                atomicMax(&seg_max[((long long)b * M + i * 32 + 4 * half + (r & 3) + 8 * (r >> 2)) * seg_nodes + key],
+                                          __float_as_uint(fmaxf(v[r], 0.0f) + 0.0f));
+                        }
                     }
                 }
         };
@@ -1381,31 +1403,37 @@
     DI2P_RETURN_LAUNCH();
 }
 
-extern "C" int di2p_point_chain(const di2p_src_t* srcs, int n_src, const float* W0t, int K0, const di2p_epilogue_t* epi0,
-                                const float* W1t, const float* scale1, const float* shift1, int relu1, const float* W2t,
-                                const float* scale2, const float* shift2, int relu2, float* Y, int B, int M, int N, void* stream) {
-    DI2P_CHECK_ARG(srcs && n_src == 1 && W0t && W1t && epi0, "fused chain: one dense source");
-    DI2P_CHECK_ARG(M == 32 || M == 64, "fused chain: width 32 or 64 (use the separate layers otherwise)");
-    DI2P_CHECK_ARG(K0 <= M, "fused chain: at most M input channels");
-    DI2P_CHECK_ARG(B >= 0 && N >= 1 && K0 >= 1, "bad size");
-    DI2P_CHECK_ARG(epi0->group_max <= 1 && !epi0->transpose_out && !epi0->planes_out, "fused chain: layer 0 takes scale/shift/relu/bias/gathered only");
+static int point_chain_launch(const char* who, const di2p_src_t* srcs, int n_src, const float* W0t, int K0, const di2p_epilogue_t* epi0,
+                              const float* W1t, const float* scale1, const float* shift1, int relu1, const float* W2t,
+                              const float* scale2, const float* shift2, int relu2, float* Y, const int32_t* seg_key, float* seg_max,
+                              int seg_nodes, int B, int M, int N, void* stream) {
+#define CHAIN_CHECK(cond, msg) do { if (!(cond)) { di2p_set_error("%s: %s", who, msg); return -1; } } while (0)
+    CHAIN_CHECK(srcs && n_src == 1 && W0t && W1t && epi0, "fused chain: one dense source");
+    CHAIN_CHECK(M == 32 || M == 64, "fused chain: width 32 or 64 (use the separate layers otherwise)");
+    CHAIN_CHECK(K0 <= M, "fused chain: at most M input channels");
+    CHAIN_CHECK(B >= 0 && N >= 1 && K0 >= 1, "bad size");
+    CHAIN_CHECK(epi0->group_max <= 1 && !epi0->transpose_out && !epi0->planes_out, "fused chain: layer 0 takes scale/shift/relu/bias/gathered only");
     if (B == 0) return 0;
-    DI2P_CHECK_ARG(Y && srcs[0].ptr && srcs[0].channels == K0 && srcs[0].mode == DI2P_SRC_DENSE, "fused chain: one dense source of K0 channels");
-    DI2P_CHECK_ARG((long long)srcs[0].channels * srcs[0].row_stride < (1ll << 31), "per-frame source extent must fit 31 bits");
+    CHAIN_CHECK(Y && srcs[0].ptr && srcs[0].channels == K0 && srcs[0].mode == DI2P_SRC_DENSE, "fused chain: one dense source of K0 channels");
+    CHAIN_CHECK((long long)srcs[0].channels * srcs[0].row_stride < (1ll << 31), "per-frame source extent must fit 31 bits");
     EpiDev e;
-    if (pw_epilogue(__func__, epi0, nullptr, M, N, false, e)) return -1;
+    if (pw_epilogue(who, epi0, nullptr, M, N, false, e)) return -1;
     ChainTail tl{W1t, scale1, shift1, W2t, scale2, shift2, relu1, relu2};
     const float* X = srcs[0].ptr;
     const long long x_bs = srcs[0].batch_stride;
     const int x_rs = (int)srcs[0].row_stride;
     hipStream_t st = (hipStream_t)stream;
     const ChainRoute rt = chain_route(M, K0, W2t != nullptr, B, N, di2p_cu_count());
-    DI2P_CHECK_ARG(rt.total < (1ll << 30), "too many column blocks");
+    CHAIN_CHECK(rt.total < (1ll << 30), "too many column blocks");
 #define DI2P_CHAIN_LAUNCH(MM, KS0, NL, TN)                                                                                          \
     do {                                                                                                                            \
         const size_t lds = (size_t)(2 * (KS0) * (MM) + ((NL) - 1) * (MM) * (MM) + 6 * (MM)) * sizeof(float);                        \
-        hipLaunchKernelGGL((point_chain_kernel<MM, KS0, NL, TN>), dim3(rt.wgs), dim3(256), lds, st, X, x_bs, x_rs, W0t, K0, e, tl, Y, N, \
-                           rt.nblk, (int)rt.total);                                                                                 \
+        if (seg_key)                                                                                                                \
+            hipLaunchKernelGGL((point_chain_kernel<MM, KS0, NL, TN, true>), dim3(rt.wgs), dim3(256), lds, st, X, x_bs, x_rs, W0t, K0, e, tl, Y, N, \
+                               rt.nblk, (int)rt.total, seg_key, (unsigned*)seg_max, seg_nodes);                                     \
+        else                                                                                                                        \
+            hipLaunchKernelGGL((point_chain_kernel<MM, KS0, NL, TN>), dim3(rt.wgs), dim3(256), lds, st, X, x_bs, x_rs, W0t, K0, e, tl, Y, N, \
+                               rt.nblk, (int)rt.total, (const int*)nullptr, (unsigned*)nullptr, 0);                                 \
     } while (0)
     const bool three = rt.layers == 3;
     if (M == 32) {
@@ -1416,7 +1444,25 @@
         else              { if (three) DI2P_CHAIN_LAUNCH(64, 32, 3, DI2P_CHAIN_TN64); else DI2P_CHAIN_LAUNCH(64, 32, 2, DI2P_CHAIN_TN64); }
     }
 #undef DI2P_CHAIN_LAUNCH
+#undef CHAIN_CHECK
     DI2P_RETURN_LAUNCH();
+}
+
+extern "C" int di2p_point_chain(const di2p_src_t* srcs, int n_src, const float* W0t, int K0, const di2p_epilogue_t* epi0,
+                                const float* W1t, const float* scale1, const float* shift1, int relu1, const float* W2t,
+                                const float* scale2, const float* shift2, int relu2, float* Y, int B, int M, int N, void* stream) {
+    return point_chain_launch(__func__, srcs, n_src, W0t, K0, epi0, W1t, scale1, shift1, relu1, W2t, scale2, shift2, relu2, Y, nullptr, nullptr, 0,
+                              B, M, N, stream);
+}
+
+extern "C" int di2p_point_chain_segmax(const di2p_src_t* srcs, int n_src, const float* W0t, int K0, const di2p_epilogue_t* epi0,
+                                       const float* W1t, const float* scale1, const float* shift1, int relu1, const float* W2t,
+                                       const float* scale2, const float* shift2, int relu2, float* Y, const int32_t* seg_key, float* seg_max,
+                                       int nodes, int B, int M, int N, void* stream) {
+    DI2P_CHECK_ARG(seg_key && seg_max && nodes >= 1, "node-order chain: seg_key, seg_max and the node count are required");
+    DI2P_CHECK_ARG(W2t ? relu2 != 0 : relu1 != 0, "node-order chain: the last layer must end in ReLU (the maxima are combined on bit patterns)");
+    return point_chain_launch(__func__, srcs, n_src, W0t, K0, epi0, W1t, scale1, shift1, relu1, W2t, scale2, shift2, relu2, Y, seg_key, seg_max,
+                              nodes, B, M, N, stream);
 }
 
 extern "C" int di2p_point_chain_route(int M, int K0, int layers, int B, int N, int cus, int32_t* out) {
diff --git a/deepi2p_amd/csrc/head_x3.hip b/deepi2p_amd/csrc/head_x3.hip
--- a/deepi2p_amd/csrc/head_x3.hip
+++ b/deepi2p_amd/csrc/head_x3.hip
@@ -19,10 +19,11 @@
     const float* tab[2]; const int* idx[2]; const float* gw[2]; int nodes[2];
     const float* W2t; const float* sc2; const float* sh2;
     float* out;
+    const int* perm;
     int relu0, relu1, relu2, P, N, nblk, total, parts;
 };
 
-template <bool TAB_LDS, int KS0, int NW, int MINW, bool SYNC, bool DEEP, bool LEAN = false>
+template <bool TAB_LDS, int KS0, int NW, int MINW, bool SYNC, bool DEEP, bool LEAN = false, bool PERM = false>
 __global__ __launch_bounds__(NW * 64, MINW) void point_head_x3_kernel(const HxArgs a) {
     extern __shared__ __attribute__((aligned(16))) float lds[];
     float* ssl = lds;
@@ -69,11 +70,12 @@
         auto request_nb = [&](int gg, int (&gi_)[6], float (&gw_)[6]) __attribute__((always_inline)) {
             const int fq = TAB_LDS ? fb_fixed : __builtin_amdgcn_readfirstlane(gg / a.nblk);
             const int nq = min((gg - fq * a.nblk) * 32 + nl, a.N - 1);
+            const int pq = PERM ? a.perm[(long long)fq * a.N + nq] : nq;
 #pragma unroll
             for (int t = 0; t < 2; ++t)
 #pragma unroll
                 for (int j = 0; j < 3; ++j) {
-                    const long long o = ((long long)fq * a.N + nq) * 3 + j;
+                    const long long o = ((long long)fq * a.N + pq) * 3 + j;
                     gi_[3 * t + j] = a.idx[t][o];
                     gw_[3 * t + j] = a.gw[t] ? a.gw[t][o] : 1.0f;
                 }
@@ -223,6 +225,7 @@
             __builtin_amdgcn_sched_barrier(0);
         }
         __builtin_amdgcn_sched_barrier(0);
+        const int n_out = PERM ? a.perm[(long long)fb * a.N + nc] : n;
         {
             const int gn = min(g + g_stride, g_end - 1);
             request_nb(gn, gi_n, gw_n);
@@ -257,7 +260,7 @@
                 if (a.sc2) o *= a.sc2[p];
                 if (a.sh2) o += a.sh2[p];
                 if (a.relu2) o = fmaxf(o, 0.0f);
-                if (n < a.N && hq == 0 && live) a.out[((long long)fb * a.P + p) * a.N + n] = o;
+                if (n < a.N && hq == 0 && live) a.out[((long long)fb * a.P + p) * a.N + n_out] = o;
             }
         }
     }
@@ -298,6 +301,10 @@
 }
 
 extern "C" int di2p_point_head_x3(const di2p_head_x3_t* hd, float* out, int B, int N, void* stream) {
+    return di2p_point_head_x3_perm(hd, nullptr, out, B, N, stream);
+}
+
+extern "C" int di2p_point_head_x3_perm(const di2p_head_x3_t* hd, const int32_t* perm, float* out, int B, int N, void* stream) {
     DI2P_CHECK_ARG(hd && out, "null pointer");
     DI2P_CHECK_ARG(B >= 0 && N >= 1, "bad size");
     DI2P_CHECK_ARG(hd->src[0] && hd->src[1] && hd->W0p && hd->W1p && hd->scale_shift && hd->W2t, "null operand");
@@ -316,7 +323,7 @@
     }
     a.c0 = hd->channels[0]; a.K0 = hd->channels[0] + hd->channels[1];
     a.W0p = (const u32x4_t*)hd->W0p; a.W1p = (const u32x4_t*)hd->W1p; a.ss = hd->scale_shift;
-    a.W2t = hd->W2t; a.sc2 = hd->scale2; a.sh2 = hd->shift2; a.out = out;
+    a.W2t = hd->W2t; a.sc2 = hd->scale2; a.sh2 = hd->shift2; a.out = out; a.perm = perm;
     a.relu0 = hd->relu0; a.relu1 = hd->relu1; a.relu2 = hd->relu2; a.P = hd->P; a.N = N;
     a.nblk = di2p_cdiv(N, 32); a.total = B * a.nblk;
     hipStream_t st = (hipStream_t)stream;
@@ -330,15 +337,18 @@
         while (parts > 1 && a.nblk < parts * 16) --parts;
         a.parts = parts;
         if (opt == 2) {
-            if (di2p_allow_dynamic_lds((const void*)point_head_x3_kernel<true, 6, 4, 1, false, true>, lds_tab, __func__)) return -1;
-            hipLaunchKernelGGL((point_head_x3_kernel<true, 6, 4, 1, false, true>), dim3(B * parts), dim3(256), lds_tab, st, a);
+            const auto k = perm ? point_head_x3_kernel<true, 6, 4, 1, false, true, false, true> : point_head_x3_kernel<true, 6, 4, 1, false, true>;
+            if (di2p_allow_dynamic_lds((const void*)k, lds_tab, __func__)) return -1;
+            hipLaunchKernelGGL(k, dim3(B * parts), dim3(256), lds_tab, st, a);
         } else {
-            if (di2p_allow_dynamic_lds((const void*)point_head_x3_kernel<true, 6, 8, 2, false, false, true>, lds_tab, __func__)) return -1;
-            hipLaunchKernelGGL((point_head_x3_kernel<true, 6, 8, 2, false, false, true>), dim3(B * parts), dim3(512), lds_tab, st, a);
+            const auto k = perm ? point_head_x3_kernel<true, 6, 8, 2, false, false, true, true> : point_head_x3_kernel<true, 6, 8, 2, false, false, true>;
+            if (di2p_allow_dynamic_lds((const void*)k, lds_tab, __func__)) return -1;
+            hipLaunchKernelGGL(k, dim3(B * parts), dim3(512), lds_tab, st, a);
         }
     } else {
         const int grid = (int)(a.total / 4 < 1ll * di2p_cu_count() ? di2p_cdiv(a.total, 4) : di2p_cu_count());
-        hipLaunchKernelGGL((point_head_x3_kernel<false, 6, 4, 1, false, true>), dim3(grid), dim3(256), lds_small, st, a);
+        const auto k = perm ? point_head_x3_kernel<false, 6, 4, 1, false, true, false, true> : point_head_x3_kernel<false, 6, 4, 1, false, true>;
+        hipLaunchKernelGGL(k, dim3(grid), dim3(256), lds_small, st, a);
     }
     DI2P_RETURN_LAUNCH();
 }
diff --git a/deepi2p_amd/csrc/point_ops.hip b/deepi2p_amd/csrc/point_ops.hip
--- a/deepi2p_amd/csrc/point_ops.hip
+++ b/deepi2p_amd/csrc/point_ops.hip
@@ -163,13 +163,89 @@
     }
 }
 
+constexpr int PERM_WAVES = 16;
+
+__device__ __forceinline__ void perm_rank(int k, bool valid, int bits, int lane, int& rank, int& count) {
+    unsigned long long same = __ballot(valid);
+    for (int q = 0; q < bits; ++q) {
+        const unsigned long long set = __ballot(valid && ((k >> q) & 1));
+        same &= ((k >> q) & 1) ? set : ~set;
+    }
+    rank = __popcll(same & ((1ull << lane) - 1ull));
+    count = __popcll(same);
+}
+
+__global__ __launch_bounds__(1024) void point_perm_kernel(const int* __restrict__ min_idx, int* __restrict__ perm, int* __restrict__ seg,
+                                                          int* __restrict__ sorted_idx, float* __restrict__ zero0, int nz0,
+                                                          float* __restrict__ zero1, int nz1, int N, int M) {
+    extern __shared__ int s_perm[];
+    int* s_scan = s_perm + PERM_WAVES * M;
+    const int b = blockIdx.x, tid = threadIdx.x, lane = tid & 63, wave = tid >> 6;
+    if (zero0) for (int i = tid; i < nz0; i += 1024) zero0[(long long)b * nz0 + i] = 0.0f;
+    if (zero1) for (int i = tid; i < nz1; i += 1024) zero1[(long long)b * nz1 + i] = 0.0f;
+    for (int i = tid; i < PERM_WAVES * M; i += 1024) s_perm[i] = 0;
+    __syncthreads();
+    int bits = 0;
+    while ((1 << bits) < M) ++bits;
+    const int* key = min_idx + (long long)b * N;
+    const int chunk = ((N + PERM_WAVES - 1) / PERM_WAVES + 63) & ~63;
+    const int n0 = min(N, wave * chunk), n1 = min(N, n0 + chunk);
+    int* mine = s_perm + wave * M;
+    for (int base = n0; base < n1; base += 64) {
+        const int n = base + lane;
+        const bool valid = n < n1;
+        const int k = valid ? min(max(key[n], 0), M - 1) : 0;
+        int rank, count;
+        perm_rank(k, valid, bits, lane, rank, count);
+        if (valid && rank == 0) mine[k] += count;
+    }
+    __syncthreads();
+    int tot = 0;
+    if (tid < M)
+        for (int w = 0; w < PERM_WAVES; ++w) tot += s_perm[w * M + tid];
+    s_scan[tid] = tid < M ? tot : 0;
+    __syncthreads();
+    for (int o = 1; o < 1024; o <<= 1) {
+        const int v = tid >= o ? s_scan[tid - o] : 0;
+        __syncthreads();
+        s_scan[tid] += v;
+        __syncthreads();
+    }
+    if (tid < M) {
+        int run = s_scan[tid] - tot;
+        seg[(long long)b * (M + 1) + tid] = run;
+        for (int w = 0; w < PERM_WAVES; ++w) {
+            const int c = s_perm[w * M + tid];
+            s_perm[w * M + tid] = run;
+            run += c;
+        }
+    }
+    if (tid == 0) seg[(long long)b * (M + 1) + M] = N;
+    __syncthreads();
+    for (int base = n0; base < n1; base += 64) {
+        const int n = base + lane;
+        const bool valid = n < n1;
+        const int k = valid ? min(max(key[n], 0), M - 1) : 0;
+        int rank, count;
+        perm_rank(k, valid, bits, lane, rank, count);
+        if (valid) {
+            const int pos = mine[k] + rank;
+            perm[(long long)b * N + pos] = n;
+            sorted_idx[(long long)b * N + pos] = k;
+        }
+        __builtin_amdgcn_wave_barrier();
+        if (valid && rank == 0) mine[k] += count;
+    }
+}
+
 __global__ __launch_bounds__(256) void build_point_input_kernel(const float* __restrict__ pc, const float* __restrict__ intensity,
                                                                 const float* __restrict__ sn, const float* __restrict__ cluster_mean,
-                                                                const int* __restrict__ min_idx, float* __restrict__ centers,
-                                                                float* __restrict__ aug, int N, int M) {
+                                                                const int* __restrict__ min_idx, const int* __restrict__ perm,
+                                                                float* __restrict__ centers, float* __restrict__ aug, int N, int M) {
     const int b = blockIdx.y;
-    const int n = blockIdx.x * blockDim.x + threadIdx.x;
-    if (n >= N) return;
+    const int col = blockIdx.x * blockDim.x + threadIdx.x;
+    if (col >= N) return;
+    const int n = perm ? perm[(long long)b * N + col] : col;
     const int k = min_idx[(long long)b * N + n];
     const float* cm = cluster_mean + (long long)b * 3 * M;
     const float* p = pc + (long long)b * 3 * N;
@@ -178,12 +254,12 @@
     for (int c = 0; c < 3; ++c) {
         const float ctr = cm[c * M + k];
         if (centers) centers[((long long)b * 3 + c) * N + n] = ctr;
-        a[c * N + n] = __fsub_rn(p[c * N + n], ctr);
-    }
-    a[3 * N + n] = intensity[(long long)b * N + n];
+        a[c * N + col] = __fsub_rn(p[c * N + n], ctr);
+    }
+    a[3 * N + col] = intensity[(long long)b * N + n];
     const float* s = sn + (long long)b * 3 * N;
 #pragma unroll
-    for (int c = 0; c < 3; ++c) a[(4 + c) * N + n] = s[c * N + n];
+    for (int c = 0; c < 3; ++c) a[(4 + c) * N + col] = s[c * N + n];
 }
 
 __global__ __launch_bounds__(256) void interpolate_kernel(const float* __restrict__ feats, const int* __restrict__ idx,
@@ -313,10 +389,26 @@
 extern "C" int di2p_build_point_input(const float* pc, const float* intensity, const float* sn, const float* cluster_mean,
                                       const int32_t* min_idx, float* pc_centers, float* augmented, int B, int N, int M,
                                       void* stream) {
+    return di2p_build_point_input_perm(pc, intensity, sn, cluster_mean, min_idx, nullptr, pc_centers, augmented, B, N, M, stream);
+}
+
+extern "C" int di2p_build_point_input_perm(const float* pc, const float* intensity, const float* sn, const float* cluster_mean,
+                                           const int32_t* min_idx, const int32_t* perm, float* pc_centers, float* augmented, int B, int N,
+                                           int M, void* stream) {
     DI2P_CHECK_ARG(B >= 0 && N >= 0 && M > 0, "bad size");
     if (B == 0 || N == 0) return 0;
     hipLaunchKernelGGL(build_point_input_kernel, dim3(di2p_cdiv(N, 256), B), dim3(256), 0, (hipStream_t)stream, pc,
-                       intensity, sn, cluster_mean, min_idx, pc_centers, augmented, N, M);
+                       intensity, sn, cluster_mean, min_idx, perm, pc_centers, augmented, N, M);
+    DI2P_RETURN_LAUNCH();
+}
+
+extern "C" int di2p_point_perm(const int32_t* min_idx, int32_t* perm, int32_t* seg, int32_t* sorted_idx, float* zero0, int nz0,
+                               float* zero1, int nz1, int B, int N, int M, void* stream) {
+    DI2P_CHECK_ARG(min_idx && perm && seg && sorted_idx, "null pointer");
+    DI2P_CHECK_ARG(B >= 0 && N >= 0 && M >= 1 && M <= 512 && nz0 >= 0 && nz1 >= 0, "bad size (at most 512 nodes)");
+    if (B == 0) return 0;
+    hipLaunchKernelGGL(point_perm_kernel, dim3(B), dim3(1024), (size_t)(PERM_WAVES * M + 1024) * sizeof(int), (hipStream_t)stream, min_idx,
+                       perm, seg, sorted_idx, zero0, nz0, zero1, nz1, N, M);
     DI2P_RETURN_LAUNCH();
 }
 
diff --git a/deepi2p_amd/csrc/solver.hip b/deepi2p_amd/csrc/solver.hip
--- a/deepi2p_amd/csrc/solver.hip
+++ b/deepi2p_amd/csrc/solver.hip
@@ -1467,17 +1467,18 @@
     best_cost[f] = cost[(long long)f * R + bi];
 }
 
-__global__ __launch_bounds__(1024) void initial_guess_kernel(const double* __restrict__ points, const int* __restrict__ labels,
+template <class PT>
+__global__ __launch_bounds__(1024) void initial_guess_kernel(const PT* __restrict__ points, const int* __restrict__ labels,
                                                              double* __restrict__ yaw0, int* __restrict__ labels_out,
                                                              int* __restrict__ has_inside, int N) {
     __shared__ double s_a[1024], s_b[1024], s_c[1024];
     const int f = blockIdx.x, tid = threadIdx.x;
-    const double* px = points + (long long)f * 3 * N;
-    const double* pz = px + 2 * (long long)N;
+    const PT* px = points + (long long)f * 3 * N;
+    const PT* pz = px + 2 * (long long)N;
     const int* lab = labels + (long long)f * N;
     double sx = 0, sz = 0, cnt = 0;
     for (int n = tid; n < N; n += 1024)
-        if (lab[n] == 1) { sx += px[n]; sz += pz[n]; cnt += 1.0; }
+        if (lab[n] == 1) { sx += (double)px[n]; sz += (double)pz[n]; cnt += 1.0; }
     s_a[tid] = sx; s_b[tid] = sz; s_c[tid] = cnt;
     __syncthreads();
     for (int o = 512; o > 0; o >>= 1) {
@@ -1499,7 +1500,7 @@
     const double c = cos(a), s = sin(a);
     double zmin = __builtin_inf();
     for (int n = tid; n < N; n += 1024)
-        if (lab[n] == 1) zmin = fmin(zmin, -s * px[n] + c * pz[n]);
+        if (lab[n] == 1) zmin = fmin(zmin, -s * (double)px[n] + c * (double)pz[n]);
     s_a[tid] = zmin;
     __syncthreads();
     for (int o = 512; o > 0; o >>= 1) {
@@ -1508,7 +1509,7 @@
     }
     const double thr = s_a[0] - 10.0;
     for (int n = tid; n < N; n += 1024) {
-        const double zr = -s * px[n] + c * pz[n];
+        const double zr = -s * (double)px[n] + c * (double)pz[n];
         labels_out[(long long)f * N + n] = zr > thr ? lab[n] : -1;
     }
     if (tid == 0) { yaw0[f] = a; has_inside[f] = 1; }
@@ -1714,7 +1715,15 @@
                                   int32_t* has_inside, int F, int N, void* stream) {
     DI2P_CHECK_ARG(points && labels && yaw0 && labels_out && has_inside && F >= 0 && N >= 0, "bad args");
     if (F == 0) return 0;
-    hipLaunchKernelGGL(initial_guess_kernel, dim3(F), dim3(1024), 0, (hipStream_t)stream, points, labels, yaw0, labels_out, has_inside, N);
+    hipLaunchKernelGGL(initial_guess_kernel<double>, dim3(F), dim3(1024), 0, (hipStream_t)stream, points, labels, yaw0, labels_out, has_inside, N);
+    DI2P_RETURN_LAUNCH();
+}
+
+extern "C" int di2p_initial_guess_f32(const float* points, const int32_t* labels, double* yaw0, int32_t* labels_out,
+                                      int32_t* has_inside, int F, int N, void* stream) {
+    DI2P_CHECK_ARG(points && labels && yaw0 && labels_out && has_inside && F >= 0 && N >= 0, "bad args");
+    if (F == 0) return 0;
+    hipLaunchKernelGGL(initial_guess_kernel<float>, dim3(F), dim3(1024), 0, (hipStream_t)stream, points, labels, yaw0, labels_out, has_inside, N);
     DI2P_RETURN_LAUNCH();
 }
 
diff --git a/deepi2p_amd/networks.py b/deepi2p_amd/networks.py
--- a/deepi2p_amd/networks.py
+++ b/deepi2p_amd/networks.py
@@ -198,19 +198,45 @@
             torch.cuda.current_stream().synchronize()
         return cache[key]
 
-    def forward_device(self, pc, intensity, sn, node_a, node_b):
+    def node_order_ok(self, Ma):
+        if not _lib.get_option("pt_node_order") or _lib.get_option("pw_nochain") or Ma > 512:
+            return False
+        p = self._pack()
+        first, second = p["first"], p["second"]
+        Ch = first[-1][0].shape[1]
+        Wt0 = second[0][0]
+        if not first[0][0].is_cuda or any(l[0].requires_grad or not l[0].is_contiguous() for l in first + second):
+            return False
+        return (len(first) in (2, 3) and Ch in (32, 64) and first[0][0].shape[0] <= Ch and all(tuple(l[0].shape) == (Ch, Ch) for l in first[1:])
+                and len(second) in (2, 3) and Wt0.shape[0] == 2 * Ch and Wt0.shape[1] in (32, 64) and Ch <= Wt0.shape[1]
+                and all(tuple(l[0].shape) == (Wt0.shape[1], Wt0.shape[1]) for l in second[1:]) and bool(first[-1][3]) and bool(second[-1][3]))
+
+    def forward_device(self, pc, intensity, sn, node_a, node_b, node_order=False):
         if pc.size(2) != self.opt.input_pt_num:
             raise RuntimeError("N must equal opt.input_pt_num (the reference bakes it in, networks_pc.py:44-45)")
         p = self._pack()
         B, N, Ma, Mb = pc.size(0), pc.size(2), node_a.size(2), node_b.size(2)
         idx_a, w_a = ops.knn_nodes(pc, node_a, self.opt.k_interp_point_a, want_weights=True)
         cluster_mean, mask, min_idx = ops.cluster_stats(pc, idx_a, Ma)
-        pc_centers, aug = ops.build_point_input(pc, intensity, sn, cluster_mean, min_idx)
-        first = _run_pn(aug, p["first"])
-        _, first_max = ops.index_max(first, min_idx, Ma, return_values=True, mask=mask)
-        Ch = first.shape[1]
-        second = _run_split_pn([Src(first)], (0, Ch), first_max, (Ch, 2 * Ch), min_idx, p["second"], N)
-        _, node_a_features = ops.index_max(second, min_idx, Ma, return_values=True, mask=mask)
+        perm = None
+        if node_order:
+            Ch, Ca = p["first"][-1][0].shape[1], p["second"][-1][0].shape[1]
+            first_max = torch.empty((B, Ch, Ma), dtype=torch.float32, device=pc.device)
+            node_a_features = torch.empty((B, Ca, Ma), dtype=torch.float32, device=pc.device)
+            perm, _, key = ops.point_perm(min_idx, Ma, zero=(first_max, node_a_features))
+            pc_centers, aug = ops.build_point_input(pc, intensity, sn, cluster_mean, min_idx, perm=perm)
+            first = ops.point_chain([Src(aug)], p["first"], N, seg_max=(key, first_max))
+            Wt, scale, shift, act = p["second"][0]
+            G = ops.pointwise_gemm([Src(first_max)], Wt[Ch:2 * Ch], Wt.shape[1], Ma, transpose_out=True)
+            second = ops.point_chain([Src(first)], [(Wt[0:Ch], scale, shift, act)] + list(p["second"][1:]), N,
+                                     gathered=[(G, key.reshape(B, N, 1), None)], seg_max=(key, node_a_features))
+        else:
+            pc_centers, aug = ops.build_point_input(pc, intensity, sn, cluster_mean, min_idx)
+            first = _run_pn(aug, p["first"])
+            _, first_max = ops.index_max(first, min_idx, Ma, return_values=True, mask=mask)
+            Ch = first.shape[1]
+            second = _run_split_pn([Src(first)], (0, Ch), first_max, (Ch, 2 * Ch), min_idx, p["second"], N)
+            _, node_a_features = ops.index_max(second, min_idx, Ma, return_values=True, mask=mask)
         K = self.opt.k_ab
         knn_I = ops.knn_nodes(node_b, cluster_mean, K)
         coord = ops.gather_neighbors(cluster_mean, node_b, knn_I)
@@ -238,7 +264,7 @@
         final = _run_pn(final, p["final"][1:])
         global_feature = ops.channel_max(final).unsqueeze(2)
         ref_tuple = (pc_centers, cluster_mean, idx_a, first, second, node_a_features, node_b_features, global_feature)
-        return ref_tuple, dict(w_a=w_a, min_idx=min_idx, mask=mask, knn_I=knn_I)
+        return ref_tuple, dict(w_a=w_a, min_idx=min_idx, mask=mask, knn_I=knn_I, perm=perm, first_max=first_max)
 
     def forward(self, pc, intensity, sn, node_a, node_b):
         t, _ = self.forward_device(pc, intensity, sn, node_a, node_b)
@@ -375,17 +401,24 @@
             self._packed = p
         return self._packed
 
+    def _head_x3_route(self, p):
+        enc = self.pc_encoder._pack()
+        return ("head_x3" in p and self.fuse_head and bool(_lib.get_option("head_x3")) and enc["first"][-1][0].shape[1] == 32
+                and enc["second"][-1][0].shape[1] == 64 and self.opt.k_interp_point_a == 3 and self.opt.k_interp_point_b == 3)
+
     def forward(self, pc, intensity, sn, node_a, node_b, img):
-        p, B, N, first, second, idx_a, idx_pb, gathered = self._trunk(pc, intensity, sn, node_a, node_b, img)
+        p = self._pack()
+        x3 = self._head_x3_route(p)
+        node_order = x3 and self.pc_encoder.node_order_ok(node_a.size(2))
+        p, B, N, first, second, idx_a, idx_pb, gathered, perm = self._trunk(pc, intensity, sn, node_a, node_b, img, node_order=node_order)
         Wt, sc, sh, act = p["per_point_pn"][0]
         M0 = Wt.shape[1]
         G_a, ex_w_a = gathered[0][0], gathered[0][2]
         G_b, w_pb = gathered[1][0], gathered[1][2]
         l1, l2 = p["per_point_pn"][1], p["per_point_pn"][2]
-        if ("head_x3" in p and self.fuse_head and _lib.get_option("head_x3") and first.shape[1] == 32 and second.shape[1] == 64
-                and idx_a.shape[-1] == 3 and idx_pb.shape[-1] == 3):
+        if x3:
             scores = ops.point_head_x3(first, second, p["head_x3"],
-                                       [(G_a, idx_a.reshape(B, N, 3), ex_w_a), (G_b, idx_pb.reshape(B, N, 3), w_pb)], N)
+                                       [(G_a, idx_a.reshape(B, N, 3), ex_w_a), (G_b, idx_pb.reshape(B, N, 3), w_pb)], N, perm=perm)
         elif M0 == 128 and l1[0].shape[1] == 128 and l2[0].shape[1] <= 4 and N % 4 == 0 and self.fuse_head:
             scores = ops.point_head([Src(first), Src(second)], (Wt[640:736], sc, sh, act), l1, l2, N, gathered=gathered)
         else:
@@ -399,7 +432,7 @@
     def predict_labels(self, pc, intensity, sn, node_a, node_b, img, scores_out=None):
         if not self.opt.is_fine_resolution:
             return ops.argmax_channels(self.forward(pc, intensity, sn, node_a, node_b, img)), None
-        p, B, N, first, second, idx_a, idx_pb, gathered = self._trunk(pc, intensity, sn, node_a, node_b, img)
+        p, B, N, first, second, idx_a, idx_pb, gathered, _ = self._trunk(pc, intensity, sn, node_a, node_b, img)
         Wt, sc, sh, act = p["per_point_pn"][0]
         M0 = Wt.shape[1]
         h = ops.pointwise_gemm([Src(first), Src(second)], Wt[640:736], M0, N, scale=sc, shift=sh, relu=act, gathered=gathered)
@@ -408,12 +441,12 @@
                                % [tuple(l[0].shape) for l in p["per_point_pn"]])
         return ops.point_head_labels(h, p["head_labels_x3"], N, scores_out=scores_out)
 
-    def _trunk(self, pc, intensity, sn, node_a, node_b, img):
+    def _trunk(self, pc, intensity, sn, node_a, node_b, img, node_order=False):
         ops.require_cuda(pc, intensity, sn, node_a, node_b, img)
         p = self._pack()
         B, N, Ma, Mb = pc.size(0), pc.size(2), node_a.size(2), node_b.size(2)
         (pc_center, cluster_mean, idx_a, first, second, node_a_features, node_b_features, global_feature), ex = \
-            self.pc_encoder.forward_device(pc, intensity, sn, node_a, node_b)
+            self.pc_encoder.forward_device(pc, intensity, sn, node_a, node_b, node_order=node_order)
         s16, s32, iglob = self.img_encoder(img)
         s16f = s16.view(B, s16.size(1), -1)
         s32f = s32.view(B, s32.size(1), -1)
@@ -445,7 +478,7 @@
         G_a = ops.pointwise_gemm([Src(up_a)], Wt[0:128], M0, Ma, transpose_out=True)
         G_b = ops.pointwise_gemm([Src(up_b)], Wt[128:640], M0, Mb, transpose_out=True)
         gathered = [(G_a, idx_a, ex["w_a"]), (G_b, idx_pb, w_pb)]
-        return p, B, N, first, second, idx_a, idx_pb, gathered
+        return p, B, N, first, second, idx_a, idx_pb, gathered, ex["perm"]
 
     def intermediates(self, pc, intensity, sn, node_a, node_b, img):
         p = self._pack()
diff --git a/deepi2p_amd/ops.py b/deepi2p_amd/ops.py
--- a/deepi2p_amd/ops.py
+++ b/deepi2p_amd/ops.py
@@ -83,8 +83,28 @@
     return mean, mask, min_idx
 
 
-def build_point_input(pc, intensity, sn, cluster_mean, min_idx):
-    require_cuda(pc, intensity, sn, cluster_mean, min_idx)
+def point_perm(min_idx, M, zero=()):
+    require_cuda(min_idx, *zero)
+    _chk(min_idx, _i32, "min_idx")
+    _shape(min_idx, (None, None), "min_idx", "i32[B, N]")
+    B, N = min_idx.shape
+    if len(zero) > 2:
+        raise RuntimeError("point_perm clears at most two tables")
+    for z in zero:
+        _chk(z, _f32, "point_perm zero")
+        if z.shape[0] != B:
+            raise RuntimeError("a table to clear must be f32[B, ...]")
+    z = list(zero) + [None] * (2 - len(zero))
+    perm = torch.empty((B, N), dtype=_i32, device=min_idx.device)
+    seg = torch.empty((B, int(M) + 1), dtype=_i32, device=min_idx.device)
+    sorted_idx = torch.empty((B, N), dtype=_i32, device=min_idx.device)
+    call("di2p_point_perm", ptr(min_idx), ptr(perm), ptr(seg), ptr(sorted_idx), ptr(z[0]), 0 if z[0] is None else z[0][0].numel(),
+         ptr(z[1]), 0 if z[1] is None else z[1][0].numel(), B, N, int(M), stream())
+    return perm, seg, sorted_idx
+
+
+def build_point_input(pc, intensity, sn, cluster_mean, min_idx, perm=None):
+    require_cuda(pc, intensity, sn, cluster_mean, min_idx, perm)
     for t, name in ((pc, "pc"), (intensity, "intensity"), (sn, "sn"), (cluster_mean, "cluster_mean")):
         _chk(t, _f32, name)
     _chk(min_idx, _i32, "min_idx")
@@ -96,6 +116,12 @@
     _shape(min_idx, (B, N), "min_idx", "i32[B, N] for pc f32[B, 3, N]")
     centers = torch.empty_like(pc)
     aug = torch.empty((B, 7, N), dtype=_f32, device=pc.device)
+    if perm is not None:
+        _chk(perm, _i32, "perm")
+        _shape(perm, (B, N), "perm", "i32[B, N] for pc f32[B, 3, N]")
+        call("di2p_build_point_input_perm", ptr(pc), ptr(intensity), ptr(sn), ptr(cluster_mean), ptr(min_idx), ptr(perm), ptr(centers),
+             ptr(aug), B, N, cluster_mean.shape[2], stream())
+        return centers, aug
     call("di2p_build_point_input", ptr(pc), ptr(intensity), ptr(sn), ptr(cluster_mean), ptr(min_idx), ptr(centers),
          ptr(aug), B, N, cluster_mean.shape[2], stream())
     return centers, aug
@@ -398,8 +424,8 @@
     return Wp
 
 
-def point_head_x3(src0, src1, packed, gathered, N):
-    require_cuda(src0, src1, packed["W0p"], packed["W1p"], packed["ss"], packed["W2t"], packed["sc2"], packed["sh2"])
+def point_head_x3(src0, src1, packed, gathered, N, perm=None):
+    require_cuda(src0, src1, packed["W0p"], packed["W1p"], packed["ss"], packed["W2t"], packed["sc2"], packed["sh2"], perm)
     B = src0.shape[0]
     P = packed["W2t"].shape[1]
     k0 = int(src0.shape[1]) + int(src1.shape[1])
@@ -432,6 +458,12 @@
     h.W2t, h.scale2, h.shift2 = ptr(packed["W2t"]), ptr(packed["sc2"]), ptr(packed["sh2"])
     out = torch.empty((B, P, N), dtype=_f32, device=src0.device)
     _work("di2p_point_head_x3", B * N * ((src0.shape[1] + src1.shape[1]) * 128 + 128 * 128 + 128 * P))
+    if perm is not None:
+        _chk(perm, _i32, "perm")
+        if tuple(perm.shape) != (B, N):
+            raise RuntimeError("perm must be i32[B, N]")
+        call("di2p_point_head_x3_perm", ctypes.byref(h), ptr(perm), ptr(out), B, N, stream())
+        return out
     call("di2p_point_head_x3", ctypes.byref(h), ptr(out), B, N, stream())
     return out
 
@@ -492,7 +524,7 @@
     return srcs[0].mode == _lib.SRC_DENSE and srcs[0].t.stride(2) == 1
 
 
-def point_chain(srcs, layers, N, batch_bias=None, gathered=None):
+def point_chain(srcs, layers, N, batch_bias=None, gathered=None, seg_max=None):
     Wt0, sc0, sh0, act0 = layers[0]
     Wt1, sc1, sh1, act1 = layers[1]
     Wt2, sc2, sh2, act2 = layers[2] if len(layers) == 3 else (None, None, None, False)
@@ -505,6 +537,16 @@
     _fill_gathered(e, gathered, B, M, N)
     out = torch.empty((B, M, N), dtype=_f32, device=Wt0.device)
     _work("di2p_point_chain", B * N * (Wt0.shape[0] * M + (len(layers) - 1) * M * M))
+    if seg_max is not None:
+        key, table = seg_max
+        require_cuda(key, table)
+        _chk(key, _i32, "seg_max index")
+        _chk(table, _f32, "seg_max table")
+        if tuple(key.shape) != (B, N) or table.dim() != 3 or tuple(table.shape[:2]) != (B, M):
+            raise RuntimeError("seg_max must be (i32[B, N], f32[B, M, nodes])")
+        call("di2p_point_chain_segmax", _fill_srcs(srcs), len(srcs), ptr(Wt0), Wt0.shape[0], ctypes.byref(e), ptr(Wt1), ptr(sc1), ptr(sh1),
+             int(bool(act1)), ptr(Wt2), ptr(sc2), ptr(sh2), int(bool(act2)), ptr(out), ptr(key), ptr(table), table.shape[2], B, M, N, stream())
+        return out
     call("di2p_point_chain", _fill_srcs(srcs), len(srcs), ptr(Wt0), Wt0.shape[0], ctypes.byref(e), ptr(Wt1), ptr(sc1), ptr(sh1),
          int(bool(act1)), ptr(Wt2), ptr(sc2), ptr(sh2), int(bool(act2)), ptr(out), B, M, N, stream())
     return out
@@ -793,13 +835,16 @@
     return a
 
 
-def initial_guess(points64, labels):
-    require_cuda(points64, labels)
-    F, _, N = points64.shape
-    yaw0 = torch.empty((F,), dtype=_f64, device=points64.device)
+def initial_guess(points, labels):
+    require_cuda(points, labels)
+    if points.dtype not in (_f64, _f32):
+        raise RuntimeError("points must be float64 or float32, got %s" % points.dtype)
+    F, _, N = points.shape
+    yaw0 = torch.empty((F,), dtype=_f64, device=points.device)
     labels_out = torch.empty_like(labels)
-    has_inside = torch.empty((F,), dtype=_i32, device=points64.device)
-    call("di2p_initial_guess", ptr(points64), ptr(labels), ptr(yaw0), ptr(labels_out), ptr(has_inside), F, N, stream())
+    has_inside = torch.empty((F,), dtype=_i32, device=points.device)
+    call("di2p_initial_guess" if points.dtype == _f64 else "di2p_initial_guess_f32", ptr(points), ptr(labels), ptr(yaw0), ptr(labels_out),
+         ptr(has_inside), F, N, stream())
     return yaw0, labels_out, has_inside
 
 
diff --git a/deepi2p_amd/registration.py b/deepi2p_amd/registration.py
--- a/deepi2p_amd/registration.py
+++ b/deepi2p_amd/registration.py
@@ -154,9 +154,7 @@
         if self.enu:
             from . import evaluation
             pc_f32 = evaluation.enu2cam_points(pc_f32)
-        pts64 = torch.empty((F, 3, N), dtype=torch.float64, device=pc_f32.device)
-        ops.call("di2p_f32_to_f64", ops.ptr(pc_f32), ops.ptr(pts64), F * 3 * N, ops.stream())
-        yaw0, lab_front, has_inside = ops.initial_guess(pts64, labels_i32)
+        yaw0, lab_front, has_inside = ops.initial_guess(pc_f32, labels_i32)
         noise, Ts = restarts
         sweeps = torch.empty(noise.shape, dtype=torch.int32, device=pc_f32.device)
         params, cost, iters = ops.solve_batched(pc_f32, lab_front, K_f64, noise, Ts, self.H, self.W, self.lb, self.ub,
diff --git a/include/deepi2p_hip.h b/include/deepi2p_hip.h
--- a/include/deepi2p_hip.h
+++ b/include/deepi2p_hip.h
@@ -27,6 +27,11 @@
 int di2p_build_point_input(const float* pc, const float* intensity, const float* sn,
                            const float* cluster_mean, const int32_t* min_idx, float* pc_centers,
                            float* augmented, int B, int N, int M, void* stream);
+int di2p_point_perm(const int32_t* min_idx, int32_t* perm, int32_t* seg, int32_t* sorted_idx, float* zero0, int nz0, float* zero1,
+                    int nz1, int B, int N, int M, void* stream);
+int di2p_build_point_input_perm(const float* pc, const float* intensity, const float* sn, const float* cluster_mean,
+                                const int32_t* min_idx, const int32_t* perm, float* pc_centers, float* augmented, int B, int N, int M,
+                                void* stream);
 int di2p_interpolate(const float* feats, const int32_t* idx, const float* weights, float* out,
                      int B, int C, int M, int Nq, int k, void* stream);
 int di2p_gather_neighbors(const float* database, const float* query, const int32_t* idx, float* out,
@@ -84,6 +89,10 @@
 int di2p_point_chain(const di2p_src_t* srcs_host, int n_src, const float* W0t, int K0, const di2p_epilogue_t* epi0_host,
                      const float* W1t, const float* scale1, const float* shift1, int relu1, const float* W2t,
                      const float* scale2, const float* shift2, int relu2, float* Y, int B, int M, int N, void* stream);
+int di2p_point_chain_segmax(const di2p_src_t* srcs_host, int n_src, const float* W0t, int K0, const di2p_epilogue_t* epi0_host,
+                            const float* W1t, const float* scale1, const float* shift1, int relu1, const float* W2t,
+                            const float* scale2, const float* shift2, int relu2, float* Y, const int32_t* seg_key, float* seg_max,
+                            int nodes, int B, int M, int N, void* stream);
 
 int di2p_batch_gemv(const float* Wt, int M, int k0, const float* v, int Kv, float* out, int B, void* stream);
 int di2p_batch_gemv2(const float* Wt, int M, int k0, const float* v0, int Kv0, int k1, const float* v1, int Kv1,
@@ -119,6 +128,7 @@
 long long di2p_head_x3_packed_bytes(int K);
 int di2p_head_x3_pack(const float* Wt, int K, void* Wp, void* stream);
 int di2p_point_head_x3(const di2p_head_x3_t* h, float* out, int B, int N, void* stream);
+int di2p_point_head_x3_perm(const di2p_head_x3_t* h, const int32_t* perm, float* out, int B, int N, void* stream);
 typedef struct {
     const float* y0; long long batch_stride; int row_stride; int K;
     const void* W1p; const float* scale1; const float* shift1; int relu1;
@@ -146,6 +156,8 @@
 
 int di2p_initial_guess(const double* points, const int32_t* labels, double* yaw0, int32_t* labels_out,
                        int32_t* has_inside, int F, int N, void* stream);
+int di2p_initial_guess_f32(const float* points, const int32_t* labels, double* yaw0, int32_t* labels_out,
+                           int32_t* has_inside, int F, int N, void* stream);
 int di2p_solve_batched(const double* points, const int32_t* labels, const double* K,
                        const double* init_y, const double* init_T, const double* yaw0,
                        double H, double W, const double* lb_host, const double* ub_host,
```

Measured after the change: 5170 frames/s, median of 6. 1.3% higher.
